# mkkellogg/GaussianSplats3D

Hardware: NVIDIA H100
Metric: frames_per_sec (higher is better)
Workload: dtype int32 sort keys / f32 raster

## Files before the change

### gaussiansplats3d_b200/csrc/engine.cu

```cuda
#include "../../include/gsplat_b200.h"
#include "common.cuh"
#include "sort_kernels.cuh"
#include "raster_kernels.cuh"
#include "shard_kernels.cuh"
#include "ksplat_transform.h"
#include "ksplat_kernels.cuh"
#include "file_kernels.cuh"
#include "cull_kernels.cuh"
#include "ray_kernels.cuh"
#include "generate_kernels.cuh"

#include <algorithm>
#include <cmath>
#include <cstdarg>
#include <cstdlib>
#include <cstring>
#include <memory>
#include <new>
#include <vector>

using namespace gs;

thread_local char g_gs_err[512] = "";
#define g_err g_gs_err
// ... 208 lines not shown
    CUE(cudaStreamCreateWithFlags(&e->stream, cudaStreamNonBlocking));
    CUE(cudaStreamCreateWithFlags(&e->stream2, cudaStreamNonBlocking));
    CUE(cudaEventCreateWithFlags(&e->ev_fork, cudaEventDisableTiming));
    CUE(cudaEventCreateWithFlags(&e->ev_join, cudaEventDisableTiming));
    for (int i = 0; i < EV_COUNT; ++i) CUE(cudaEventCreate(&e->ev[i]));
    int kb = 0;
    while ((1u << kb) < c.distance_map_range) ++kb;
    e->key_bits = kb;
    int rc = GS_OK;
    const size_t n = std::max<uint32_t>(c.max_splat_count, 1);
    if ((rc = e->centers.ensure(n)) || (rc = e->indexes.ensure(n)) || (rc = e->dist.ensure(n)) || (rc = e->sorted.ensure(n)) ||
        (rc = e->vals[0].ensure(n)) || (rc = e->vals[1].ensure(n)) || (rc = e->keys[0].ensure(n)) || (rc = e->keys[1].ensure(n)) ||
        (rc = e->ctl.ensure(1)) || (rc = e->depthp.ensure(2)) || (rc = e->transforms.ensure(16 * GS_MAX_SCENES)) || (rc = e->h_ctl.ensure(sizeof(SortControl) / 4 + 64 + sizeof(RasterControl) / 4 + sizeof(ShardHeader) / 4))) {
        gs_destroy(e);
        return rc;
    }
    if (c.dynamic_mode && (rc = e->scene_idx.ensure(n))) { gs_destroy(e); return rc; }
    if (c.ray_records && (rc = e->ray.rec.ensure(n))) { gs_destroy(e); return rc; }
    if (e->scene_idx.p) CUE(cudaMemsetAsync(e->scene_idx.p, 0, e->scene_idx.n * 4, e->stream));
    {
        std::vector<float> id(16 * GS_MAX_SCENES, 0.f);
        for (int s = 0; s < GS_MAX_SCENES; ++s) id[16 * s] = id[16 * s + 5] = id[16 * s + 10] = id[16 * s + 15] = 1.f;
        CUE(cudaMemcpy(e->transforms.p, id.data(), id.size() * 4, cudaMemcpyHostToDevice));
    }
    CUE(cudaMemset(e->ctl.p, 0, sizeof(SortControl)));
    rc = raster_init(e->rs, c, e->sm_count);
    if (rc) { gs_destroy(e); return fail(rc, "raster_init failed: %s", g_err); }
    if ((rc = e->status_dev.ensure(2 * kPipeSlotWords))) { gs_destroy(e); return rc; }
    CUE(cudaMemset(e->status_dev.p, 0, 2 * kPipeSlotWords * 4));
    e->rs.snap_base = e->status_dev.p;
    e->rs.snap_stride = (uint32_t)kPipeSlotWords;
    e->rs.snap_sort_ctl = reinterpret_cast<const uint32_t *>(e->ctl.p);
    CUE(cudaStreamSynchronize(e->stream));
    *out = e;
    return GS_OK;
}

#undef CUE

extern "C" void gs_destroy(gs_engine *e) {
    if (!e) return;
    cudaSetDevice(e->cfg.device);
    if (e->stream) cudaStreamSynchronize(e->stream);
    e->centers.release(); e->scene_idx.release(); e->indexes.release(); e->precomputed.release(); e->dist.release();
    e->keys[0].release(); e->keys[1].release(); e->vals[0].release(); e->vals[1].release(); e->sorted.release();
    e->transforms.release(); e->ctl.release(); e->depthp.release(); e->tile_hist.release(); e->freq.release(); e->dist_rows_i.release(); e->dist_rows_f.release(); e->sub_idx.release(); e->sub_dist.release();
    e->h_indexes.release(); e->h_sorted.release(); e->h_ctl.release(); e->h_frame.release(); e->h_pipe.release();
    e->tree.center.release(); e->tree.nmin.release(); e->tree.nmax.release(); e->tree.offsets.release(); e->tree.indexes.release(); e->tree.start.release(); e->tree.key.release(); e->tree.total.release(); e->tree.all_min.release(); e->tree.all_max.release(); e->tree.parent.release(); e->tree.leaf_node.release(); e->ray.release(); e->flush.release(); e->prof.release();
    e->shard.block.release(); e->shard.total.release(); e->shard.ahead.release(); e->shard.block_total.release(); e->shard.delta.release(); e->shard.local_sorted.release();
    for (void *m : e->shard.opened) if (m) cudaIpcCloseMemHandle(m);
    if (e->rs.peer_attached) { if (e->rs.peer_frame) cudaIpcCloseMemHandle(e->rs.peer_frame); if (e->rs.peer_sync) cudaIpcCloseMemHandle(e->rs.peer_sync); }
    raster_release(e->rs);
    for (int i = 0; i < EV_COUNT; ++i) if (e->ev[i]) cudaEventDestroy(e->ev[i]);
    if (e->stream) cudaStreamDestroy(e->stream);
    if (e->stream2) cudaStreamDestroy(e->stream2);
    if (e->copy_stream) cudaStreamDestroy(e->copy_stream);
    for (int i = 0; i < gs_engine::kPipeRing; ++i) { if (e->ev_frame_done[i]) cudaEventDestroy(e->ev_frame_done[i]); if (e->ev_copy_done[i]) cudaEventDestroy(e->ev_copy_done[i]); }
    for (int i = 0; i < 2; ++i) if (e->ev_params[i]) cudaEventDestroy(e->ev_params[i]);
    if (e->param_stream) cudaStreamDestroy(e->param_stream);
    e->status_dev.release();
    if (e->graph_exec) cudaGraphExecDestroy(e->graph_exec);
    if (e->graph_exec_alt) cudaGraphExecDestroy(e->graph_exec_alt);
    if (e->ev_fork) cudaEventDestroy(e->ev_fork);
    if (e->ev_join) cudaEventDestroy(e->ev_join);
    delete e;
}

extern "C" int gs_upload_centers(gs_engine *e, const void *centers, const uint32_t *sceneIndexes, uint32_t from, uint32_t count) {
    int rc = check_engine(e);
    if (rc) return rc;
    if (!centers && count) return fail(GS_ERR_BAD_ARG, "gs_upload_centers: null centers");
    if ((uint64_t)from + count > e->cfg.max_splat_count) return fail(GS_ERR_CAPACITY, "centres [%u,%u) exceed max_splat_count %u", from, from + count, e->cfg.max_splat_count);
    e->ray.valid = false;
    if (count) CU(cudaMemcpyAsync(e->centers.p + from, centers, (size_t)count * 16, cudaMemcpyHostToDevice, e->stream));
    if (e->cfg.dynamic_mode && sceneIndexes && count)
        CU(cudaMemcpyAsync(e->scene_idx.p + from, sceneIndexes, (size_t)count * 4, cudaMemcpyHostToDevice, e->stream));
    CU(cudaStreamSynchronize(e->stream));
    e->uploaded_splats = from + count;
    return GS_OK;
}

template <int MODE>
static void launch_depth(bool identity, int blocks, cudaStream_t st, const uint32_t *idx, const void *centers, const void *pre,
                         const uint32_t *scene, const float *tr, const DepthParams *P, uint32_t s0, uint32_t rc, int32_t *dist, SortControl *ctl) {
    if (identity) gs_launch(k_depth<MODE, true>, blocks, kDepthThreads, 0, st, idx, centers, pre, scene, tr, P, s0, rc, dist, ctl);
    else gs_launch(k_depth<MODE, false>, blocks, kDepthThreads, 0, st, idx, centers, pre, scene, tr, P, s0, rc, dist, ctl);
}

static int enqueue_depth(gs_engine *e, const uint32_t *d_indexes, const float *mvp, bool use_pre, uint32_t lo, uint32_t hi, bool capturing) {
    cudaStream_t st = e->stream;
    const uint32_t n = hi - lo;
    DepthParams P{};
    memcpy(P.mvp, mvp, 64);
    P.irow[0] = (int32_t)((double)mvp[2] * 1000.0);
    P.irow[1] = (int32_t)((double)mvp[6] * 1000.0);
    P.irow[2] = (int32_t)((double)mvp[10] * 1000.0);
    P.irow[3] = 1;
    P.frow[0] = mvp[2]; P.frow[1] = mvp[6]; P.frow[2] = mvp[10]; P.frow[3] = 0.f;
    if (!capturing) CU(cudaMemcpyAsync(e->depthp.p + e->rs.frame_parity, &P, sizeof(P), cudaMemcpyHostToDevice, st));
    const bool integer = e->cfg.integer_based_sort, dyn = e->cfg.dynamic_mode;
    const int mode = use_pre ? (integer ? kIntPrecomputed : kFloatPrecomputed)
                             : (integer ? (dyn ? kIntDynamic : kIntStatic) : (dyn ? kFloatDynamic : kFloatStatic));
    const int dblocks = (int)std::max<uint64_t>(1, std::min<uint64_t>(((uint64_t)n + kDepthThreads * kDepthItems - 1) / (kDepthThreads * kDepthItems), (uint64_t)e->sm_count * 8));
    const bool identity = (d_indexes == nullptr);
    const void *pre = e->precomputed.p;
    switch (mode) {
        case kIntStatic: launch_depth<kIntStatic>(identity, dblocks, st, d_indexes, e->centers.p, pre, e->scene_idx.p, e->transforms.p, e->depthp.p + e->rs.frame_parity, lo, hi, e->dist.p, e->ctl.p); break;
        case kIntDynamic: launch_depth<kIntDynamic>(identity, dblocks, st, d_indexes, e->centers.p, pre, e->scene_idx.p, e->transforms.p, e->depthp.p + e->rs.frame_parity, lo, hi, e->dist.p, e->ctl.p); break;
        case kIntPrecomputed: launch_depth<kIntPrecomputed>(identity, dblocks, st, d_indexes, e->centers.p, pre, e->scene_idx.p, e->transforms.p, e->depthp.p + e->rs.frame_parity, lo, hi, e->dist.p, e->ctl.p); break;
        case kFloatStatic: launch_depth<kFloatStatic>(identity, dblocks, st, d_indexes, e->centers.p, pre, e->scene_idx.p, e->transforms.p, e->depthp.p + e->rs.frame_parity, lo, hi, e->dist.p, e->ctl.p); break;
        case kFloatDynamic: launch_depth<kFloatDynamic>(identity, dblocks, st, d_indexes, e->centers.p, pre, e->scene_idx.p, e->transforms.p, e->depthp.p + e->rs.frame_parity, lo, hi, e->dist.p, e->ctl.p); break;
        default: launch_depth<kFloatPrecomputed>(identity, dblocks, st, d_indexes, e->centers.p, pre, e->scene_idx.p, e->transforms.p, e->depthp.p + e->rs.frame_parity, lo, hi, e->dist.p, e->ctl.p); break;
    }
    return GS_OK;
}

static int sort_on_device(gs_engine *e, const uint32_t *d_indexes, const float *mvp, uint32_t sort_count, uint32_t render_count,
                          bool use_pre, bool write_buckets, bool capturing = false, bool subset = false, cudaEvent_t wait_for_rects = nullptr) {
    if (sort_count > render_count) return fail(GS_ERR_BAD_ARG, "sortCount %u > renderCount %u", sort_count, render_count);
    if (render_count > e->cfg.max_splat_count) return fail(GS_ERR_CAPACITY, "renderCount %u > max_splat_count %u", render_count, e->cfg.max_splat_count);
    cudaStream_t st = e->stream;
    const uint32_t s0 = render_count - sort_count, n = sort_count;
    const PassPlan pl = make_plan_bits(e->key_bits);
    uint32_t launches = 0;
    uint32_t stride = 0;
    int rc = e->tile_hist.ensure(radix_tile_hist_words(std::max(n, 1u), pl.npasses, &stride));
    if (rc) return rc;
    if (!capturing) CU(cudaEventRecord(e->ev[EV_SORT0], st));
    if (!e->have_prof_begin) e->prof.begin(st);
    if (e->ctl_dirty && !capturing) {
        gs_launch(k_sort_init, 1, 256, 0, st, e->ctl.p);
        ++launches;
    }
    if (!capturing) e->ctl_dirty = true;
    if (s0 > 0) { gs_launch(k_copy_head, std::min<uint32_t>((s0 + 255) / 256, e->sm_count * 8), 256, 0, st, d_indexes, e->sorted.p, s0); ++launches; e->prof.mark("k_copy_head", st); }
    if (n > 0) {
        if ((rc = enqueue_depth(e, d_indexes, mvp, use_pre, s0, render_count, capturing))) return rc;
        const bool identity = (d_indexes == nullptr);
        ++launches;
        e->prof.mark("k_depth", st);
        if (!capturing) CU(cudaEventRecord(e->ev[EV_DEPTH], st));
        const uint32_t tiles = (n + kRadixTile - 1) / kRadixTile;
        const uint32_t R = e->cfg.distance_map_range;
        const uint32_t *vsrc = identity ? nullptr : d_indexes + s0;
        int vmode = identity ? kValIotaReversed : kValArrayReversed;
        int32_t *dist_sorted = e->dist.p + s0;
        const unsigned long long *n_dev = nullptr;
        if (subset) {
            if (wait_for_rects) CU(cudaStreamWaitEvent(st, wait_for_rects, 0));
            int rcs = raster_subset(e->rs, e->cfg, d_indexes, render_count, e->dist.p, e->sub_idx.p, e->sub_dist.p, st, e->prof, launches);
            if (rcs) return rcs;
            vsrc = e->sub_idx.p; vmode = kValArrayReversed;
            dist_sorted = e->sub_dist.p;
            n_dev = &e->rs.rctl.p->subset_count;
        }
        static const RadixNames names = {{"k_radix_hist[depth,0]", "k_radix_hist[depth,1]", "k_radix_hist[depth,2]", "k_radix_hist[depth,3]"},
                                         {"k_radix_scan[depth,0]", "k_radix_scan[depth,1]", "k_radix_scan[depth,2]", "k_radix_scan[depth,3]"},
                                         {"k_radix_scatter[depth,0]", "k_radix_scatter[depth,1]", "k_radix_scatter[depth,2]", "k_radix_scatter[depth,3]"}};
        if (e->key_bits <= 16) {
            gs_launch(k_bucket<uint16_t>, tiles, kRadixThreads, 0, st, dist_sorted, (uint16_t *)e->keys[0].p, n, n_dev, R, pl, write_buckets ? 1 : 0, e->ctl.p, e->tile_hist.p, stride);
            ++launches;
            e->prof.mark("k_bucket", st);
            if (!capturing) CU(cudaEventRecord(e->ev[EV_BUCKET], st));
            radix_sort_pairs<uint16_t, uint32_t>((uint16_t *)e->keys[0].p, (uint16_t *)e->keys[1].p, vsrc, render_count - 1u, vmode, e->vals[0].p, e->vals[1].p,
                                       e->sorted.p + s0, n, n_dev, (unsigned long long)n, pl, e->ctl.p, e->tile_hist.p, stride, true, nullptr, st, launches, &e->prof, names, true);
        } else {
            gs_launch(k_bucket<uint32_t>, tiles, kRadixThreads, 0, st, dist_sorted, e->keys[0].p, n, n_dev, R, pl, write_buckets ? 1 : 0, e->ctl.p, e->tile_hist.p, stride);
            ++launches;
            e->prof.mark("k_bucket", st);
            if (!capturing) CU(cudaEventRecord(e->ev[EV_BUCKET], st));
            radix_sort_pairs<uint32_t, uint32_t>(e->keys[0].p, e->keys[1].p, vsrc, render_count - 1u, vmode, e->vals[0].p, e->vals[1].p, e->sorted.p + s0, n,
                                       n_dev, (unsigned long long)n, pl, e->ctl.p, e->tile_hist.p, stride, true, nullptr, st, launches, &e->prof, names, true);
        }
    } else if (!capturing) {
        CU(cudaEventRecord(e->ev[EV_DEPTH], st));
        CU(cudaEventRecord(e->ev[EV_BUCKET], st));
    }
    if (!capturing) CU(cudaEventRecord(e->ev[EV_SORT1], st));
    CU(cudaGetLastError());
    e->tm.kernel_launches = launches;
    e->last_render_count = render_count;
    e->have_sorted = true;
    if (!capturing) e->ctl_dirty = false;
    return GS_OK;
}

static int finish_sort(gs_engine *e, float *sort_time_ms) {
    CU(cudaMemcpyAsync(e->h_ctl.p, e->ctl.p, 12, cudaMemcpyDeviceToHost, e->stream));
    CU(cudaStreamSynchronize(e->stream));
    float ms = 0.f;
    if (e->last_frame_was_graph) {
        e->tm.depth_ms = e->tm.bucket_ms = e->tm.scatter_ms = 0.f;
        cudaEventElapsedTime(&ms, e->ev[EV_SORT0], e->ev[EV_R1]);
    } else {
        cudaEventElapsedTime(&e->tm.depth_ms, e->ev[EV_SORT0], e->ev[EV_DEPTH]);
        cudaEventElapsedTime(&e->tm.bucket_ms, e->ev[EV_DEPTH], e->ev[EV_BUCKET]);
        cudaEventElapsedTime(&e->tm.scatter_ms, e->ev[EV_BUCKET], e->ev[EV_SORT1]);
        cudaEventElapsedTime(&ms, e->ev[EV_SORT0], e->ev[EV_SORT1]);
    }
    e->tm.sort_total_ms = ms;
    if (sort_time_ms) *sort_time_ms = ms;
    const uint32_t err = e->h_ctl.p[2];
    if (err & kErrBucketRange) return fail(GS_ERR_BUCKET_RANGE, "a bucket index fell outside [0,%u): distances overflow the int32/f32 range map", e->cfg.distance_map_range);
    return GS_OK;
}

static int stage_sort_inputs(gs_engine *e, const gs_sort_params *p, const uint32_t **d_indexes) {
    cudaStream_t st = e->stream;
    *d_indexes = nullptr;
    CU(cudaEventRecord(e->ev[EV_H2D0], st));
    if (p->indexes_to_sort_dev) *d_indexes = p->indexes_to_sort_dev;
    else if (p->indexes_to_sort) {
        CU(cudaMemcpyAsync(e->indexes.p, p->indexes_to_sort, (size_t)p->render_count * 4, cudaMemcpyHostToDevice, st));
        *d_indexes = e->indexes.p;
    }
    if (e->cfg.dynamic_mode && p->transforms) CU(cudaMemcpyAsync(e->transforms.p, p->transforms, 16 * GS_MAX_SCENES * 4, cudaMemcpyHostToDevice, st));
    if (p->use_precomputed_distances) {
        if (!p->precomputed_distances) return fail(GS_ERR_BAD_ARG, "use_precomputed_distances without precomputed_distances");
        int rc = e->precomputed.ensure(e->cfg.max_splat_count);
        if (rc) return rc;
        CU(cudaMemcpyAsync(e->precomputed.p, p->precomputed_distances, (size_t)e->uploaded_splats * 4, cudaMemcpyHostToDevice, st));
    }
    CU(cudaEventRecord(e->ev[EV_H2D1], st));
    return GS_OK;
}

extern "C" int gs_sort(gs_engine *e, const gs_sort_params *p, uint32_t *sorted_out, float *sort_time_ms) {
    int rc = check_engine(e);
    if (rc) return rc;
    if (!p) return fail(GS_ERR_BAD_ARG, "gs_sort: null params");
    gs_sort_params q = *p;
    q.render_count = std::min(q.render_count, e->uploaded_splats);
    q.sort_count = std::min(q.sort_count, e->uploaded_splats);
    if (q.sort_count > q.render_count) return fail(GS_ERR_BAD_ARG, "sortCount %u > renderCount %u", q.sort_count, q.render_count);
    const uint32_t *d_idx = nullptr;
    e->last_frame_was_graph = false;
    if ((rc = stage_sort_inputs(e, &q, &d_idx))) return rc;
    if ((rc = sort_on_device(e, d_idx, q.model_view_proj, q.sort_count, q.render_count, q.use_precomputed_distances != 0, false))) return rc;
    CU(cudaEventRecord(e->ev[EV_D2H0], e->stream));
    if (sorted_out && q.render_count) CU(cudaMemcpyAsync(sorted_out, e->sorted.p, (size_t)q.render_count * 4, cudaMemcpyDeviceToHost, e->stream));
    CU(cudaEventRecord(e->ev[EV_D2H1], e->stream));
    rc = finish_sort(e, sort_time_ms);
    cudaEventElapsedTime(&e->tm.h2d_ms, e->ev[EV_H2D0], e->ev[EV_H2D1]);
    cudaEventElapsedTime(&e->tm.d2h_ms, e->ev[EV_D2H0], e->ev[EV_D2H1]);
    return rc;
}


static int shard_prepare(gs_engine *e) {
    const uint32_t R = e->cfg.distance_map_range;
    int rc;
    const size_t bytes = sizeof(ShardHeader) + (size_t)R * sizeof(uint2);
    if (e->shard.block.n < bytes) {
        if ((rc = e->shard.block.ensure(bytes))) return rc;
        CU(cudaMemset(e->shard.block.p, 0, bytes));
    }
    const size_t blocks = ((size_t)R + kShardScanThreads - 1) / kShardScanThreads;
    if ((rc = e->shard.total.ensure(R)) || (rc = e->shard.ahead.ensure(R)) || (rc = e->shard.delta.ensure(R)) || (rc = e->shard.block_total.ensure(blocks)) ||
        (rc = e->shard.local_sorted.ensure(e->cfg.max_splat_count)))
        return rc;
    const PassPlan pl = make_plan_bits(e->key_bits);
    if ((rc = e->tile_hist.ensure(radix_tile_hist_words(std::max(e->cfg.max_splat_count, 1u), pl.npasses, nullptr))) || (rc = e->precomputed.ensure(e->cfg.max_splat_count))) return rc;
    return GS_OK;
}
template <typename F> static inline void preload_kernel(F f) { cudaFuncAttributes a; (void)cudaFuncGetAttributes(&a, f); }
template <typename KeyT> static void shard_preload_keyed() {
    preload_kernel(k_bucket<KeyT>);
    preload_kernel(k_radix_hist<KeyT>);
    preload_kernel(k_shard_place<KeyT>);
    preload_kernel(k_radix_scatter<KeyT, uint32_t, kValArray, true, false>);
    preload_kernel(k_radix_scatter<KeyT, uint32_t, kValArrayReversed, true, false>);
    preload_kernel(k_radix_scatter<KeyT, uint32_t, kValIotaReversed, true, false>);
    preload_kernel(k_radix_scatter<KeyT, uint32_t, kValArray, true, true>);
    preload_kernel(k_radix_scatter<KeyT, uint32_t, kValArrayReversed, true, true>);
    preload_kernel(k_radix_scatter<KeyT, uint32_t, kValIotaReversed, true, true>);
}
template <int MODE> static void shard_preload_depth() { preload_kernel(k_depth<MODE, true>); preload_kernel(k_depth<MODE, false>); }
static void shard_preload(gs_engine *e) {
    preload_kernel(k_sort_init); preload_kernel(k_copy_head); preload_kernel(k_radix_scan);
    preload_kernel(k_shard_exchange_minmax); preload_kernel(k_shard_exchange_runs); preload_kernel(k_shard_totals); preload_kernel(k_shard_delta); preload_kernel(k_shard_done);
    shard_preload_depth<kIntStatic>(); shard_preload_depth<kIntDynamic>(); shard_preload_depth<kIntPrecomputed>();
    shard_preload_depth<kFloatStatic>(); shard_preload_depth<kFloatDynamic>(); shard_preload_depth<kFloatPrecomputed>();
    if (e->key_bits <= 16) shard_preload_keyed<uint16_t>(); else shard_preload_keyed<uint32_t>();
    (void)cudaGetLastError();
}
static inline ShardHeader *shard_hdr(void *block) { return (ShardHeader *)block; }
static inline const uint2 *shard_runs(void *block) { return (const uint2 *)((unsigned char *)block + sizeof(ShardHeader)); }

extern "C" int gs_shard_export(gs_engine *e, void *block_handle, void *sorted_handle) {
    int rc = check_engine(e);
    if (rc) return rc;
    if (!block_handle || !sorted_handle) return fail(GS_ERR_BAD_ARG, "gs_shard_export: null");
    if ((rc = shard_prepare(e))) return rc;
    cudaIpcMemHandle_t h;
    CU(cudaIpcGetMemHandle(&h, e->shard.block.p));
    memcpy(block_handle, &h, sizeof(h));
    CU(cudaIpcGetMemHandle(&h, e->sorted.p));
    memcpy(sorted_handle, &h, sizeof(h));
    return GS_OK;
}
static int shard_bind(gs_engine *e, uint32_t world, void *const *blocks, uint32_t *root_out) {
    for (uint32_t g = 0; g < world; ++g) {
        e->shard.peers.hdr[g] = shard_hdr(blocks[g]);
        e->shard.peers.runs[g] = shard_runs(blocks[g]);
    }
    shard_preload(e);
    e->shard.root_out = root_out;
    e->shard.world = world;
    e->shard.seq = 0;
    e->shard.attached = true;
    return GS_OK;
}
static int shard_check_group(gs_engine *e, uint32_t world, const char *who) {
    if (world < 1 || world > (uint32_t)kMaxShardRanks) return fail(GS_ERR_BAD_ARG, "%s: world %u outside [1, %d]", who, world, kMaxShardRanks);
    if (e->cfg.world_size != world || e->cfg.rank >= world) return fail(GS_ERR_BAD_ARG, "%s: engine was created as rank %u of %u, not of %u", who, e->cfg.rank, e->cfg.world_size, world);
    return GS_OK;
}
extern "C" int gs_shard_attach(gs_engine *e, uint32_t world, const void *block_handles, const void *root_sorted_handle) {
    int rc = check_engine(e);
    if (rc) return rc;
    if (!block_handles || !root_sorted_handle) return fail(GS_ERR_BAD_ARG, "gs_shard_attach: null");
    if ((rc = shard_check_group(e, world, "gs_shard_attach")) || (rc = shard_prepare(e))) return rc;
    void *blocks[kMaxShardRanks] = {nullptr};
    for (uint32_t g = 0; g < world; ++g) {
        if (g == e->cfg.rank) { blocks[g] = e->shard.block.p; continue; }
        cudaIpcMemHandle_t h;
        memcpy(&h, (const unsigned char *)block_handles + (size_t)g * GS_IPC_HANDLE_BYTES, sizeof(h));
        CU(cudaIpcOpenMemHandle(&blocks[g], h, cudaIpcMemLazyEnablePeerAccess));
        e->shard.opened[g] = blocks[g];
    }
    uint32_t *root_out = e->sorted.p;
    if (e->cfg.rank != 0) {
        cudaIpcMemHandle_t h;
        void *m = nullptr;
        memcpy(&h, root_sorted_handle, sizeof(h));
        CU(cudaIpcOpenMemHandle(&m, h, cudaIpcMemLazyEnablePeerAccess));
        e->shard.opened[kMaxShardRanks] = m;
        root_out = (uint32_t *)m;
    }
    return shard_bind(e, world, blocks, root_out);
}
extern "C" int gs_shard_attach_local(gs_engine *e, uint32_t world, gs_engine *const *engines) {
    int rc = check_engine(e);
    if (rc) return rc;
    if (!engines) return fail(GS_ERR_BAD_ARG, "gs_shard_attach_local: null");
    if ((rc = shard_check_group(e, world, "gs_shard_attach_local"))) return rc;
    void *blocks[kMaxShardRanks] = {nullptr};
    for (uint32_t g = 0; g < world; ++g) {
        gs_engine *pe = engines[g];
        if (!pe || pe->cfg.device != e->cfg.device || pe->cfg.rank != g || pe->cfg.world_size != world ||
            pe->cfg.distance_map_range != e->cfg.distance_map_range)
            return fail(GS_ERR_BAD_ARG, "gs_shard_attach_local: engines[%u] must be rank %u of %u on device %d with the same distance_map_range", g, g, world, e->cfg.device);
        if ((rc = shard_prepare(pe))) return rc;
        blocks[g] = pe->shard.block.p;
    }
    return shard_bind(e, world, blocks, engines[0]->sorted.p);
}

template <typename KeyT>
static int shard_local_sort(gs_engine *e, const uint32_t *d_indexes, uint32_t s0, uint32_t lo, uint32_t hi, uint32_t &launches) {
    cudaStream_t st = e->stream;
    const uint32_t n = hi - lo, R = e->cfg.distance_map_range;
    const PassPlan pl = make_plan_bits(e->key_bits);
    uint32_t stride = 0;
    int rc = e->tile_hist.ensure(radix_tile_hist_words(std::max(n, 1u), pl.npasses, &stride));
    if (rc) return rc;
    const bool identity = (d_indexes == nullptr);
    static const RadixNames names = {{"k_radix_hist[shard,0]", "k_radix_hist[shard,1]", "k_radix_hist[shard,2]", "k_radix_hist[shard,3]"},
                                     {"k_radix_scan[shard,0]", "k_radix_scan[shard,1]", "k_radix_scan[shard,2]", "k_radix_scan[shard,3]"},
                                     {"k_radix_scatter[shard,0]", "k_radix_scatter[shard,1]", "k_radix_scatter[shard,2]", "k_radix_scatter[shard,3]"}};
    const uint32_t me = e->cfg.rank, world = e->shard.world, seq = e->shard.seq;
    uint2 *runs = (uint2 *)shard_runs(e->shard.block.p);
    KeyT *final_keys = nullptr;
    if (n) {
        const uint32_t tiles = (n + kRadixTile - 1) / kRadixTile;
        gs_launch(k_bucket<KeyT>, tiles, kRadixThreads, 0, st, e->dist.p + lo, (KeyT *)e->keys[0].p, n, nullptr, R, pl, 0, e->ctl.p, e->tile_hist.p, stride);
        ++launches;
        e->prof.mark("k_bucket", st);
        radix_sort_pairs<KeyT, uint32_t>((KeyT *)e->keys[0].p, (KeyT *)e->keys[1].p, identity ? nullptr : d_indexes + lo, hi - 1u,
                                         identity ? kValIotaReversed : kValArrayReversed, e->vals[0].p, e->vals[1].p, e->shard.local_sorted.p, n, nullptr,
                                         (unsigned long long)n, pl, e->ctl.p, e->tile_hist.p, stride, true, runs, st, launches, &e->prof, names, true, true, &final_keys);
    }
    k_shard_exchange_runs<<<1, 32, 0, st>>>(e->shard.peers, me, world, seq);
    ++launches;
    e->prof.mark("k_shard_exchange_runs", st);
    if (n) {
        const uint32_t sblocks = (R + kShardScanThreads - 1) / kShardScanThreads;
        k_shard_totals<<<sblocks, kShardScanThreads, 0, st>>>(e->shard.peers, me, world, R, e->shard.total.p, e->shard.ahead.p, e->shard.block_total.p);
        k_shard_delta<<<sblocks, kShardScanThreads, 0, st>>>(runs, R, e->shard.total.p, e->shard.ahead.p, e->shard.block_total.p, e->shard.delta.p);
        e->prof.mark("k_shard_offsets", st);
        k_shard_place<KeyT><<<std::min<uint32_t>((n + 255) / 256, e->sm_count * 16), 256, 0, st>>>(final_keys, e->shard.local_sorted.p, n, e->shard.delta.p, e->shard.root_out + s0);
        e->prof.mark("k_shard_place", st);
        launches += 3;
    }
    return GS_OK;
}

static inline uint32_t shard_bound(uint32_t s0, uint32_t n, uint32_t g, uint32_t world) { return s0 + (uint32_t)(((uint64_t)n * g) / world); }

extern "C" int gs_sort_sharded_async(gs_engine *e, const gs_sort_params *p) {
    int rc = check_engine(e);
    if (rc) return rc;
    if (!p) return fail(GS_ERR_BAD_ARG, "gs_sort_sharded: null params");
    if (!e->shard.attached) return fail(GS_ERR_NOT_READY, "gs_sort_sharded: call gs_shard_attach (or gs_shard_attach_local) first");
    if (e->shard.pending) return fail(GS_ERR_NOT_READY, "gs_sort_sharded_async: the previous sharded sort has not been finished");
    gs_sort_params q = *p;
    q.render_count = std::min(q.render_count, e->uploaded_splats);
    q.sort_count = std::min(q.sort_count, e->uploaded_splats);
    if (q.sort_count > q.render_count) return fail(GS_ERR_BAD_ARG, "sortCount %u > renderCount %u", q.sort_count, q.render_count);
    const uint32_t *d_idx = nullptr;
    e->last_frame_was_graph = false;
    const uint32_t me = e->cfg.rank, world = e->shard.world;
    uint32_t split_min = 8000000u;
    if (const char *sv = getenv("GS_SHARD_MIN")) split_min = (uint32_t)strtoul(sv, nullptr, 10);
    if (world == 1 || q.sort_count < split_min) {
        e->shard.pending = true;
        e->shard.pending_unsplit = true;
        e->shard.pending_render_count = q.render_count;
        if (me != 0) return GS_OK;
        if ((rc = stage_sort_inputs(e, &q, &d_idx)) ||
            (rc = sort_on_device(e, d_idx, q.model_view_proj, q.sort_count, q.render_count, q.use_precomputed_distances != 0, false))) {
            e->shard.pending = false;
            return rc;
        }
        return GS_OK;
    }
    e->shard.pending_unsplit = false;
    if ((rc = stage_sort_inputs(e, &q, &d_idx))) return rc;
    cudaStream_t st = e->stream;
    const uint32_t s0 = q.render_count - q.sort_count;
    const uint32_t lo = shard_bound(s0, q.sort_count, me, world), hi = shard_bound(s0, q.sort_count, me + 1, world);
    const uint32_t seq = ++e->shard.seq;
    uint32_t launches = 0;
    CU(cudaEventRecord(e->ev[EV_SORT0], st));
    e->prof.begin(st);
    if (e->ctl_dirty) { gs_launch(k_sort_init, 1, 256, 0, st, e->ctl.p); ++launches; }
    e->ctl_dirty = true;
    if (me == 0 && s0 > 0) { gs_launch(k_copy_head, std::min<uint32_t>((s0 + 255) / 256, e->sm_count * 8), 256, 0, st, d_idx, e->sorted.p, s0); ++launches; e->prof.mark("k_copy_head", st); }
    if (hi > lo) {
        if ((rc = enqueue_depth(e, d_idx, q.model_view_proj, q.use_precomputed_distances != 0, lo, hi, false))) return rc;
        ++launches;
        e->prof.mark("k_depth", st);
    }
    k_shard_exchange_minmax<<<1, kShardSyncThreads, 0, st>>>(e->shard.peers, e->ctl.p, me, world, seq, hi > lo ? 0 : 1, (uint2 *)shard_runs(e->shard.block.p),
                                                             e->cfg.distance_map_range);
    ++launches;
    e->prof.mark("k_shard_exchange_minmax", st);
    CU(cudaEventRecord(e->ev[EV_DEPTH], st));
    CU(cudaEventRecord(e->ev[EV_BUCKET], st));
    rc = (e->key_bits <= 16) ? shard_local_sort<uint16_t>(e, d_idx, s0, lo, hi, launches) : shard_local_sort<uint32_t>(e, d_idx, s0, lo, hi, launches);
    if (rc) return rc;
    k_shard_done<<<1, 32, 0, st>>>(e->shard.peers, me, world, seq);
    ++launches;
    e->prof.mark("k_shard_done", st);
    CU(cudaEventRecord(e->ev[EV_SORT1], st));
    CU(cudaGetLastError());
    e->tm.kernel_launches = launches;
    e->last_render_count = q.render_count;
    e->have_sorted = (me == 0);
    e->ctl_dirty = !(hi > lo);
    e->shard.pending = true;
    e->shard.pending_render_count = q.render_count;
    return GS_OK;
}
// ... 204 lines not shown
    e->tm.visible_splats = vis;
    if (rc.peer_timeout) return fail(GS_ERR_CUDA, "multi-GPU tile gather: a peer did not arrive within the time limit (ranks must render the same frames)");
    if (rc.overflow) return fail(GS_ERR_CAPACITY, "tile-instance buffer overflow: %llu instances needed, capacity %llu (raise GS_INSTANCE_FACTOR)",
                                 (unsigned long long)rc.total_instances, (unsigned long long)e->rs.instance_capacity);
    return GS_OK;
}

static int stage_order(gs_engine *e, const gs_render_params *p, const uint32_t **d_order) {
    *d_order = nullptr;
    if (p->render_count > e->cfg.max_splat_count) return fail(GS_ERR_CAPACITY, "render_count %u > max_splat_count %u", p->render_count, e->cfg.max_splat_count);
    if (p->sorted_indexes_dev) *d_order = p->sorted_indexes_dev;
    else if (p->sorted_indexes) {
        CU(cudaMemcpyAsync(e->sorted.p, p->sorted_indexes, (size_t)p->render_count * 4, cudaMemcpyHostToDevice, e->stream));
        *d_order = e->sorted.p;
        e->have_sorted = true;
        e->last_render_count = p->render_count;
    } else {
        if (!e->have_sorted || e->last_render_count < p->render_count) return fail(GS_ERR_NOT_READY, "gs_render without sorted indexes: call gs_sort first or pass sorted_indexes");
        *d_order = e->sorted.p;
    }
    return GS_OK;
}

extern "C" int gs_render(gs_engine *e, const gs_uniforms *u, const gs_render_params *p, void *frame_out) {
    int rc = check_engine(e);
    if (rc) return rc;
    if (!u || !p) return fail(GS_ERR_BAD_ARG, "gs_render: null argument");
    if (e->pipe_inflight()) return fail(GS_ERR_NOT_READY, "gs_render: pipelined frames are in flight (gs_frame_end first)");
    const uint32_t *d_order = nullptr;
    e->last_frame_was_graph = false;
    if ((rc = stage_order(e, p, &d_order))) return rc;
    if ((rc = render_on_device(e, u, p, d_order))) return rc;
    return finish_render(e, p, frame_out);
}

static int upload_frame_params(gs_engine *e, const float *mvp, const gs_uniforms &u, const gs_render_params &p) {
    DepthParams P{};
    memcpy(P.mvp, mvp, 64);
    P.irow[0] = (int32_t)((double)mvp[2] * 1000.0);
    P.irow[1] = (int32_t)((double)mvp[6] * 1000.0);
    P.irow[2] = (int32_t)((double)mvp[10] * 1000.0);
    P.irow[3] = 1;
    P.frow[0] = mvp[2]; P.frow[1] = mvp[6]; P.frow[2] = mvp[10]; P.frow[3] = 0.f;
    cudaStream_t st = e->param_side ? e->param_stream : e->stream;
    CU(cudaMemcpyAsync(e->depthp.p + e->rs.frame_parity, &P, sizeof(P), cudaMemcpyHostToDevice, st));
    int rc = raster_upload_params(e->rs, e->cfg, u, p, st);
    if (rc) return rc;
    if (e->param_side) {
        CU(cudaEventRecord(e->ev_params[e->rs.frame_parity], st));
        CU(cudaStreamWaitEvent(e->stream, e->ev_params[e->rs.frame_parity], 0));
    }
    return GS_OK;
}

static int enqueue_frame(gs_engine *e, const gs_sort_params *s, const gs_uniforms *u, const gs_render_params *p, gs_sort_params &q, gs_render_params &rp) {
    q = *s;
    q.render_count = std::min(q.render_count, e->uploaded_splats);
    q.sort_count = std::min(q.sort_count, e->uploaded_splats);
    const uint32_t *d_idx = nullptr;
    int rc;
    if ((rc = stage_sort_inputs(e, &q, &d_idx))) return rc;
    rp = *p;
    rp.sorted_indexes = nullptr; rp.sorted_indexes_dev = nullptr;
    rp.render_count = std::min(rp.render_count, q.render_count);
    cudaStream_t st = e->stream;
    e->last_frame_was_graph = false;
    const uint32_t subset_min = getenv("GS_SUBSET_MIN") ? (uint32_t)atoll(getenv("GS_SUBSET_MIN")) : 3000000u;
    const bool subset = e->cfg.world_size > 1 && q.sort_count == q.render_count && q.render_count >= subset_min && q.render_count > 0 && !e->no_subset;
    if (subset) {
        if ((rc = e->sub_idx.ensure(e->cfg.max_splat_count)) || (rc = e->sub_dist.ensure(e->cfg.max_splat_count))) return rc;
    }
    const unsigned long long *order_count = subset ? &e->rs.rctl.p->subset_count : nullptr;
    const bool use_graph = e->graph_enabled && !e->prof.on && q.sort_count <= q.render_count && q.render_count <= e->cfg.max_splat_count && e->rs.uploaded;
    if (use_graph) {
        const unsigned long long key[8] = {q.render_count, q.sort_count, ((unsigned long long)rp.width << 32) | rp.height,
                                           ((unsigned long long)rp.frame_format << 8) | (unsigned long long)(rp.flip_y ? 1 : 0) | ((unsigned long long)q.use_precomputed_distances << 4),
                                           (unsigned long long)(uintptr_t)d_idx, ((unsigned long long)e->rs.cov_format << 16) | ((unsigned long long)e->rs.sh_format << 8) | e->rs.sh_degree,
                                           e->rs.uploaded, ((unsigned long long)rp.render_count << 1) | (subset ? 1ull : 0ull)};
        if ((rc = upload_frame_params(e, q.model_view_proj, *u, rp))) return rc;
        cudaGraphExec_t &gexec = e->rs.frame_parity ? e->graph_exec_alt : e->graph_exec;
        unsigned long long *gkey = e->rs.frame_parity ? e->graph_key_alt : e->graph_key;
        if (!gexec || memcmp(key, gkey, sizeof(key)) != 0) {
            if (gexec) { cudaGraphExecDestroy(gexec); gexec = nullptr; }
            uint32_t stride = 0;
            const PassPlan pl = make_plan_bits(e->key_bits);
            if ((rc = e->tile_hist.ensure(radix_tile_hist_words(std::max(q.sort_count, 1u), pl.npasses, &stride)))) return rc;
            CU(cudaStreamBeginCapture(st, cudaStreamCaptureModeThreadLocal));
            struct CaptureGuard {
                cudaStream_t st; bool armed;
                ~CaptureGuard() { if (armed) { cudaGraph_t g = nullptr; cudaStreamEndCapture(st, &g); if (g) cudaGraphDestroy(g); (void)cudaGetLastError(); } }
            } guard{st, true};
            CU(cudaEventRecord(e->ev_fork, st));
            CU(cudaStreamWaitEvent(e->stream2, e->ev_fork, 0));
            int rc2 = GS_OK;
            uint32_t proj_launches = 0;
            {
                cudaStream_t keep = e->stream;
                e->stream = e->stream2;
                rc2 = render_on_device(e, u, &rp, e->sorted.p, true, 1);
                proj_launches = e->tm.kernel_launches;
                e->stream = keep;
            }
            CU(cudaEventRecord(e->ev_join, e->stream2));
            rc = sort_on_device(e, d_idx, q.model_view_proj, q.sort_count, q.render_count, q.use_precomputed_distances != 0, false, true, subset, e->ev_join);
            const uint32_t sort_launches = e->tm.kernel_launches;
            CU(cudaStreamWaitEvent(st, e->ev_join, 0));
            if (!rc2) rc2 = rc ? rc : render_on_device(e, u, &rp, e->sorted.p, true, 2, order_count);
            e->graph_launches = e->tm.kernel_launches + sort_launches + proj_launches;
            cudaGraph_t g = nullptr;
            guard.armed = false;
            cudaError_t ce = cudaStreamEndCapture(st, &g);
            if (rc2) { if (g) cudaGraphDestroy(g); return rc2; }
            if (ce != cudaSuccess) return fail(GS_ERR_CUDA, "cudaStreamEndCapture -> %s", cudaGetErrorString(ce));
            ce = cudaGraphInstantiate(&gexec, g, 0);
            cudaGraphDestroy(g);
            if (ce != cudaSuccess) { gexec = nullptr; return fail(GS_ERR_CUDA, "cudaGraphInstantiate -> %s", cudaGetErrorString(ce)); }
            memcpy(gkey, key, sizeof(key));
            e->graph_snapshot[e->rs.frame_parity ? 1 : 0] = e->rs.snapshot_taken;
        }
        if (e->ctl_dirty) gs_launch(k_sort_init, 1, 256, 0, st, e->ctl.p);
        e->ctl_dirty = true;
        CU(cudaEventRecord(e->ev[EV_SORT0], st));
        CU(cudaGraphLaunch(gexec, st));
        e->ctl_dirty = false;
        CU(cudaEventRecord(e->ev[EV_R1], st));
        e->tm.kernel_launches = e->graph_launches;
        e->last_render_count = q.render_count;
        e->have_sorted = !subset;
        e->last_frame_was_graph = true;
        return GS_OK;
    }
    if (subset) {
        e->prof.begin(st);
        e->have_prof_begin = true;
        if ((rc = render_on_device(e, u, &rp, e->sorted.p, false, 1))) { e->have_prof_begin = false; return rc; }
        const uint32_t proj_launches = e->tm.kernel_launches;
        if ((rc = sort_on_device(e, d_idx, q.model_view_proj, q.sort_count, q.render_count, q.use_precomputed_distances != 0, false, false, true, nullptr))) { e->have_prof_begin = false; return rc; }
        const uint32_t sort_launches = e->tm.kernel_launches;
        rc = render_on_device(e, u, &rp, e->sorted.p, false, 2, order_count);
        e->have_prof_begin = false;
        if (rc) return rc;
        e->tm.kernel_launches += sort_launches + proj_launches;
        e->have_sorted = false;
        return GS_OK;
    }
    if ((rc = sort_on_device(e, d_idx, q.model_view_proj, q.sort_count, q.render_count, q.use_precomputed_distances != 0, false))) return rc;
    const uint32_t sort_launches = e->tm.kernel_launches;
    e->have_prof_begin = true;
    rc = render_on_device(e, u, &rp, e->sorted.p);
    e->have_prof_begin = false;
    if (rc) return rc;
    e->tm.kernel_launches += sort_launches;
    return GS_OK;
}

extern "C" int gs_frame(gs_engine *e, const gs_sort_params *s, const gs_uniforms *u, const gs_render_params *p, uint32_t *sorted_out, void *frame_out) {
    int rc = check_engine(e);
    if (rc) return rc;
    if (!s || !u || !p) return fail(GS_ERR_BAD_ARG, "gs_frame: null argument");
    if (e->pipe_inflight()) return fail(GS_ERR_NOT_READY, "gs_frame: pipelined frames are in flight (gs_frame_end first)");
    e->rs.frame_parity = 0;
    gs_sort_params q; gs_render_params rp;
    e->no_subset = (sorted_out != nullptr);
    rc = enqueue_frame(e, s, u, p, q, rp);
    e->no_subset = false;
    if (rc) return rc;
    if (sorted_out && q.render_count) CU(cudaMemcpyAsync(sorted_out, e->sorted.p, (size_t)q.render_count * 4, cudaMemcpyDeviceToHost, e->stream));
    int rc2 = finish_render(e, &rp, frame_out);
    rc = finish_sort(e, nullptr);
// ... 142 lines not shown
    return GS_OK;
}

extern "C" int gs_upload_ray_records(gs_engine *e, const gs_ray_record *records, uint32_t from, uint32_t count, const double *scene_transform) {
    int rc = check_engine(e);
    if (rc) return rc;
    if (!e->ray.rec.p) return fail(GS_ERR_NOT_READY, "gs_upload_ray_records: engine created without ray_records");
    if (!records && count) return fail(GS_ERR_BAD_ARG, "gs_upload_ray_records: null records");
    if ((uint64_t)from + count > e->cfg.max_splat_count) return fail(GS_ERR_CAPACITY, "ray records [%u,%u) exceed max_splat_count %u", from, from + count, e->cfg.max_splat_count);
    if (count) CU(cudaMemcpyAsync(e->ray.rec.p + from, records, (size_t)count * sizeof(gs_ray_record), cudaMemcpyHostToDevice, e->stream));
    CU(cudaStreamSynchronize(e->stream));
    static const double kIdentity[16] = {1, 0, 0, 0, 0, 1, 0, 0, 0, 0, 1, 0, 0, 0, 0, 1};
    memcpy(e->ray.xf, scene_transform ? scene_transform : kIdentity, sizeof(e->ray.xf));
    e->ray.valid = true;
    return GS_OK;
}

extern "C" int gs_upload_splat_tree_nodes(gs_engine *e, const double *node_min, const double *node_max, const int32_t *node_parent, uint32_t node_count,
                                          const uint32_t *leaf_node, uint32_t leaf_count) {
    int rc = check_engine(e);
    if (rc) return rc;
    auto &t = e->tree;
    if (leaf_count != t.count) return fail(GS_ERR_BAD_ARG, "gs_upload_splat_tree_nodes: %u leaves, the uploaded tree has %u", leaf_count, t.count);
    if ((node_count && (!node_min || !node_max || !node_parent)) || (leaf_count && !leaf_node)) return fail(GS_ERR_BAD_ARG, "gs_upload_splat_tree_nodes: null argument");
    for (uint32_t i = 0; i < node_count; ++i)
        if (node_parent[i] >= (int32_t)i || (i == 0) != (node_parent[i] < 0)) return fail(GS_ERR_BAD_ARG, "gs_upload_splat_tree_nodes: node %u has parent %d", i, node_parent[i]);
    for (uint32_t i = 0; i < leaf_count; ++i)
        if (leaf_node[i] >= node_count) return fail(GS_ERR_BAD_ARG, "gs_upload_splat_tree_nodes: leaf %u -> node %u of %u", i, leaf_node[i], node_count);
    const size_t m = std::max<uint32_t>(node_count, 1);
    if ((rc = t.all_min.ensure(3 * m)) || (rc = t.all_max.ensure(3 * m)) || (rc = t.parent.ensure(m)) || (rc = t.leaf_node.ensure(std::max<uint32_t>(leaf_count, 1))))
        return rc;
    cudaStream_t st = e->stream;
    if (node_count) {
        CU(cudaMemcpyAsync(t.all_min.p, node_min, 24 * (size_t)node_count, cudaMemcpyHostToDevice, st));
        CU(cudaMemcpyAsync(t.all_max.p, node_max, 24 * (size_t)node_count, cudaMemcpyHostToDevice, st));
        CU(cudaMemcpyAsync(t.parent.p, node_parent, 4 * (size_t)node_count, cudaMemcpyHostToDevice, st));
    }
    if (leaf_count) CU(cudaMemcpyAsync(t.leaf_node.p, leaf_node, 4 * (size_t)leaf_count, cudaMemcpyHostToDevice, st));
    CU(cudaStreamSynchronize(st));
    t.node_count = node_count;
    t.have_nodes = true;
    return GS_OK;
}

extern "C" int gs_raycast(gs_engine *e, const gs_raycast_params *p, gs_ray_hit *hits, uint32_t capacity, uint32_t *hit_count) {
    int rc = check_engine(e);
    if (rc) return rc;
    if (!p || !hit_count || (capacity && !hits)) return fail(GS_ERR_BAD_ARG, "gs_raycast: null argument");
    gs_raycast_params q{};
    memcpy(&q, p, std::min<size_t>(p->struct_size ? p->struct_size : sizeof(q), sizeof(q)));
    auto &t = e->tree;
    auto &R = e->ray;
    if (!R.rec.p) return fail(GS_ERR_NOT_READY, "gs_raycast: engine created without ray_records");
    if (!R.valid) return fail(GS_ERR_NOT_READY, "gs_raycast: the ray records are stale (upload the scene or gs_upload_ray_records)");
    if (!t.have_nodes) return fail(GS_ERR_NOT_READY, "gs_raycast: no SplatTree (gs_upload_splat_tree + gs_upload_splat_tree_nodes)");
    *hit_count = 0;
    if (!t.count || !t.node_count || !q.scene_visible) return GS_OK;
    RayParams P{};
    memcpy(P.origin, q.origin, sizeof(P.origin)); memcpy(P.dir, q.direction, sizeof(P.dir));
    memcpy(P.from_local, q.from_local, sizeof(P.from_local)); memcpy(P.xf, R.xf, sizeof(P.xf));
    P.ellipsoid = q.mode == GS_RAYCAST_ELLIPSOID; P.dynamic = e->cfg.dynamic_mode;
    const uint32_t m = t.count, nn = t.node_count, n = std::max<uint32_t>(t.splats, 1);
    if ((rc = R.setup.ensure(1)) || (rc = R.pass.ensure(nn)) || (rc = R.reached.ensure(m)) || (rc = R.list.ensure(m)) || (rc = R.counts.ensure(4)) ||
        (rc = R.hits.ensure(n)))
        return rc;
    cudaStream_t st = e->stream;
    uint32_t launches = 0;
    k_ray_setup<<<1, 1, 0, st>>>(P, R.setup.p);
    k_ray_nodes<<<(nn + 127) / 128, 128, 0, st>>>(t.all_min.p, t.all_max.p, nn, R.setup.p, R.pass.p);
    k_ray_leaves<<<(m + 127) / 128, 128, 0, st>>>(t.leaf_node.p, t.parent.p, R.pass.p, m, R.reached.p);
    k_ray_compact<<<1, kRayCompactThreads, 0, st>>>(R.reached.p, m, R.list.p, R.counts.p);
    const uint32_t grid = std::min<uint32_t>((m + kRaySplatThreads / 32 - 1) / (kRaySplatThreads / 32), (uint32_t)e->sm_count * 16);
    k_ray_splats<<<grid, kRaySplatThreads, 0, st>>>(R.list.p, R.counts.p, t.offsets.p, t.indexes.p, R.rec.p, P, R.setup.p, R.hits.p, R.counts.p + 1);
    launches += 5;
    CU(cudaGetLastError());
    CU(cudaMemcpyAsync(e->h_ctl.p + 8, R.counts.p, 8, cudaMemcpyDeviceToHost, st));
    CU(cudaStreamSynchronize(st));
    const uint32_t total = e->h_ctl.p[9];
    *hit_count = total;
    const uint32_t k = std::min(capacity, total);
    if (!k) { e->tm.kernel_launches = launches; return GS_OK; }
    const uint32_t *perm = nullptr;
    if (total > 1) {
        uint32_t stride = 0;
        int pos_bits = 1;
        while (pos_bits < 32 && (1ull << pos_bits) < (unsigned long long)t.splats) ++pos_bits;
        if ((rc = R.keys[0].ensure(n)) || (rc = R.keys[1].ensure(n)) || (rc = R.vals[0].ensure(n)) || (rc = R.vals[1].ensure(n)) || (rc = R.vals[2].ensure(n)) ||
            (rc = R.vals[3].ensure(n)) || (rc = R.tile_hist.ensure(radix_tile_hist_words(total, 4, &stride))))
            return rc;
        if (!R.ctl.p) {
            if ((rc = R.ctl.ensure(1))) return rc;
            CU(cudaMemsetAsync(R.ctl.p, 0, sizeof(SortControl), st));
        }
        static const RadixNames names{{"ray_hist0", "ray_hist1", "ray_hist2", "ray_hist3"}, {"ray_scan0", "ray_scan1", "ray_scan2", "ray_scan3"},
                                      {"ray_scatter0", "ray_scatter1", "ray_scatter2", "ray_scatter3"}};
        uint32_t *order = nullptr;
        for (int which = 0; which < 4; ++which) {
            const PassPlan pl = make_plan_bits(which == 0 ? pos_bits : kRayKeyBits[which]);
            uint32_t *dst = R.vals[2 + (which & 1)].p;
            k_ray_keys<<<(total + 255) / 256, 256, 0, st>>>(R.hits.p, order, total, which, R.keys[0].p, R.vals[0].p);
            ++launches;
            radix_sort_pairs<uint32_t, uint32_t>(R.keys[0].p, R.keys[1].p, R.vals[0].p, 0, kValArray, R.vals[1].p, R.vals[0].p, dst, total, nullptr, 0, pl,
                                                 R.ctl.p, R.tile_hist.p, stride, false, nullptr, st, launches, nullptr, names, true);
            order = dst;
        }
        perm = order;
    }
    if ((rc = R.out.ensure(k))) return rc;
    k_ray_out<<<(k + 127) / 128, 128, 0, st>>>(R.hits.p, perm, k, R.out.p);
    ++launches;
    CU(cudaMemcpyAsync(hits, R.out.p, (size_t)k * sizeof(gs_ray_hit), cudaMemcpyDeviceToHost, st));
    CU(cudaStreamSynchronize(st));
    CU(cudaGetLastError());
    e->tm.kernel_launches = launches;
    return GS_OK;
}

static void set_ray_scene(gs_engine *e, const gs_ksplat_options &o) {
    if (!e->ray.rec.p) return;
    static const double kIdentity[16] = {1, 0, 0, 0, 0, 1, 0, 0, 0, 0, 1, 0, 0, 0, 0, 1};
    memcpy(e->ray.xf, o.has_transform ? o.transform : kIdentity, sizeof(e->ray.xf));
    e->ray.valid = true;
}

static uint32_t rd32(const unsigned char *p) { uint32_t v; memcpy(&v, p, 4); return v; }
static uint16_t rd16(const unsigned char *p) { uint16_t v; memcpy(&v, p, 2); return v; }
static float rdf(const unsigned char *p) { float v; memcpy(&v, p, 4); return v; }

static int upload_ksplat_image(gs_engine *e, const void *data, size_t bytes, const gs_ksplat_options *opt, gs_ksplat_info *info, const unsigned char *d_image) {
    int rc = check_engine(e);
    if (rc) return rc;
    if (!data || bytes < 4096) return fail(GS_ERR_BAD_ARG, "gs_upload_ksplat: buffer shorter than the 4096-byte header");
    if (!e->cfg.max_width || !e->cfg.max_height) return fail(GS_ERR_NOT_READY, "engine created without a framebuffer (max_width/max_height = 0)");
    gs_ksplat_options o{};
    o.minimum_alpha = 1; o.upload_sort_centers = 1;
    if (opt) memcpy(&o, opt, std::min<size_t>(opt->struct_size ? opt->struct_size : sizeof(o), sizeof(o)));
    const unsigned char *f = (const unsigned char *)data;
    const uint32_t max_sections = rd32(f + 4), max_splats = rd32(f + 12), level = rd16(f + 20);
    if (f[0] == 0 && f[1] < 1) return fail(GS_ERR_BAD_ARG, "unsupported .ksplat version %u.%u", f[0], f[1]);
    if (level > 2) return fail(GS_ERR_BAD_ARG, ".ksplat compression level %u unknown", level);
    if (max_splats > e->cfg.max_splat_count) return fail(GS_ERR_CAPACITY, ".ksplat holds %u splats, engine capacity %u", max_splats, e->cfg.max_splat_count);
    if (4096ull + 1024ull * max_sections > bytes) return fail(GS_ERR_BAD_ARG, ".ksplat truncated (section headers)");
    static const uint32_t kC[3] = {12, 6, 6}, kS[3] = {12, 6, 6}, kR[3] = {16, 8, 8}, kSH[3] = {4, 2, 1}, kRange[3] = {1, 32767, 32767};
    std::vector<KSectionParams> secs;
    std::vector<std::vector<uint32_t>> prefixes;
    unsigned long long base = 4096ull + 1024ull * max_sections;
    uint32_t offset = 0, min_degree = 2;
    for (uint32_t i = 0; i < max_sections; ++i) {
        const unsigned char *h = f + 4096 + 1024ull * i;
        KSectionParams P{};
        P.count = rd32(h + 4);
        P.bucket_size = rd32(h + 8);
        const uint32_t bucket_count = rd32(h + 12);
        const float block = rdf(h + 16);
        const uint32_t storage = rd16(h + 20);
        P.scale_range = rd32(h + 24) ? rd32(h + 24) : kRange[level];
        P.full_bucket_count = rd32(h + 32);
        P.partial_count = rd32(h + 36);
        P.sh_degree_file = rd16(h + 40);
        if (P.sh_degree_file > 2) return fail(GS_ERR_BAD_ARG, ".ksplat section %u: SH degree %d", i, P.sh_degree_file);
        const uint32_t ncomp = P.sh_degree_file == 2 ? 24 : (P.sh_degree_file == 1 ? 9 : 0);
        P.bytes_per_splat = kC[level] + kS[level] + kR[level] + 4 + kSH[level] * ncomp;
        const unsigned long long meta = 4ull * P.partial_count, buckets_bytes = (unsigned long long)storage * bucket_count + meta;
        P.base = base; P.buckets_base = base + meta; P.data_base = base + buckets_bytes;
        P.splat_offset = offset; P.level = (int)level;
        P.scale_factor = ((double)block / 2.0) / (double)P.scale_range;
        if (P.data_base + (unsigned long long)P.bytes_per_splat * P.count > bytes) return fail(GS_ERR_BAD_ARG, ".ksplat truncated (section %u data)", i);
        if (level >= 1 && P.count) {
            if (P.bucket_size == 0 || storage != 12) return fail(GS_ERR_BAD_ARG, ".ksplat section %u: bucket size %u / bucket storage %u bytes (expected > 0 / 12)", i, P.bucket_size, storage);
            if ((unsigned long long)P.full_bucket_count + P.partial_count > bucket_count) return fail(GS_ERR_BAD_ARG, ".ksplat section %u: %u full + %u partial buckets exceed its %u bucket centres", i, P.full_bucket_count, P.partial_count, bucket_count);
        }
        if (P.data_base > bytes || P.buckets_base > P.data_base) return fail(GS_ERR_BAD_ARG, ".ksplat truncated (section %u buckets)", i);
        std::vector<uint32_t> pre(P.partial_count + 1, 0);
        for (uint32_t k = 0; k < P.partial_count; ++k) {
            const unsigned long long len = rd32(f + P.base + 4ull * k);
            if (len > P.count) return fail(GS_ERR_BAD_ARG, ".ksplat section %u: partial bucket %u claims %llu splats", i, k, len);
            pre[k + 1] = pre[k] + (uint32_t)len;
        }
        if (level >= 1 && (unsigned long long)P.full_bucket_count * P.bucket_size + pre[P.partial_count] < P.count) return fail(GS_ERR_BAD_ARG, ".ksplat section %u: buckets do not cover its splats", i);
        if ((unsigned long long)offset + P.count > max_splats || (unsigned long long)offset + P.count > e->cfg.max_splat_count)
            return fail(GS_ERR_CAPACITY, ".ksplat sections hold more than the %u splats its header declares (engine capacity %u)", max_splats, e->cfg.max_splat_count);
        prefixes.push_back(pre);
        min_degree = std::min<uint32_t>(min_degree, (uint32_t)P.sh_degree_file);
        base += (unsigned long long)P.bytes_per_splat * P.count + buckets_bytes;
        offset += P.count;
        secs.push_back(P);
// ... 186 lines not shown

extern "C" int gs_upload_file(gs_engine *e, int format, const void *data, size_t bytes, uint32_t sh_degree, const gs_ksplat_options *opt,
                              gs_ksplat_info *info) {
    int rc = check_engine(e);
    if (rc) return rc;
    if (!e->cfg.max_width || !e->cfg.max_height) return fail(GS_ERR_NOT_READY, "engine created without a framebuffer (max_width/max_height = 0)");
    if (sh_degree > 2) return fail(GS_ERR_BAD_ARG, "gs_upload_file: sphericalHarmonicsDegree %u (0..2)", sh_degree);
    FileLayout L;
    if (parse_file(format, data, bytes, L, g_err, sizeof(g_err))) return GS_ERR_BAD_ARG;
    if (L.count > e->cfg.max_splat_count) return fail(GS_ERR_CAPACITY, "the file holds %u splats, engine capacity %u", L.count, e->cfg.max_splat_count);
    gs_ksplat_options o{};
    o.minimum_alpha = 1; o.upload_sort_centers = 1;
    if (opt) memcpy(&o, opt, std::min<size_t>(opt->struct_size ? opt->struct_size : sizeof(o), sizeof(o)));
    const uint32_t degree = std::min<uint32_t>(sh_degree, (uint32_t)L.sh_degree);
    const uint32_t ncomp = degree == 2 ? 24 : (degree == 1 ? 9 : 0), out_bytes = 44 + 4 * ncomp;

    DevBuf<KTransform> d_xf;
    struct Scratch {
        DevBuf<KTransform> &c;
        ~Scratch() { c.release(); }
    } scratch{d_xf};
    cudaStream_t st = e->stream;
    RasterState &rs = e->rs;
    KSectionParams KP{};
    KP.level = 0; KP.bytes_per_splat = out_bytes; KP.sh_degree_file = (int)degree; KP.sh_degree_out = (int)degree;
    KP.scale_range = 1; KP.minimum_alpha = o.minimum_alpha; KP.half_cov = o.half_covariances; KP.integer_centers = e->cfg.integer_based_sort;
    KP.write_sort_centers = o.upload_sort_centers;
    auto prepare = [&]() -> int {
        if (o.has_transform) {
            KTransform K;
            ksplat_transform_params(o.transform, -1.5, 1.5, K);
            int r;
            if ((r = d_xf.ensure(1))) return r;
            CU(cudaMemcpyAsync(d_xf.p, &K, sizeof(K), cudaMemcpyHostToDevice, st));
            CU(cudaStreamSynchronize(st));
        }
        cudaError_t ce;
        if ((ce = rs.cov.ensure((size_t)e->cfg.max_splat_count * (o.half_covariances ? 12 : 24) + 16)) != cudaSuccess) return fail(GS_ERR_CUDA, "cudaMalloc -> %s", cudaGetErrorString(ce));
        if (ncomp && (ce = rs.sh.ensure((size_t)e->cfg.max_splat_count * ncomp * 2 + 16)) != cudaSuccess) return fail(GS_ERR_CUDA, "cudaMalloc -> %s", cudaGetErrorString(ce));
        rs.uploaded = 0;
        e->ray.valid = false;
        rs.cov_format = o.half_covariances ? GS_COV_F16 : GS_COV_F32;
        rs.sh_degree = degree;
        rs.sh_format = degree ? GS_SH_F16 : GS_SH_NONE;
        e->prof.begin(st);
        return GS_OK;
    };
    rc = parse_file_chunks(L, data, degree, st, e->prof, nullptr, GenOut{}, prepare, [&](uint32_t first, uint32_t n, const unsigned char *d_l0) -> int {
        KP.count = n; KP.splat_offset = first;
        if (o.has_transform) k_ksplat_decode<true><<<(n + 127) / 128, 128, 0, st>>>(d_l0, KP, nullptr, rs.cc.p, rs.cov.p, rs.sh.p, e->centers.p, d_xf.p, e->ray.rec.p);
        else k_ksplat_decode<false><<<(n + 127) / 128, 128, 0, st>>>(d_l0, KP, nullptr, rs.cc.p, rs.cov.p, rs.sh.p, e->centers.p, nullptr, e->ray.rec.p);
        e->prof.mark("k_ksplat_decode", st);
        CU(cudaGetLastError());
        return GS_OK;
    });
    if (rc) return rc;
    rs.uploaded = L.count;
    rs.have_scene_idx = false;
    if (o.upload_sort_centers) e->uploaded_splats = L.count;
    set_ray_scene(e, o);
    if (info) fill_file_info(info, L.count, degree);
    return GS_OK;
}

template <typename T> struct ScopedBuf : DevBuf<T> {
    ScopedBuf() = default;
    ScopedBuf(const ScopedBuf &) = delete;
    ScopedBuf &operator=(const ScopedBuf &) = delete;
    ~ScopedBuf() { this->release(); }
};
struct GenImage {
    ScopedBuf<unsigned char> image;
    size_t bytes = 0;
    uint32_t splats = 0, sections = 0, level = 0;
    std::vector<unsigned char> head;
    std::vector<std::pair<unsigned long long, uint32_t>> lens;
};

struct GenSort {
    ScopedBuf<uint32_t> keys[2], vals[3], tile_hist;
    ScopedBuf<SortControl> ctl;
    int run(const unsigned long long *key, const uint32_t *order, uint32_t n, int bits, uint32_t *out, cudaStream_t st, uint32_t &launches) {
        int rc;
        uint32_t stride = 0;
        if ((rc = keys[0].ensure(n)) || (rc = keys[1].ensure(n)) || (rc = vals[0].ensure(n)) || (rc = vals[1].ensure(n)) || (rc = vals[2].ensure(n)) ||
            (rc = tile_hist.ensure(radix_tile_hist_words(std::max(n, 1u), 3, &stride))))
            return rc;
        if (!ctl.p) {
            if ((rc = ctl.ensure(1))) return rc;
            CU(cudaMemsetAsync(ctl.p, 0, sizeof(SortControl), st));
        }
        static const RadixNames names{{"gen_hist0", "gen_hist1", "gen_hist2", "gen_hist3"}, {"gen_scan0", "gen_scan1", "gen_scan2", "gen_scan3"},
                                      {"gen_scatter0", "gen_scatter1", "gen_scatter2", "gen_scatter3"}};
        if (n == 0) return GS_OK;
        const int rounds = std::max(1, (bits + 23) / 24);
        for (int r = 0; r < rounds; ++r) {
            const PassPlan pl = make_plan_bits(std::min(24, bits - 24 * r));
            uint32_t *dst = (r == rounds - 1) ? out : vals[2].p;
            k_gen_sort_piece<<<(n + 255) / 256, 256, 0, st>>>(key, order, n, 24 * r, keys[0].p, vals[0].p);
            ++launches;
            radix_sort_pairs<uint32_t, uint32_t>(keys[0].p, keys[1].p, vals[0].p, 0, kValArray, vals[1].p, vals[0].p, dst, n, nullptr, 0, pl,
                                                 ctl.p, tile_hist.p, stride, false, nullptr, st, launches, nullptr, names, true);
            order = dst;
        }
        return GS_OK;
    }
};

static int gen_scan(const uint32_t *in, uint32_t n, uint32_t *out, ScopedBuf<uint32_t> &sums, cudaStream_t st, uint32_t &launches) {
    int rc;
    const uint32_t tiles = (uint32_t)(((uint64_t)n + kScanTile - 1) / kScanTile);
    if ((rc = sums.ensure(tiles + 1))) return rc;
    CU(cudaMemsetAsync(sums.p + tiles, 0, 4, st));
    if (tiles) k_gen_scan_reduce<<<tiles, kScanThreads, 0, st>>>(in, n, sums.p);
    k_exclusive_scan_single_block<<<1, 1024, 0, st>>>(sums.p, tiles + 1);
    if (tiles) k_gen_scan_apply<<<tiles, kScanThreads, 0, st>>>(in, n, sums.p, tiles, out);
    else CU(cudaMemsetAsync(out, 0, 4, st));
    launches += tiles ? 3 : 1;
    return GS_OK;
}

static int check_generate_options(const gs_generate_options *gen, gs_generate_options &g) {
    memset(&g, 0, sizeof(g));
    g.compression_level = 1; g.minimum_alpha = 1;
    if (gen) memcpy(&g, gen, std::min<size_t>(gen->struct_size ? gen->struct_size : sizeof(g), sizeof(g)));
    if (g.bucket_size == 0) g.bucket_size = 256;
    if (g.block_size == 0.0) g.block_size = 5.0;
    if (g.compression_level > 2) return fail(GS_ERR_BAD_ARG, "generate: compression level %u (0..2)", g.compression_level);
    if (!(g.block_size > 0.0) || !std::isfinite(g.block_size)) return fail(GS_ERR_BAD_ARG, "generate: block size %g (finite, > 0)", g.block_size);
    if (g.bucket_size > 0x80000000u) return fail(GS_ERR_BAD_ARG, "generate: bucket size %u (<= 2^31)", g.bucket_size);
    return GS_OK;
}

static void put32(unsigned char *p, uint32_t v) { memcpy(p, &v, 4); }
static void put16(unsigned char *p, uint16_t v) { memcpy(p, &v, 2); }
static void putf(unsigned char *p, float v) { memcpy(p, &v, 4); }

static int generate_image(const FileLayout &L, const void *data, uint32_t sh_degree, const gs_generate_options &g, cudaStream_t st, Profiler &prof,
                          GenImage &out, uint32_t &launches) {
    int rc;
    const uint32_t degree = std::min<uint32_t>(sh_degree, (uint32_t)L.sh_degree);
    const uint32_t ncomp = degree == 2 ? 24 : (degree == 1 ? 9 : 0), rec_bytes = 44 + 4 * ncomp, n = L.count;
    const uint32_t level = g.compression_level, B = g.bucket_size;
    static const uint32_t kBytes[3] = {44, 24, 24}, kSH[3] = {4, 2, 1};
    const uint32_t bps = kBytes[level] + kSH[level] * ncomp;
    const uint32_t S = (g.section_size == 0 || g.section_size > n) ? n : g.section_size;
    const uint32_t nsec = n ? (uint32_t)(((uint64_t)n + S - 1) / S) : 0;

    ScopedBuf<unsigned char> rec0; ScopedBuf<double> c64, sh64, bcenter, bucket_center, range;
    ScopedBuf<unsigned long long> key, lo, hi, bmin, bmax, pkey_lo, pkey_hi, offs;
    ScopedBuf<uint32_t> perm, keep, kscan, src, sec, sec_base, nanf, order, head, gscan, gstart, complete, fscan, fbase, pflag, pscan, plist, porder, pinv,
        plen, pcount, pbase, pprefix, bbase, out_src, out_bucket, sums;
    ScopedBuf<GenGeom> geom; ScopedBuf<ShRun> runs;
    GenSort sorter;
    if ((rc = rec0.ensure((size_t)n * rec_bytes)) || (rc = c64.ensure((size_t)n * 3)) || (ncomp && (rc = sh64.ensure((size_t)n * ncomp)))) return rc;
    rc = parse_file_chunks(L, data, degree, st, prof, rec0.p, GenOut{c64.p, ncomp ? sh64.p : nullptr}, [] { return GS_OK; },
                           [](uint32_t, uint32_t, const unsigned char *) { return GS_OK; });
    if (rc) return rc;
    const uint32_t grid_n = (n + kGenThreads - 1) / kGenThreads;
    if ((rc = key.ensure(n)) || (rc = perm.ensure(n))) return rc;
    if (n) k_gen_partition_key<<<grid_n, kGenThreads, 0, st>>>(c64.p, n, g.scene_center[0], g.scene_center[1], g.scene_center[2], key.p);
    if ((rc = sorter.run(key.p, nullptr, n, 64, perm.p, st, launches))) return rc;
    prof.mark("gen_partition", st);
    const uint32_t sh_blocks = (uint32_t)(((uint64_t)n + kGenThreads * kGenShItems - 1) / (kGenThreads * kGenShItems));
    if ((rc = range.ensure(2)) || (rc = runs.ensure(2 * (size_t)std::max(sh_blocks, 1u)))) return rc;
    if (ncomp && sh_blocks) k_gen_sh_scan<<<sh_blocks, kGenThreads, 0, st>>>(sh64.p, (int)ncomp, (int)std::min(ncomp, 23u), perm.p, n, runs.p);
    k_gen_sh_final<<<1, 1, 0, st>>>(runs.p, ncomp ? sh_blocks : 0, range.p);
    prof.mark("gen_sh_range", st);
    if ((rc = keep.ensure(n)) || (rc = kscan.ensure((size_t)n + 1)) || (rc = src.ensure(n)) || (rc = sec.ensure(n)) || (rc = sec_base.ensure((size_t)nsec + 1)))
        return rc;
    if (n) k_gen_keep<<<grid_n, kGenThreads, 0, st>>>(rec0.p, rec_bytes, perm.p, n, g.minimum_alpha, keep.p);
    if ((rc = gen_scan(keep.p, n, kscan.p, sums, st, launches))) return rc;
    if (n) k_gen_compact<<<grid_n, kGenThreads, 0, st>>>(perm.p, keep.p, kscan.p, n, std::max(S, 1u), src.p, sec.p);
    k_gen_section_base<<<nsec / 256 + 1, 256, 0, st>>>(kscan.p, n, std::max(S, 1u), nsec, sec_base.p);
    uint32_t m = 0;
    CU(cudaMemcpyAsync(&m, kscan.p + n, 4, cudaMemcpyDeviceToHost, st));
    CU(cudaStreamSynchronize(st));
    prof.mark("gen_alpha", st);
    const uint32_t grid_m = (m + kGenThreads - 1) / kGenThreads, grid_s = nsec / 256 + 1;
    if ((rc = bmin.ensure((size_t)nsec * 3 + 1)) || (rc = bmax.ensure((size_t)nsec * 3 + 1)) || (rc = nanf.ensure((size_t)nsec * 3 + 1)) ||
        (rc = geom.ensure((size_t)nsec + 1)) || (rc = lo.ensure(m)) || (rc = hi.ensure(m)) || (rc = bcenter.ensure((size_t)m * 3)) || (rc = order.ensure(m)))
        return rc;
    CU(cudaMemsetAsync(bmin.p, 0xff, ((size_t)nsec * 3 + 1) * 8, st));
    CU(cudaMemsetAsync(bmax.p, 0, ((size_t)nsec * 3 + 1) * 8, st));
    CU(cudaMemsetAsync(nanf.p, 0, ((size_t)nsec * 3 + 1) * 4, st));
// ... 353 lines not shown
```

### gaussiansplats3d_b200/csrc/raster_kernels.cuh

```cuda
#pragma once
#include "common.cuh"
#include "sort_kernels.cuh"
#include "../../include/gsplat_b200.h"
#include <cuda_fp16.h>
#include "ellipse_mask.h"

namespace gs {

constexpr int kTile = 16;
constexpr int kTileShift = 4;
constexpr float kTransmittanceCutoff = 1.0f / 512.0f;

struct __align__(16) SplatRecord {
    float cx, cy;
    float g1x, g1y;
    float g2x, g2y;
    uint32_t hxhy;
    float a;
    float r, g, b;
    float ndc_z;
};

constexpr int kVisibleSlots = 64;
struct RasterControl {
// ... 494 lines not shown
            const int src = __ffs(multi) - 1;
            multi &= multi - 1;
            const uint32_t bsid = __shfl_sync(0xffffffffu, sid, src);
            unsigned long long bw = __shfl_sync(0xffffffffu, w, src);
            const int bx0 = __shfl_sync(0xffffffffu, (int)r.x, src), by0 = __shfl_sync(0xffffffffu, (int)r.y, src);
            const int bx1 = __shfl_sync(0xffffffffu, (int)r.z, src), by1 = __shfl_sync(0xffffffffu, (int)r.w, src);
            const int ccx0 = bx0 >> kCoarseShiftX, ccy0 = by0 >> kCoarseShiftY;
            const int cw = (bx1 >> kCoarseShiftX) - ccx0 + 1, chh = (by1 >> kCoarseShiftY) - ccy0 + 1;
            const int ntile = cw * chh;
            for (int i0 = 0; i0 < ntile; i0 += 32) {
                const int i = i0 + lane;
                bool mineq = false;
                int cx = 0, cy = 0;
                if (i < ntile) {
                    cy = ccy0 + i / cw; cx = ccx0 + i % cw;
                    mineq = !sharded || own_diag(own, cx + cy);
                }
                const uint32_t bal = __ballot_sync(0xffffffffu, mineq);
                if (mineq) {
                    const unsigned long long at = bw + __popc(bal & lanemask_lt());
                    const int fx0 = max(bx0, cx * kCoarseW) - cx * kCoarseW, fx1 = min(bx1, cx * kCoarseW + kCoarseW - 1) - cx * kCoarseW;
                    const int fy0 = max(by0, cy * kCoarseH) - cy * kCoarseH, fy1 = min(by1, cy * kCoarseH + kCoarseH - 1) - cy * kCoarseH;
                    const uint32_t rowsel = (0x01010101u >> (8 * (kCoarseH - 1 - (fy1 - fy0)))) << (8 * fy0);
                    const uint32_t mask = (((1u << (fx1 - fx0 + 1)) - 1u) << fx0) * rowsel;
                    if (at < capacity) {
                        keys[at] = (uint16_t)(cy * coarse_x + cx);
                        vals[at] = ((unsigned long long)mask << 32) | bsid;
                    } else overflow = true;
                }
                bw += __popc(bal);
            }
        }
    }
    if (overflow) rctl->overflow = 1;
}


constexpr int kBinTiles = 256;
constexpr int kBinWarps = 16;
constexpr int kBinRankItems = 4;
constexpr int kBinRanks = kBinWarps * 32 * kBinRankItems;

__device__ __forceinline__ uint32_t fine_mask_in_coarse(int rx0, int ry0, int rx1, int ry1, int cx, int cy) {
    const int fx0 = max(rx0, cx * kCoarseW) - cx * kCoarseW, fx1 = min(rx1, cx * kCoarseW + kCoarseW - 1) - cx * kCoarseW;
    const int fy0 = max(ry0, cy * kCoarseH) - cy * kCoarseH, fy1 = min(ry1, cy * kCoarseH + kCoarseH - 1) - cy * kCoarseH;
    const uint32_t rowsel = (0x01010101u >> (8 * (kCoarseH - 1 - (fy1 - fy0)))) << (8 * fy0);
    return (((1u << (fx1 - fx0 + 1)) - 1u) << fx0) * rowsel;
}

template <typename F>
__device__ __forceinline__ void round_instances(bool valid, uint32_t sid, ushort4 r, int coarse_x, const OwnMask &own, bool sharded, F f) {
    const int lane = threadIdx.x & 31;
    const bool nonempty = valid && r.z >= r.x && r.w >= r.y;
    const int cx0 = r.x >> kCoarseShiftX, cx1 = r.z >> kCoarseShiftX, cy0 = r.y >> kCoarseShiftY, cy1 = r.w >> kCoarseShiftY;
    const bool big = nonempty && (uint32_t)(cx1 - cx0 + 1) * (uint32_t)(cy1 - cy0 + 1) > 32u;
    if (nonempty && !big) {
#pragma unroll 1
        for (int cy = cy0; cy <= cy1; ++cy)
#pragma unroll 1
            for (int cx = cx0; cx <= cx1; ++cx) {
                if (sharded && !own_diag(own, cx + cy)) continue;
                f(lane, sid, cy * coarse_x + cx, fine_mask_in_coarse((int)r.x, (int)r.y, (int)r.z, (int)r.w, cx, cy));
            }
    }
    uint32_t multi = __ballot_sync(0xffffffffu, big);
    while (multi) {
        const int src = __ffs(multi) - 1;
        multi &= multi - 1;
        const uint32_t bsid = __shfl_sync(0xffffffffu, sid, src);
        const int bx0 = __shfl_sync(0xffffffffu, (int)r.x, src), by0 = __shfl_sync(0xffffffffu, (int)r.y, src);
        const int bx1 = __shfl_sync(0xffffffffu, (int)r.z, src), by1 = __shfl_sync(0xffffffffu, (int)r.w, src);
        const int ccx0 = bx0 >> kCoarseShiftX, ccy0 = by0 >> kCoarseShiftY;
        const int cw = (bx1 >> kCoarseShiftX) - ccx0 + 1, ntile = cw * ((by1 >> kCoarseShiftY) - ccy0 + 1);
        for (int i = lane; i < ntile; i += 32) {
            const int cy = ccy0 + i / cw, cx = ccx0 + i % cw;
            if (sharded && !own_diag(own, cx + cy)) continue;
            f(src, bsid, cy * coarse_x + cx, fine_mask_in_coarse(bx0, by0, bx1, by1, cx, cy));
        }
    }
}

__global__ void __launch_bounds__(kBinWarps * 32)
k_bin_count(const uint32_t *__restrict__ order, uint32_t render_count_host, const unsigned long long *__restrict__ n_dev, const ushort4 *__restrict__ rects,
            int coarse_x, uint32_t nt, uint32_t *__restrict__ hist, uint32_t stride, uint32_t *__restrict__ totals, ushort4 *__restrict__ rect_by_rank,
            OwnMask own, int sharded) {
    pdl_enter();
    constexpr int W = kBinWarps, ITEMS = kBinRankItems, NT = kBinTiles;
    const uint32_t n = n_dev ? (uint32_t)*n_dev : render_count_host;
    const uint32_t base = blockIdx.x * (uint32_t)(W * 32 * ITEMS);
    if (base >= n) return;
    __shared__ uint32_t s_hist[NT];
    for (uint32_t t = threadIdx.x; t < nt; t += W * 32) s_hist[t] = 0;
    __syncthreads();
    const int lane = threadIdx.x & 31, warp = threadIdx.x >> 5;
    const uint32_t run = base + (uint32_t)warp * (32 * ITEMS) + lane;
    uint32_t sid[ITEMS];
    ushort4 rc[ITEMS];
#pragma unroll
    for (int k = 0; k < ITEMS; ++k) {
        const uint32_t p = run + (uint32_t)k * 32;
        sid[k] = p < n ? ld_nc_u32(order + (n - 1u - p)) : 0xffffffffu;
    }
#pragma unroll
    for (int k = 0; k < ITEMS; ++k) rc[k] = sid[k] != 0xffffffffu ? rects[sid[k]] : make_ushort4(1, 1, 0, 0);
#pragma unroll
    for (int k = 0; k < ITEMS; ++k) {
        const uint32_t p = run + (uint32_t)k * 32;
        if (p < n) rect_by_rank[p] = rc[k];
    }
#pragma unroll 1
    for (int k = 0; k < ITEMS; ++k) {
        uint32_t id = 0; ushort4 r = make_ushort4(1, 1, 0, 0);
#pragma unroll
        for (int j = 0; j < ITEMS; ++j) if (j == k) { id = sid[j]; r = rc[j]; }
        round_instances(id != 0xffffffffu, id, r, coarse_x, own, sharded != 0, [&](int, uint32_t, int t, uint32_t) { atomicAdd(&s_hist[t], 1u); });
    }
    __syncthreads();
    for (uint32_t t = threadIdx.x; t < nt; t += W * 32) {
        const uint32_t v = s_hist[t];
        hist[(size_t)t * stride + blockIdx.x] = v;
        if (v) atomicAdd(&totals[t], v);
    }
}

__global__ void __launch_bounds__(1024)
k_bin_scan(uint32_t *__restrict__ hist, uint32_t stride, uint32_t ranks_per_chunk, uint32_t render_count_host, const unsigned long long *__restrict__ n_dev,
           const uint32_t *__restrict__ totals, uint32_t nt, uint2 *__restrict__ ranges, RasterControl *rctl, uint32_t *__restrict__ tile_order,
           unsigned long long capacity) {
    pdl_enter();
    __shared__ uint32_t s_scan[40];
    __shared__ uint32_t s_carry;
    {
        const uint32_t mine = totals[blockIdx.x];
        bool ahead = false;
        if (threadIdx.x < nt) { const uint32_t o = totals[threadIdx.x]; ahead = o > mine || (o == mine && threadIdx.x < blockIdx.x); }
        const int rank = __syncthreads_count(ahead);
        if (threadIdx.x == 0) tile_order[rank] = blockIdx.x;
    }
    const uint32_t n = n_dev ? (uint32_t)*n_dev : render_count_host;
    const uint32_t nchunks = (uint32_t)(((uint64_t)n + ranks_per_chunk - 1) / ranks_per_chunk);
    const uint32_t d = blockIdx.x;
    {
        uint32_t total;
        const uint32_t c = threadIdx.x < d ? totals[threadIdx.x] : 0u;
        (void)block_exclusive_scan<1024>(c, s_scan, total);
        if (threadIdx.x == 0) {
            s_carry = total;
            const uint32_t mine = totals[d];
            const unsigned long long lo = total, hi = lo + mine;
            ranges[d] = make_uint2((uint32_t)min(lo, capacity), (uint32_t)min(hi, capacity));
            if (d == nt - 1) rctl->total_instances = hi;
        }
    }
    __syncthreads();
    uint32_t *col = hist + (size_t)d * stride;
    for (uint32_t b = 0; b < nchunks; b += 1024) {
        const uint32_t t = b + threadIdx.x;
        const uint32_t v = t < nchunks ? col[t] : 0u;
        uint32_t total;
        const uint32_t ex = block_exclusive_scan<1024>(v, s_scan, total);
        const uint32_t carry = s_carry;
        if (t < nchunks) col[t] = ex + carry;
        __syncthreads();
        if (threadIdx.x == 0) s_carry = carry + total;
        __syncthreads();
    }
}

__global__ void __launch_bounds__(kBinWarps * 32)
k_bin_place(const uint32_t *__restrict__ order, uint32_t render_count_host, const unsigned long long *__restrict__ n_dev, const ushort4 *__restrict__ rect_by_rank,
            int coarse_x, uint32_t nt, const uint32_t *__restrict__ offsets, uint32_t stride, unsigned long long *__restrict__ list, unsigned long long capacity,
            RasterControl *rctl, OwnMask own, int sharded, int pack_ok) {
    pdl_enter();
    constexpr int W = kBinWarps, ITEMS = kBinRankItems, NT = kBinTiles;
    const uint32_t n = n_dev ? (uint32_t)*n_dev : render_count_host;
    const uint32_t base = blockIdx.x * (uint32_t)(W * 32 * ITEMS);
    if (base >= n) return;
    __shared__ uint32_t s_pre[W][NT];
    __shared__ __align__(8) uint32_t s_mask[W][NT];
    static_assert(NT * 4 >= 32 * ITEMS * 8, "the mask row of a warp doubles as the staging buffer of its compacted items");
    for (uint32_t i = threadIdx.x; i < (uint32_t)(W * NT); i += W * 32) (&s_pre[0][0])[i] = 0;
    __syncthreads();
    const int lane = threadIdx.x & 31, warp = threadIdx.x >> 5;
    const uint32_t run = base + (uint32_t)warp * (32 * ITEMS) + lane;
    uint32_t sid[ITEMS];
    ushort4 rc[ITEMS];
#pragma unroll
    for (int k = 0; k < ITEMS; ++k) {
        const uint32_t p = run + (uint32_t)k * 32;
        sid[k] = p < n ? ld_nc_u32(order + (n - 1u - p)) : 0xffffffffu;
        rc[k] = p < n ? rect_by_rank[p] : make_ushort4(1, 1, 0, 0);
    }
    uint32_t *my_pre = s_pre[warp], *my_mask = s_mask[warp];
    uint32_t nvalid = 32u * ITEMS;
    if (pack_ok) {
        const uint32_t lt = lanemask_lt();
        unsigned long long *stage = reinterpret_cast<unsigned long long *>(my_mask);
        uint32_t before = 0;
#pragma unroll
        for (int k = 0; k < ITEMS; ++k) {
            const bool keep = sid[k] != 0xffffffffu && (sharded ? rect_touches_owned(rc[k], own) : (rc[k].z >= rc[k].x && rc[k].w >= rc[k].y));
            const uint32_t bal = __ballot_sync(0xffffffffu, keep);
            if (keep) stage[before + __popc(bal & lt)] = ((unsigned long long)((uint32_t)rc[k].x | ((uint32_t)rc[k].y << 8) | ((uint32_t)rc[k].z << 16) | ((uint32_t)rc[k].w << 24)) << 32) | sid[k];
            before += __popc(bal);
        }
        nvalid = before;
        __syncwarp();
#pragma unroll
        for (int k = 0; k < ITEMS; ++k) {
            const uint32_t j = (uint32_t)k * 32u + (uint32_t)lane;
            sid[k] = 0xffffffffu;
            rc[k] = make_ushort4(1, 1, 0, 0);
            if (j < nvalid) {
                const unsigned long long v = stage[j];
                const uint32_t pr = (uint32_t)(v >> 32);
                sid[k] = (uint32_t)v;
                rc[k] = make_ushort4((unsigned short)(pr & 255u), (unsigned short)((pr >> 8) & 255u), (unsigned short)((pr >> 16) & 255u), (unsigned short)(pr >> 24));
            }
        }
        __syncwarp();
#pragma unroll
        for (int i = 0; i < NT / 32; ++i) my_mask[i * 32 + lane] = 0u;
        __syncwarp();
    }
#pragma unroll
    for (int k = 0; k < ITEMS; ++k)
        if ((uint32_t)k * 32u < nvalid)
            round_instances(sid[k] != 0xffffffffu, sid[k], rc[k], coarse_x, own, sharded != 0, [&](int, uint32_t, int t, uint32_t) { atomicAdd(&my_pre[t], 1u); });
    __syncthreads();
    for (uint32_t t = threadIdx.x; t < nt; t += W * 32) {
        uint32_t at = offsets[(size_t)t * stride + blockIdx.x];
#pragma unroll
        for (int w = 0; w < W; ++w) {
            const uint32_t c = s_pre[w][t];
            s_pre[w][t] = at;
            at += c;
        }
    }
    __syncthreads();
    bool overflow = false;
#pragma unroll
    for (int k = 0; k < ITEMS; ++k) {
        if ((uint32_t)k * 32u >= nvalid) break;
        const bool valid = sid[k] != 0xffffffffu;
#pragma unroll
        for (int i = 0; i < NT / 32; ++i) my_mask[i * 32 + lane] = 0u;
        __syncwarp();
        round_instances(valid, sid[k], rc[k], coarse_x, own, sharded != 0, [&](int owner, uint32_t, int t, uint32_t) {
            atomicOr(&my_mask[t], 1u << owner);
            atomicAdd(&my_pre[t], 1u);
        });
        __syncwarp();
        round_instances(valid, sid[k], rc[k], coarse_x, own, sharded != 0, [&](int owner, uint32_t sid_o, int t, uint32_t fmask) {
            const uint32_t m = my_mask[t];
            const unsigned long long at = (unsigned long long)(my_pre[t] - (uint32_t)__popc(m)) + __popc(m & ((1u << owner) - 1u));
            if (at < capacity) list[at] = ((unsigned long long)fmask << 32) | sid_o;
            else overflow = true;
        });
        __syncwarp();
    }
    if (overflow) rctl->overflow = 1;
}

__global__ void __launch_bounds__(kBinThreads)
k_subset_count(const uint32_t *__restrict__ indexes, uint32_t count, const ushort4 *__restrict__ rects, OwnMask own,
               uint32_t *__restrict__ block_sums, uint32_t *__restrict__ warp_sums, uint32_t *__restrict__ super_sums) {
    pdl_enter();
    __shared__ uint32_t s_w[kBinThreads / 32];
    const int lane = threadIdx.x & 31, warp = threadIdx.x >> 5;
    const uint32_t run = blockIdx.x * kBinTile + (uint32_t)warp * (32 * kBinItems) + lane;
    uint32_t mine = 0;
#pragma unroll
    for (int k = 0; k < kBinItems; ++k) {
        const uint32_t i = run + (uint32_t)k * 32;
        if (i < count) mine += rect_touches_owned(rects[indexes ? ld_nc_u32(indexes + i) : i], own) ? 1u : 0u;
    }
#pragma unroll
    for (int o = 16; o > 0; o >>= 1) mine += __shfl_xor_sync(0xffffffffu, mine, o);
    if (lane == 0) { s_w[warp] = mine; warp_sums[blockIdx.x * (kBinThreads / 32) + warp] = mine; }
    __syncthreads();
    if (threadIdx.x == 0) {
        uint32_t total = 0;
#pragma unroll
        for (int w = 0; w < kBinThreads / 32; ++w) total += s_w[w];
        block_sums[blockIdx.x] = total;
        if (total) atomicAdd(&super_sums[blockIdx.x / kBinThreads], total);
    }
}
__global__ void __launch_bounds__(kBinThreads)
k_subset_emit(const uint32_t *__restrict__ indexes, uint32_t count, const ushort4 *__restrict__ rects, OwnMask own,
              const uint32_t *__restrict__ block_sums, const uint32_t *__restrict__ warp_sums, const uint32_t *__restrict__ super_sums,
              const int32_t *__restrict__ dist, uint32_t *__restrict__ sub_idx, int32_t *__restrict__ sub_dist, RasterControl *rctl) {
    pdl_enter();
    __shared__ uint32_t s_prefix;
    const int lane = threadIdx.x & 31, warp = threadIdx.x >> 5;
    uint32_t before = (uint32_t)chunk_prefix(block_sums, super_sums);
#pragma unroll
    for (int o = 16; o > 0; o >>= 1) before += __shfl_xor_sync(0xffffffffu, before, o);
    if (threadIdx.x == 0) s_prefix = 0;
    __syncthreads();
    if (lane == 0 && before) atomicAdd(&s_prefix, before);
    __syncthreads();
    if (blockIdx.x == gridDim.x - 1 && threadIdx.x == 0) rctl->subset_count = (unsigned long long)s_prefix + block_sums[blockIdx.x];
    uint32_t w0 = s_prefix;
    for (int w = 0; w < warp; ++w) w0 += warp_sums[blockIdx.x * (kBinThreads / 32) + w];
    const uint32_t run = blockIdx.x * kBinTile + (uint32_t)warp * (32 * kBinItems) + lane;
#pragma unroll 2
    for (int k = 0; k < kBinItems; ++k) {
        const uint32_t i = run + (uint32_t)k * 32;
        uint32_t g = 0;
        bool keep = false;
        if (i < count) {
            g = indexes ? ld_nc_u32(indexes + i) : i;
            keep = rect_touches_owned(rects[g], own);
        }
        const uint32_t bal = __ballot_sync(0xffffffffu, keep);
        if (keep) {
            const uint32_t at = w0 + __popc(bal & lanemask_lt());
            sub_idx[at] = g;
            sub_dist[at] = dist[i];
        }
        w0 += __popc(bal);
    }
}

__global__ void k_raster_init(RasterControl *rctl, SortControl *ctl, uint2 *ranges, uint32_t ntiles, uint32_t *super_sums, uint32_t nsuper, uint32_t *bin_totals, uint32_t *tile_order) {
    pdl_enter();
    const size_t tid = (size_t)blockIdx.x * blockDim.x + threadIdx.x;
    const size_t stride = (size_t)gridDim.x * blockDim.x;
    if (tid == 0) {
        rctl->total_instances = 0; rctl->overflow = 0; rctl->visible = 0; rctl->subset_count = 0;
        rctl->frame_seq += 1;
        ctl->error = 0;
    }
    uint32_t *h = &ctl->hist[0][0];
    for (size_t i = tid; i < 4 * kRadix; i += stride) h[i] = 0;
    for (size_t i = tid; i < ntiles; i += stride) ranges[i] = make_uint2(0xffffffffu, 0u);
    for (size_t i = tid; i < (size_t)kVisibleSlots * 8; i += stride) rctl->visible_slots[i] = 0;
    for (size_t i = tid; i < nsuper; i += stride) super_sums[i] = 0;
    if (bin_totals) for (size_t i = tid; i < kBinTiles; i += stride) bin_totals[i] = 0;
    for (size_t i = tid; i < ntiles; i += stride) tile_order[i] = (uint32_t)i;
}

__device__ __forceinline__ float ex2_approx(float x) {
    float y;
    asm("ex2.approx.ftz.f32 %0, %1;" : "=f"(y) : "f"(x));
    return y;
}

struct f32x2 { float lo, hi; };
__device__ __forceinline__ f32x2 pack2(float lo, float hi) { return f32x2{lo, hi}; }
__device__ __forceinline__ f32x2 bcast2(float v) { return pack2(v, v); }
__device__ __forceinline__ float lo2(f32x2 v) { return v.lo; }
__device__ __forceinline__ float hi2(f32x2 v) { return v.hi; }
__device__ __forceinline__ f32x2 fma2(f32x2 a, f32x2 b, f32x2 c) { return f32x2{__fmaf_rn(a.lo, b.lo, c.lo), __fmaf_rn(a.hi, b.hi, c.hi)}; }
__device__ __forceinline__ f32x2 mul2(f32x2 a, f32x2 b) { return f32x2{__fmul_rn(a.lo, b.lo), __fmul_rn(a.hi, b.hi)}; }

template <int NBX, int NBY>
__device__ __noinline__ uint32_t block_touch_mask(float4 a0, float4 a1, float tile_x0, float tile_y0) {
    if (!(a1.w > 0.0f)) return 0u;
    const uint32_t hb = __float_as_uint(a1.z);
    const __half2 hh = *reinterpret_cast<const __half2 *>(&hb);
    const float hx = __low2float(hh), hy = __high2float(hh);
    const float qxx = a0.z * a0.z + a1.x * a1.x, qxy = a0.z * a0.w + a1.x * a1.y, qyy = a0.w * a0.w + a1.y * a1.y;
    const float X0 = tile_x0 - a0.x, Y0 = tile_y0 - a0.y;
    const int ix0 = max(0, (int)ceilf((-hx - X0 - 7.0f) * 0.125f)), ix1 = min(NBX - 1, (int)floorf((hx - X0) * 0.125f));
    const int iy0 = max(0, (int)ceilf((-hy - Y0 - 7.0f) * 0.125f)), iy1 = min(NBY - 1, (int)floorf((hy - Y0) * 0.125f));
    if (ix0 == ix1 && iy0 == iy1) return 1u << (iy0 * NBX + ix0);
    uint32_t bm = 0;
#pragma unroll 1
    for (int iy = iy0; iy <= iy1; ++iy) {
        const float by0 = Y0 + (float)(8 * iy), by1 = by0 + 7.0f;
#pragma unroll 1
        for (int ix = ix0; ix <= ix1; ++ix) {
            const float bx0 = X0 + (float)(8 * ix), bx1 = bx0 + 7.0f;
            if (ellipse_min_q(bx0, bx1, by0, by1, qxx, qxy, qyy) <= 1.0f + kEllipseSlack) bm |= 1u << (iy * NBX + ix);
        }
    }
    return bm;
}

struct StatusSnapshot {
    const uint32_t *sort_ctl;
    const uint32_t *raster_ctl;
    uint32_t *dst;
    const uint32_t *half_src;
    unsigned long long half_bytes;
};

template <int FORMAT, int S>
__global__ void __launch_bounds__(128 * S * S, S == 1 ? 8 : 2)
k_blend(const uint2 *__restrict__ ranges, const unsigned long long *__restrict__ list, const SplatRecord *__restrict__ rec, int tiles_x,
        int tiles_y, int coarse_x, uint32_t rank, uint32_t world, int width, int height, int flip_y, void *__restrict__ frame_base, const uint32_t *__restrict__ tile_order,
        StatusSnapshot snap) {
    pdl_enter();
    void *__restrict__ frame = snap.half_src ? (void *)((unsigned char *)frame_base + (size_t)(*snap.half_src & 1u) * snap.half_bytes) : frame_base;
    if (snap.dst && blockIdx.x == 0) {
        if (threadIdx.x < 3) snap.dst[threadIdx.x] = snap.sort_ctl[threadIdx.x];
        for (uint32_t i = threadIdx.x; i < (uint32_t)(sizeof(RasterControl) / 4); i += blockDim.x) snap.dst[4 + i] = snap.raster_ctl[i];
    }
    constexpr int THREADS = 128 * S * S, WARPS = THREADS / 32, NBX = 2 * S, NBY = 2 * S, TILE = 16 * S;
    constexpr int ROUNDS = S == 1 ? 4 : 1;
    constexpr int BATCH = ROUNDS * THREADS;
    __shared__ float4 s_rec[THREADS + 1][3];
    __shared__ uint32_t s_ids[BATCH];
    __shared__ uint32_t s_cnt[ROUNDS * WARPS + 1];
    __shared__ uint8_t s_list[WARPS][THREADS];
    __shared__ uint8_t s_nlist[WARPS][WARPS];
    static_assert(THREADS <= 256 || sizeof(uint8_t) == 1, "");
    const uint32_t coarse = tile_order[blockIdx.x / kFinePerCoarse], sub = blockIdx.x % kFinePerCoarse;
    const int ccx = (int)(coarse % (uint32_t)coarse_x), ccy = (int)(coarse / (uint32_t)coarse_x);
    const int tx = ccx * kCoarseW + (int)(sub & (kCoarseW - 1)), ty = ccy * kCoarseH + (int)(sub >> kCoarseShiftX);
    if (tx >= tiles_x || ty >= tiles_y) return;
    if (!owns_coarse(ccx, ccy, rank, world)) return;
    const int lane = threadIdx.x & 31, warp = threadIdx.x >> 5;
    const int x = tx * TILE + (warp % NBX) * 8 + (lane & 7), y0 = ty * TILE + (warp / NBX) * 8 + (lane >> 3) * 2;
    const float pxc = (float)x + 0.5f, pyc = (float)y0 + 0.5f;
    const float tile_x0 = (float)(tx * TILE) + 0.5f, tile_y0 = (float)(ty * TILE) + 0.5f;
    f32x2 T = pack2((x < width && y0 < height) ? 1.0f : 0.0f, (x < width && y0 + 1 < height) ? 1.0f : 0.0f);
// ... 94 lines not shown
                    }
                }
            }
            if (__syncthreads_and(wdone)) break;
        }
    }
    const float T0 = lo2(T), T1 = hi2(T), r0 = lo2(Rr), r1 = hi2(Rr), g0 = lo2(Gg), g1 = hi2(Gg), b0 = lo2(Bb), b1 = hi2(Bb);
    if (x < width) {
#pragma unroll
        for (int k = 0; k < 2; ++k) {
            const int y = y0 + k;
            if (y < height) {
                const float Tk = k ? T1 : T0, Rk = k ? r1 : r0, Gk = k ? g1 : g0, Bk = k ? b1 : b0;
                const float A = 1.0f - Tk;
                const int out_row = flip_y ? (height - 1 - y) : y;
                const size_t at = (size_t)out_row * width + x;
                if (FORMAT == GS_FRAME_RGBA32F) {
                    reinterpret_cast<float4 *>(frame)[at] = make_float4(Rk, Gk, Bk, A);
                } else {
                    const uint32_t r8 = (uint32_t)(__saturatef(Rk) * 255.0f + 0.5f), g8 = (uint32_t)(__saturatef(Gk) * 255.0f + 0.5f);
                    const uint32_t b8 = (uint32_t)(__saturatef(Bk) * 255.0f + 0.5f), a8 = (uint32_t)(__saturatef(A) * 255.0f + 0.5f);
                    reinterpret_cast<uint32_t *>(frame)[at] = r8 | (g8 << 8) | (b8 << 16) | (a8 << 24);
                }
            }
        }
    }
    if (world > 1) __threadfence_system();
}

__global__ void k_export_projected(const SplatRecord *__restrict__ rec, const ushort4 *__restrict__ rects, uint32_t count, gs_projected_splat *out) {
    const uint32_t s = blockIdx.x * blockDim.x + threadIdx.x;
    if (s >= count) return;
    const SplatRecord r = rec[s];
    gs_projected_splat o;
    o.cx = r.cx; o.cy = r.cy;
    const float n1 = r.g1x * r.g1x + r.g1y * r.g1y, n2 = r.g2x * r.g2x + r.g2y * r.g2y;
    o.b1x = n1 > 0.f ? r.g1x / n1 : 0.f; o.b1y = n1 > 0.f ? r.g1y / n1 : 0.f;
    o.b2x = n2 > 0.f ? r.g2x / n2 : 0.f; o.b2y = n2 > 0.f ? r.g2y / n2 : 0.f;
    o.r = r.r; o.g = r.g; o.b = r.b; o.a = r.a;
    o.ndc_z = r.ndc_z;
    o.valid = (r.ndc_z >= -1.0f && r.ndc_z <= 1.0f) ? 1u : 0u;
    if (!o.valid) o.ndc_z = 0.f;
    out[s] = o;
}

template <typename T> struct RBuf {
    T *p = nullptr;
    size_t n = 0;
    cudaError_t ensure(size_t count) {
        if (count <= n) return cudaSuccess;
        if (p) cudaFree(p);
        p = nullptr; n = 0;
        cudaError_t e = cudaMalloc((void **)&p, (count ? count : 1) * sizeof(T));
        if (e == cudaSuccess) n = count;
        return e;
    }
    void release() { if (p) cudaFree(p); p = nullptr; n = 0; }
};

struct RasterState {
    RBuf<uint4> cc;
    RBuf<unsigned char> cov, sh;
    RBuf<uint32_t> scene_idx;
    int cov_format = GS_COV_F32, sh_format = GS_SH_NONE;
    uint32_t sh_degree = 0, uploaded = 0;
    bool have_scene_idx = false;
    RBuf<SplatRecord> records;
    RBuf<ushort4> rects;
    RBuf<uint32_t> block_sums;
    RBuf<uint32_t> warp_sums;
    RBuf<uint32_t> super_sums;
    uint32_t super_stride = 0;
    RBuf<uint16_t> ikeys[2];
    RBuf<unsigned long long> ivals[2];
    RBuf<unsigned long long> list;
    RBuf<uint2> ranges;
    RBuf<RasterControl> rctl;
    RBuf<SortControl> sctl;
    RBuf<uint32_t> tile_hist;
    RBuf<uint32_t> bin_hist;
    RBuf<ushort4> rect_by_rank;
    RBuf<uint32_t> tile_order;
    RBuf<uint32_t> bin_totals;
    uint32_t bin_stride = 0;
    RBuf<DynamicUniforms> dyn;
    RBuf<ProjParams> projp;
    RBuf<unsigned char> frame;
    RBuf<unsigned char> frame_alt;
    unsigned char *frame_half2 = nullptr;
    size_t frame_half_bytes = 0;
    int frame_parity = 0;
    uint32_t *snap_base = nullptr;
    uint32_t snap_stride = 0;
    const uint32_t *snap_sort_ctl = nullptr;
    bool snapshot_taken = false;
    RBuf<gs_projected_splat> exported;
    RBuf<PeerSync> peer_sync_local;
    PeerSync *peer_sync = nullptr;
    void *peer_frame = nullptr;
    bool peer_root = false, peer_attached = false;
    unsigned long long instance_capacity = 0;
    uint32_t hist_stride = 0;
    int sm_count = 132;
    int last_format = GS_FRAME_RGBA32F;
    size_t last_frame_bytes = 0;
};

#define RCU(call)                                                                                                 \
    do {                                                                                                          \
        cudaError_t _e = (call);                                                                                  \
        if (_e != cudaSuccess) { snprintf(raster_err(), 512, "%s -> %s (%s:%d)", #call, cudaGetErrorString(_e), __FILE__, __LINE__); return GS_ERR_CUDA; } \
    } while (0)

static inline char *raster_err() { return g_gs_err; }

static inline int frame_tile_shift(uint32_t width, uint32_t height) {
    const uint32_t cx = (width + kTile * kCoarseW - 1) / (kTile * kCoarseW), cy = (height + kTile * kCoarseH - 1) / (kTile * kCoarseH);
    return (cx * cy <= (uint32_t)kBinTiles) ? kTileShift : kTileShift + 1;
}

static inline uint32_t frame_coarse_tiles(uint32_t width, uint32_t height) {
    const uint32_t tpx = 1u << frame_tile_shift(width, height);
    const uint32_t tiles_x = (width + tpx - 1) / tpx, tiles_y = (height + tpx - 1) / tpx;
    return ((tiles_x + kCoarseW - 1) / kCoarseW) * ((tiles_y + kCoarseH - 1) / kCoarseH);
}

static int raster_init(RasterState &rs, const gs_config &c, int sm_count) {
    rs.sm_count = sm_count;
    const size_t n = c.max_splat_count ? c.max_splat_count : 1;
    RCU(rs.rctl.ensure(1));
    RCU(cudaMemset(rs.rctl.p, 0, sizeof(RasterControl)));
    RCU(rs.sctl.ensure(1));
    RCU(rs.dyn.ensure(2));
    RCU(rs.projp.ensure(2));
    RCU(cudaMemset(rs.dyn.p, 0, 2 * sizeof(DynamicUniforms)));
    if (c.max_width && c.max_height) {
        RCU(rs.cc.ensure(n));
        RCU(rs.records.ensure(n));
        RCU(rs.rects.ensure(n));
        RCU(rs.block_sums.ensure((n + kBinTile - 1) / kBinTile + 1));
        RCU(rs.warp_sums.ensure(((n + kBinTile - 1) / kBinTile + 1) * (kBinThreads / 32)));
        rs.super_stride = (uint32_t)(((n + kBinTile - 1) / kBinTile) / kBinThreads + 2);
        RCU(rs.super_sums.ensure(2 * (size_t)rs.super_stride));
        const char *f = getenv("GS_INSTANCE_FACTOR");
        const double factor = f ? atof(f) : 4.0;
        const size_t tiles = (size_t)((c.max_width + kTile - 1) / kTile) * ((c.max_height + kTile - 1) / kTile);
        rs.instance_capacity = (unsigned long long)(factor * (double)n) + 4ull * tiles + 65536ull;
        if (rs.instance_capacity > 0xfffffff0ull) rs.instance_capacity = 0xfffffff0ull;
        RCU(rs.list.ensure(rs.instance_capacity));
        RCU(rs.ranges.ensure(65536));
        RCU(rs.tile_order.ensure(65536));
        RCU(rs.frame.ensure((size_t)c.max_width * (c.max_height + kTile) * 16));
        if (frame_coarse_tiles(c.max_width, c.max_height) > (uint32_t)kBinTiles) {
            for (int i = 0; i < 2; ++i) { RCU(rs.ikeys[i].ensure(rs.instance_capacity)); RCU(rs.ivals[i].ensure(rs.instance_capacity)); }
            RCU(rs.tile_hist.ensure(radix_tile_hist_words(rs.instance_capacity, 2, &rs.hist_stride)));
        }
        {
            const size_t coarse = (size_t)((c.max_width + kTile * kCoarseW - 1) / (kTile * kCoarseW)) * ((c.max_height + kTile * kCoarseH - 1) / (kTile * kCoarseH));
            const size_t chunks = (n + kBinRanks - 1) / kBinRanks + 1;
            rs.bin_stride = (uint32_t)((chunks + 31) & ~(size_t)31);
            RCU(rs.bin_hist.ensure(std::max<size_t>(coarse, 1) * rs.bin_stride));
            RCU(rs.rect_by_rank.ensure(n));
            RCU(rs.bin_totals.ensure(kBinTiles));
            RCU(cudaMemset(rs.bin_totals.p, 0, kBinTiles * 4));
        }
    }
    return GS_OK;
}

static void raster_release(RasterState &rs) {
    rs.cc.release(); rs.cov.release(); rs.sh.release(); rs.scene_idx.release(); rs.records.release(); rs.rects.release();
    rs.block_sums.release(); rs.warp_sums.release(); rs.super_sums.release(); rs.ikeys[0].release(); rs.ikeys[1].release(); rs.ivals[0].release(); rs.ivals[1].release();
    rs.list.release(); rs.ranges.release(); rs.rctl.release(); rs.sctl.release(); rs.tile_hist.release(); rs.bin_hist.release(); rs.bin_totals.release(); rs.rect_by_rank.release(); rs.tile_order.release();
    rs.dyn.release(); rs.projp.release(); rs.frame.release(); rs.frame_alt.release(); rs.peer_sync_local.release(); rs.exported.release();
}

static int raster_upload(RasterState &rs, const gs_config &c, const gs_splat_data &d, cudaStream_t st) {
    if (!c.max_width || !c.max_height) { snprintf(raster_err(), 512, "engine created without a framebuffer (max_width/max_height = 0)"); return GS_ERR_NOT_READY; }
    if ((uint64_t)d.from + d.count > c.max_splat_count) { snprintf(raster_err(), 512, "splat data [%u,%u) exceeds max_splat_count %u", d.from, d.from + d.count, c.max_splat_count); return GS_ERR_CAPACITY; }
    if (!d.centers_colors || !d.covariances) { snprintf(raster_err(), 512, "gs_upload_splat_data: null centers_colors/covariances"); return GS_ERR_BAD_ARG; }
    if (d.sh_degree > 2) { snprintf(raster_err(), 512, "sh_degree %u > 2", d.sh_degree); return GS_ERR_BAD_ARG; }
    const size_t n = c.max_splat_count;
    const size_t cov_elt = d.cov_format == GS_COV_F16 ? 12 : 24;
    const size_t ncomp = d.sh_degree == 2 ? 24 : (d.sh_degree == 1 ? 9 : 0);
    const size_t sh_elt = ncomp * (d.sh_format == GS_SH_F16 ? 2 : (d.sh_format == GS_SH_U8 ? 1 : 4));
    if (d.from == 0) rs.uploaded = 0;
    if (rs.uploaded && (rs.cov_format != d.cov_format || (rs.sh_degree != d.sh_degree) || (ncomp && rs.sh_format != d.sh_format))) {
        snprintf(raster_err(), 512, "splat data format changed between partial uploads"); return GS_ERR_BAD_ARG;
    }
    rs.cov_format = d.cov_format;
    rs.sh_degree = d.sh_degree;
    rs.sh_format = ncomp ? d.sh_format : GS_SH_NONE;
    RCU(rs.cov.ensure(n * cov_elt + 16));
    if (ncomp) {
        if (!d.spherical_harmonics) { snprintf(raster_err(), 512, "sh_degree %u without spherical_harmonics", d.sh_degree); return GS_ERR_BAD_ARG; }
        RCU(rs.sh.ensure(n * sh_elt + 16));
    }
    RCU(cudaMemcpyAsync(rs.cc.p + d.from, d.centers_colors, (size_t)d.count * 16, cudaMemcpyHostToDevice, st));
    RCU(cudaMemcpyAsync(rs.cov.p + (size_t)d.from * cov_elt, d.covariances, (size_t)d.count * cov_elt, cudaMemcpyHostToDevice, st));
    if (ncomp) RCU(cudaMemcpyAsync(rs.sh.p + (size_t)d.from * sh_elt, d.spherical_harmonics, (size_t)d.count * sh_elt, cudaMemcpyHostToDevice, st));
    if (d.scene_indexes) {
        RCU(rs.scene_idx.ensure(n));
        RCU(cudaMemcpyAsync(rs.scene_idx.p + d.from, d.scene_indexes, (size_t)d.count * 4, cudaMemcpyHostToDevice, st));
        rs.have_scene_idx = true;
    }
    rs.uploaded = std::max<uint32_t>(rs.uploaded, d.from + d.count);
    return GS_OK;
}

static unsigned char *raster_second_frame(RasterState &rs) { return rs.frame_alt.p ? rs.frame_alt.p : rs.frame_half2; }
static void *raster_frame_ptr(RasterState &rs, int) { return (rs.frame_parity && raster_second_frame(rs)) ? raster_second_frame(rs) : rs.frame.p; }

template <bool COVF16>
static void launch_project(RasterState &rs, uint32_t count, cudaStream_t st) {
    const int blocks = (int)((count + kProjThreads - 1) / kProjThreads);
    const uint32_t *sc = rs.have_scene_idx ? rs.scene_idx.p : nullptr;
#define GS_PROJ(FMT) gs_launch(k_project<COVF16, FMT>, blocks, kProjThreads, 0, st, rs.cc.p, rs.cov.p, rs.sh.p, (int)rs.sh_degree, sc, rs.dyn.p + rs.frame_parity, rs.projp.p + rs.frame_parity, count, rs.records.p, rs.rects.p, rs.rctl.p)
    switch (rs.sh_format) {
        case GS_SH_F16: GS_PROJ(GS_SH_F16); break;
        case GS_SH_U8: GS_PROJ(GS_SH_U8); break;
        case GS_SH_F32: GS_PROJ(GS_SH_F32); break;
        default: GS_PROJ(GS_SH_NONE); break;
    }
#undef GS_PROJ
}

static int raster_upload_params(RasterState &rs, const gs_config &c, const gs_uniforms &u, const gs_render_params &p, cudaStream_t st) {
    const int tshift = frame_tile_shift(p.width, p.height), tpx = 1 << tshift;
    const int tiles_x = (p.width + tpx - 1) / tpx, tiles_y = (p.height + tpx - 1) / tpx;
    const uint32_t world = c.world_size, rank = c.rank;
    ProjParams P{};
    memcpy(P.mv, u.model_view, 64); memcpy(P.proj, u.projection, 64);
    memcpy(P.cam, u.camera_position, 12);
    P.focal[0] = u.focal[0]; P.focal[1] = u.focal[1]; P.viewport[0] = u.viewport[0]; P.viewport[1] = u.viewport[1];
    P.inv_focal_adj = u.inverse_focal_adjustment; P.ortho_zoom = u.ortho_zoom; P.orthographic = u.orthographic_mode;
    P.splat_scale = u.splat_scale; P.point_cloud = u.point_cloud_mode; P.sh_degree = u.sh_degree; P.antialiased = u.antialiased;
    P.kernel2d = u.kernel_2d_size; P.max_size = u.max_screen_space_splat_size; P.fade_in_complete = u.fade_in_complete;
    memcpy(P.scene_center, u.scene_center, 12); P.fade_start = u.visible_region_fade_start_radius;
    P.dynamic = u.dynamic_mode; P.optional_effects = u.enable_optional_effects; P.scene_count = (int)u.scene_count;
    P.tiles_x = tiles_x; P.tiles_y = tiles_y; P.rank = rank; P.world = world; P.width = (int)p.width; P.height = (int)p.height;
    P.tile_shift = tshift;
    RCU(cudaMemcpyAsync(rs.projp.p + rs.frame_parity, &P, sizeof(P), cudaMemcpyHostToDevice, st));
    if (u.dynamic_mode || u.enable_optional_effects || rs.sh_format == GS_SH_U8) {
        DynamicUniforms du;
        memcpy(du.view, u.view_matrix, 64);
        memcpy(du.transforms, u.scene_transforms, sizeof(du.transforms));
        memcpy(du.sh8_min, u.sh8_min, sizeof(du.sh8_min)); memcpy(du.sh8_max, u.sh8_max, sizeof(du.sh8_max));
        memcpy(du.opacity, u.scene_opacity, sizeof(du.opacity)); memcpy(du.visibility, u.scene_visibility, sizeof(du.visibility));
        RCU(cudaMemcpyAsync(rs.dyn.p + rs.frame_parity, &du, sizeof(du), cudaMemcpyHostToDevice, st));
    }

    return GS_OK;
}

static int raster_render(RasterState &rs, const gs_config &c, const gs_uniforms &u, const gs_render_params &p, const uint32_t *d_order,
                         cudaStream_t st, cudaEvent_t ev_project, cudaEvent_t ev_bin, gs_timings &tm, Profiler &prof, bool upload_params, bool record_events,
                         int phases = 3, const unsigned long long *order_count_dev = nullptr) {
    if (!rs.uploaded) { snprintf(raster_err(), 512, "gs_render before gs_upload_splat_data"); return GS_ERR_NOT_READY; }
    if (p.width == 0 || p.height == 0 || p.width > c.max_width || p.height > c.max_height) {
        snprintf(raster_err(), 512, "frame %ux%u outside the engine's %ux%u", p.width, p.height, c.max_width, c.max_height); return GS_ERR_BAD_ARG;
    }
    if (p.render_count > rs.uploaded) { snprintf(raster_err(), 512, "render_count %u > uploaded splats %u", p.render_count, rs.uploaded); return GS_ERR_CAPACITY; }
    const int tshift = frame_tile_shift(p.width, p.height), tpx = 1 << tshift;
    const int tiles_x = (p.width + tpx - 1) / tpx, tiles_y = (p.height + tpx - 1) / tpx;
    const uint32_t world = c.world_size, rank = c.rank;
    const uint32_t local_tiles = (uint32_t)tiles_x * (uint32_t)tiles_y;
    uint32_t launches = 0;

    if (upload_params) { int prc = raster_upload_params(rs, c, u, p, st); if (prc) return prc; }
    const int coarse_x = (tiles_x + kCoarseW - 1) / kCoarseW, coarse_y = (tiles_y + kCoarseH - 1) / kCoarseH;
    const uint32_t ncoarse = (uint32_t)coarse_x * (uint32_t)coarse_y;
    if (ncoarse > 65536u) { snprintf(raster_err(), 512, "frame %ux%u needs %u coarse tiles (> 65536)", p.width, p.height, ncoarse); return GS_ERR_BAD_ARG; }
    int tile_bits = 1;
    while ((1u << tile_bits) < std::max(ncoarse, 2u)) ++tile_bits;
    const PassPlan pl = make_plan_bits(tile_bits);
    if (phases & 1) {
        gs_launch(k_raster_init, 8, 256, 0, st, rs.rctl.p, rs.sctl.p, rs.ranges.p, ncoarse, rs.super_sums.p, 2 * rs.super_stride, rs.bin_totals.p, rs.tile_order.p);
        ++launches;
        prof.mark("k_raster_init", st);
        if (world > 1 && rs.peer_root) { k_peer_release<<<1, 1, 0, st>>>(rs.peer_sync, rs.rctl.p, (uint32_t)(rs.frame_parity && rs.frame_half2)); ++launches; }
        const uint32_t count = rs.uploaded;
        if (rs.cov_format == GS_COV_F16) launch_project<true>(rs, count, st); else launch_project<false>(rs, count, st);
        ++launches;
        prof.mark("k_project", st);
        if (record_events) RCU(cudaEventRecord(ev_project, st));
    }
    if (!(phases & 2)) { tm.kernel_launches = launches; return GS_OK; }
    rs.snapshot_taken = false;
    const bool counting_sort = ncoarse <= (uint32_t)kBinTiles;
    if (p.render_count && local_tiles && counting_sort) {
        const OwnMask own = make_own_mask(rank, world);
        const int sharded = world > 1 ? 1 : 0;
        const uint32_t chunks = (p.render_count + kBinRanks - 1u) / kBinRanks;
        gs_launch(k_bin_count, chunks, kBinWarps * 32, 0, st, d_order, p.render_count, order_count_dev, rs.rects.p, coarse_x, ncoarse, rs.bin_hist.p, rs.bin_stride,
                  rs.bin_totals.p, rs.rect_by_rank.p, own, sharded);
        ++launches;
        prof.mark("k_bin_count", st);
        gs_launch(k_bin_scan, ncoarse, 1024, 0, st, rs.bin_hist.p, rs.bin_stride, (uint32_t)kBinRanks, p.render_count, order_count_dev, rs.bin_totals.p, ncoarse, rs.ranges.p, rs.rctl.p, rs.tile_order.p, rs.instance_capacity);
        ++launches;
        prof.mark("k_bin_scan", st);
        gs_launch(k_bin_place, chunks, kBinWarps * 32, 0, st, d_order, p.render_count, order_count_dev, rs.rect_by_rank.p, coarse_x, ncoarse, rs.bin_hist.p, rs.bin_stride,
                  rs.list.p, rs.instance_capacity, rs.rctl.p, own, sharded, (tiles_x <= 256 && tiles_y <= 256) ? 1 : 0);
        ++launches;
        prof.mark("k_bin_place", st);
    }
    if (p.render_count && local_tiles && !counting_sort) {
        const uint32_t chunks = (p.render_count + kBinTile - 1) / kBinTile;
        gs_launch(k_tile_count, chunks, kBinThreads, 0, st, d_order, p.render_count, order_count_dev, rs.rects.p, rs.block_sums.p, rs.warp_sums.p, rs.super_sums.p, make_own_mask(rank, world), world > 1 ? 1 : 0);
        ++launches;
        prof.mark("k_tile_count", st);
        gs_launch(k_tile_emit, chunks, kBinThreads, 0, st, d_order, p.render_count, order_count_dev, rs.rects.p, rs.block_sums.p, rs.warp_sums.p, rs.super_sums.p, coarse_x, rs.ikeys[0].p,
                                                    rs.ivals[0].p, rs.instance_capacity, rs.rctl.p, make_own_mask(rank, world), world > 1 ? 1 : 0);
        ++launches;
        prof.mark("k_tile_emit", st);
        static const RadixNames names = {{"k_radix_hist[tile,0]", "k_radix_hist[tile,1]", "k_radix_hist[tile,2]", "k_radix_hist[tile,3]"},
                                         {"k_radix_scan[tile,0]", "k_radix_scan[tile,1]", "k_radix_scan[tile,2]", "k_radix_scan[tile,3]"},
                                         {"k_radix_scatter[tile,0]", "k_radix_scatter[tile,1]", "k_radix_scatter[tile,2]", "k_radix_scatter[tile,3]"}};
        const unsigned long long *n_dev = &rs.rctl.p->total_instances;
        radix_sort_pairs<uint16_t, unsigned long long>(rs.ikeys[0].p, rs.ikeys[1].p, rs.ivals[0].p, 0u, kValArray, rs.ivals[1].p, rs.ivals[0].p, rs.list.p, 0u,
                                                       n_dev, rs.instance_capacity, pl, rs.sctl.p, rs.tile_hist.p, rs.hist_stride, false, rs.ranges.p, st, launches,
                                                       &prof, names);
    }
    if (record_events) RCU(cudaEventRecord(ev_bin, st));
    if (local_tiles) {
        const bool peer_mode = world > 1 && (rs.peer_root || rs.peer_attached);
        void *target = raster_frame_ptr(rs, p.frame_format);
        if (world > 1 && !peer_mode) RCU(cudaMemsetAsync(target, 0, (size_t)p.width * p.height * (p.frame_format == GS_FRAME_RGBA8 ? 4 : 16), st));
        if (peer_mode && rs.peer_attached) {
            k_peer_wait_release<<<1, 1, 0, st>>>(rs.peer_sync, rs.rctl.p);
            ++launches;
            target = rs.peer_frame;
        }
        const uint32_t grid = ncoarse * kFinePerCoarse;
        const bool to_peer = peer_mode && rs.peer_attached;
        const StatusSnapshot snap{rs.snap_sort_ctl, reinterpret_cast<const uint32_t *>(rs.rctl.p),
                                  (rs.snap_base && rs.snap_sort_ctl) ? rs.snap_base + (size_t)rs.frame_parity * rs.snap_stride : nullptr,
                                  to_peer ? &rs.rctl.p->peer_parity : nullptr, to_peer ? (unsigned long long)rs.frame.n : 0ull};
        rs.snapshot_taken = snap.dst != nullptr;
        const bool rgba8 = p.frame_format == GS_FRAME_RGBA8, tile16 = tshift == kTileShift;
        const auto blend = tile16 ? (rgba8 ? k_blend<GS_FRAME_RGBA8, 1> : k_blend<GS_FRAME_RGBA32F, 1>)
                                  : (rgba8 ? k_blend<GS_FRAME_RGBA8, 2> : k_blend<GS_FRAME_RGBA32F, 2>);
        gs_launch(blend, grid, tile16 ? 128 : 512, 0, st, rs.ranges.p, rs.list.p, rs.records.p, tiles_x, tiles_y, coarse_x, rank, world, (int)p.width, (int)p.height,
                  p.flip_y, target, rs.tile_order.p, snap);
        ++launches;
        prof.mark("k_blend", st);
        if (peer_mode && rs.peer_attached) { k_peer_signal<<<1, 1, 0, st>>>(rs.peer_sync); ++launches; }
        if (peer_mode && rs.peer_root) { k_peer_wait_arrived<<<1, 1, 0, st>>>(rs.peer_sync, rs.rctl.p, world - 1); ++launches; prof.mark("k_peer_wait_arrived", st); }
    }
    rs.last_format = p.frame_format;
    const size_t rows = p.height;
    rs.last_frame_bytes = rows * p.width * (p.frame_format == GS_FRAME_RGBA8 ? 4 : 16);
    tm.kernel_launches = launches;
    return GS_OK;
}

static int raster_subset(RasterState &rs, const gs_config &c, const uint32_t *d_indexes, uint32_t count, const int32_t *dist, uint32_t *sub_idx,
                         int32_t *sub_dist, cudaStream_t st, Profiler &prof, uint32_t &launches) {
    const uint32_t chunks = (count + kBinTile - 1) / kBinTile;
    const OwnMask own = make_own_mask(c.rank, c.world_size);
    gs_launch(k_subset_count, chunks, kBinThreads, 0, st, d_indexes, count, rs.rects.p, own, rs.block_sums.p, rs.warp_sums.p, rs.super_sums.p + rs.super_stride);
    ++launches;
    prof.mark("k_subset_count", st);
    gs_launch(k_subset_emit, chunks, kBinThreads, 0, st, d_indexes, count, rs.rects.p, own, rs.block_sums.p, rs.warp_sums.p, rs.super_sums.p + rs.super_stride, dist, sub_idx, sub_dist, rs.rctl.p);
    ++launches;
    prof.mark("k_subset_emit", st);
    return GS_OK;
}

static int raster_read_projected(RasterState &rs, gs_projected_splat *out, uint32_t count, cudaStream_t st) {
    if (count > rs.uploaded) { snprintf(raster_err(), 512, "count %u > uploaded %u", count, rs.uploaded); return GS_ERR_CAPACITY; }
    RCU(rs.exported.ensure(count));
    if (count) k_export_projected<<<(count + 255) / 256, 256, 0, st>>>(rs.records.p, rs.rects.p, count, rs.exported.p);
    RCU(cudaMemcpyAsync(out, rs.exported.p, (size_t)count * sizeof(gs_projected_splat), cudaMemcpyDeviceToHost, st));
    return GS_OK;
}

}
```

### gaussiansplats3d_b200/csrc/sort_kernels.cuh

```cuda
#pragma once
#include "common.cuh"

namespace gs {

enum DepthMode : int {
    kIntStatic = 0, kIntDynamic = 1, kIntPrecomputed = 2, kFloatStatic = 3, kFloatDynamic = 4, kFloatPrecomputed = 5
};

struct DepthParams {
    int32_t irow[4];
    float frow[4];
    float mvp[16];
};

__global__ void k_sort_init(SortControl *ctl) {
    pdl_enter();
    const uint32_t tid = threadIdx.x;
    if (tid == 0) {
        ctl->dmin = 2147483640;
        ctl->dmax = -2147483640;
        ctl->error = 0;
    }
    uint32_t *h = &ctl->hist[0][0];
    for (uint32_t i = tid; i < 4 * kRadix; i += blockDim.x) h[i] = 0;
}

__device__ __forceinline__ void scene_row(const float *mvp, const float *t, float out[4]) {
#pragma unroll
    for (int c = 0; c < 4; ++c) {
        float acc = __fmul_rn(mvp[2], t[4 * c + 0]);
        acc = __fadd_rn(acc, __fmul_rn(mvp[6], t[4 * c + 1]));
        acc = __fadd_rn(acc, __fmul_rn(mvp[10], t[4 * c + 2]));
        acc = __fadd_rn(acc, __fmul_rn(mvp[14], t[4 * c + 3]));
        out[c] = acc;
    }
}
__device__ __forceinline__ int32_t trunc_scaled(float f, double scale) { return __double2int_rz((double)f * scale); }

template <int MODE>
__device__ __forceinline__ int32_t splat_distance(uint32_t g, const void *__restrict__ centers, const void *__restrict__ pre,
                                                  const uint32_t *__restrict__ scene_idx, const DepthParams &P,
                                                  const int32_t (*s_irow)[4], const float (*s_frow)[4]) {
    if (MODE == kIntPrecomputed) return (int32_t)ld_nc_u32((const uint32_t *)pre + g);
    if (MODE == kFloatPrecomputed) return trunc_scaled(__uint_as_float(ld_nc_u32((const uint32_t *)pre + g)), 4096.0);
    const int4 c = ld_nc_v4((const int4 *)centers + g);
    if (MODE == kIntStatic) {
        return (int32_t)((uint32_t)P.irow[0] * (uint32_t)c.x + (uint32_t)P.irow[1] * (uint32_t)c.y + (uint32_t)P.irow[2] * (uint32_t)c.z);
    } else if (MODE == kIntDynamic) {
        const int32_t *r = s_irow[ld_nc_u32(scene_idx + g) & (GS_MAX_SCENES_DEV - 1)];
        return (int32_t)((uint32_t)r[0] * (uint32_t)c.x + (uint32_t)r[1] * (uint32_t)c.y + (uint32_t)r[2] * (uint32_t)c.z +
                         (uint32_t)r[3] * (uint32_t)c.w);
    } else if (MODE == kFloatStatic) {
        float acc = __fmul_rn(P.frow[0], __int_as_float(c.x));
        acc = __fadd_rn(acc, __fmul_rn(P.frow[1], __int_as_float(c.y)));
        acc = __fadd_rn(acc, __fmul_rn(P.frow[2], __int_as_float(c.z)));
        return trunc_scaled(acc, 4096.0);
    } else {
        const float *r = s_frow[ld_nc_u32(scene_idx + g) & (GS_MAX_SCENES_DEV - 1)];
        float acc = __fmul_rn(r[0], __int_as_float(c.x));
        acc = __fadd_rn(acc, __fmul_rn(r[1], __int_as_float(c.y)));
        acc = __fadd_rn(acc, __fmul_rn(r[2], __int_as_float(c.z)));
        acc = __fadd_rn(acc, __fmul_rn(r[3], __int_as_float(c.w)));
        return trunc_scaled(acc, 4096.0);
    }
}

constexpr int kDepthThreads = 256;
constexpr int kDepthItems = 4;

template <int MODE, bool IDENTITY>
__global__ void __launch_bounds__(kDepthThreads)
k_depth(const uint32_t *__restrict__ indexes, const void *__restrict__ centers, const void *__restrict__ pre,
        const uint32_t *__restrict__ scene_idx, const float *__restrict__ transforms, const DepthParams *__restrict__ Pp, uint32_t s0,
        uint32_t rc, int32_t *__restrict__ dist, SortControl *ctl) {
    pdl_enter();
    DepthParams P;
#pragma unroll
    for (int i = 0; i < 4; ++i) { P.irow[i] = __ldg(&Pp->irow[i]); P.frow[i] = __ldg(&Pp->frow[i]); }
    if (MODE == kIntDynamic || MODE == kFloatDynamic) {
#pragma unroll
        for (int i = 0; i < 16; ++i) P.mvp[i] = __ldg(&Pp->mvp[i]);
    }
    __shared__ int32_t s_irow[GS_MAX_SCENES_DEV][4];
    __shared__ float s_frow[GS_MAX_SCENES_DEV][4];
    __shared__ int s_min[kDepthThreads / 32], s_max[kDepthThreads / 32];
    if (MODE == kIntDynamic || MODE == kFloatDynamic) {
        if (threadIdx.x < GS_MAX_SCENES_DEV) {
            float row[4];
            scene_row(P.mvp, transforms + 16 * threadIdx.x, row);
#pragma unroll
            for (int k = 0; k < 4; ++k) {
                s_frow[threadIdx.x][k] = row[k];
                s_irow[threadIdx.x][k] = trunc_scaled(row[k], 1000.0);
            }
        }
        __syncthreads();
    }
    if (blockIdx.x == 0 && threadIdx.x == 0) ctl->error = 0;
    int32_t lmin = 2147483640, lmax = -2147483640;
    const uint32_t tile = kDepthThreads * kDepthItems;
    for (uint64_t base = (uint64_t)s0 + (uint64_t)blockIdx.x * tile; base < rc; base += (uint64_t)gridDim.x * tile) {
        uint32_t g[kDepthItems];
#pragma unroll
        for (int k = 0; k < kDepthItems; ++k) {
            const uint64_t i = base + (uint64_t)k * kDepthThreads + threadIdx.x;
            g[k] = (i < rc) ? (IDENTITY ? (uint32_t)i : ld_nc_u32(indexes + i)) : 0xffffffffu;
        }
        int32_t d[kDepthItems];
#pragma unroll
        for (int k = 0; k < kDepthItems; ++k)
            if (g[k] != 0xffffffffu) d[k] = splat_distance<MODE>(g[k], centers, pre, scene_idx, P, s_irow, s_frow);
#pragma unroll
        for (int k = 0; k < kDepthItems; ++k) {
            const uint64_t i = base + (uint64_t)k * kDepthThreads + threadIdx.x;
            if (i < rc) {
                dist[i] = d[k];
                lmin = min(lmin, d[k]);
                lmax = max(lmax, d[k]);
            }
        }
    }
    lmin = warp_min(lmin);
    lmax = warp_max(lmax);
    if ((threadIdx.x & 31) == 0) { s_min[threadIdx.x >> 5] = lmin; s_max[threadIdx.x >> 5] = lmax; }
    __syncthreads();
    if (threadIdx.x < 32) {
        lmin = threadIdx.x < kDepthThreads / 32 ? s_min[threadIdx.x] : 2147483640;
        lmax = threadIdx.x < kDepthThreads / 32 ? s_max[threadIdx.x] : -2147483640;
        lmin = warp_min(lmin);
        lmax = warp_max(lmax);
        if (threadIdx.x == 0) {
            atomicMin(&ctl->dmin, lmin);
            atomicMax(&ctl->dmax, lmax);
        }
    }
}

struct PassPlan {
    int npasses;
    int shift[4];
    int bits[4];
};

constexpr int kRadixThreads = 512;
constexpr int kRadixItems = 8;
constexpr int kRadixTile = kRadixThreads * kRadixItems;
constexpr int kRadixWarps = kRadixThreads / 32;

enum ValMode : int { kValArray = 0, kValArrayReversed = 1, kValIotaReversed = 2 };

template <int NB>
__device__ __forceinline__ uint32_t warp_peers(uint32_t d) {
    uint32_t peers = 0xffffffffu;
#pragma unroll
    for (int b = 0; b < NB; ++b) {
        const bool bit = (d >> b) & 1u;
        const uint32_t vote = __ballot_sync(0xffffffffu, bit);
        peers &= bit ? vote : ~vote;
    }
    return peers;
}

template <typename KeyT>
__global__ void __launch_bounds__(kRadixThreads)
k_bucket(int32_t *__restrict__ dist , KeyT *__restrict__ keys, uint32_t n_host,
         const unsigned long long *__restrict__ n_dev, uint32_t R, PassPlan plan, int write_buckets, SortControl *ctl,
         uint32_t *__restrict__ tile_hist, uint32_t stride) {
    pdl_enter();
    __shared__ uint32_t s_hist[kRadix];
    if (threadIdx.x < kRadix) s_hist[threadIdx.x] = 0;
    __syncthreads();
    const int32_t dmin = ctl->dmin, dmax = ctl->dmax;
    const float span = __fsub_rn(__int2float_rn(dmax), __int2float_rn(dmin));
    const float range_map = __fdiv_rn(__uint2float_rn(R - 1u), span);
    const bool degenerate = (dmax == dmin);
    uint32_t err = 0;
    const uint32_t n = n_dev ? (uint32_t)*n_dev : n_host;
    const uint64_t jbase = (uint64_t)blockIdx.x * kRadixTile;
    int32_t d[kRadixItems];
#pragma unroll
    for (int k = 0; k < kRadixItems; ++k) {
        const uint64_t j = jbase + (uint64_t)k * kRadixThreads + threadIdx.x;
        d[k] = (j < n) ? dist[(uint64_t)n - 1u - j] : 0;
    }
#pragma unroll
    for (int k = 0; k < kRadixItems; ++k) {
        const uint64_t j = jbase + (uint64_t)k * kRadixThreads + threadIdx.x;
        if (j < n) {
            const int32_t rel = (int32_t)((uint32_t)d[k] - (uint32_t)dmin);
            int32_t b = __float2int_rz(__fmul_rn(__int2float_rn(rel), range_map));
            if (degenerate) b = 0;
            if (rel < 0 || b < 0) { err |= kErrBucketRange; b = 0; }
            else if ((uint32_t)b >= R) b = (int32_t)(R - 1u);
            if (write_buckets) dist[(uint64_t)n - 1u - j] = b;
            const uint32_t key = (R - 1u) - (uint32_t)b;
            keys[j] = (KeyT)key;
            atomicAdd(&s_hist[(key >> plan.shift[0]) & ((1u << plan.bits[0]) - 1u)], 1u);
        }
    }
    __syncthreads();
    if (threadIdx.x < kRadix) {
        const uint32_t v = s_hist[threadIdx.x];
        tile_hist[(size_t)threadIdx.x * stride + blockIdx.x] = v;
        if (v) atomicAdd(&ctl->hist[0][threadIdx.x], v);
    }
    if (err) atomicOr(&ctl->error, err);
    if (degenerate && blockIdx.x == 0 && threadIdx.x == 0) atomicOr(&ctl->error, kErrDegenerate);
}

template <typename KeyT>
__global__ void __launch_bounds__(kRadixThreads)
k_radix_hist(const KeyT *__restrict__ keys, uint32_t n_host, const unsigned long long *__restrict__ n_dev, unsigned long long n_cap,
             int shift, int bits, uint32_t *__restrict__ tile_hist, uint32_t stride, uint32_t *global_hist, int add_global) {
    pdl_enter();
    const uint32_t n = n_dev ? (uint32_t)min(*n_dev, n_cap) : n_host;
    const uint64_t base = (uint64_t)blockIdx.x * kRadixTile;
    if (base >= n) return;
    __shared__ uint32_t s_hist[kRadix];
    if (threadIdx.x < kRadix) s_hist[threadIdx.x] = 0;
    __syncthreads();
    const uint32_t dmask = (1u << bits) - 1u;
    uint32_t kk[kRadixItems];
#pragma unroll
    for (int k = 0; k < kRadixItems; ++k) {
        const uint64_t e = base + (uint64_t)k * kRadixThreads + threadIdx.x;
        kk[k] = (e < n) ? (((uint32_t)keys[e] >> shift) & dmask) : 0xffffffffu;
    }
#pragma unroll
    for (int k = 0; k < kRadixItems; ++k)
        if (kk[k] != 0xffffffffu) atomicAdd(&s_hist[kk[k]], 1u);
    __syncthreads();
    if (threadIdx.x < kRadix) {
        const uint32_t v = s_hist[threadIdx.x];
        tile_hist[(size_t)threadIdx.x * stride + blockIdx.x] = v;
        if (add_global && v) atomicAdd(global_hist + threadIdx.x, v);
    }
}

constexpr int kScanColThreads = 1024;
__global__ void __launch_bounds__(kScanColThreads)
k_radix_scan(uint32_t *__restrict__ tile_hist, uint32_t stride, uint32_t n_host, const unsigned long long *__restrict__ n_dev,
             unsigned long long n_cap, const uint32_t *__restrict__ global_hist) {
    pdl_enter();
    __shared__ uint32_t s_scan[40];
    __shared__ uint32_t s_carry;
    const uint32_t n = n_dev ? (uint32_t)min(*n_dev, n_cap) : n_host;
    const uint32_t ntiles = (uint32_t)(((uint64_t)n + kRadixTile - 1) / kRadixTile);
    const uint32_t d = blockIdx.x;
    {
        uint32_t total;
        const uint32_t c = (threadIdx.x < kRadix && threadIdx.x < d) ? global_hist[threadIdx.x] : 0u;
        (void)block_exclusive_scan<kScanColThreads>(c, s_scan, total);
        if (threadIdx.x == 0) s_carry = total;
    }
    __syncthreads();
    uint32_t *col = tile_hist + (size_t)d * stride;
    for (uint32_t base = 0; base < ntiles; base += kScanColThreads) {
        const uint32_t t = base + threadIdx.x;
        const uint32_t v = t < ntiles ? col[t] : 0u;
        uint32_t total;
        const uint32_t ex = block_exclusive_scan<kScanColThreads>(v, s_scan, total);
        const uint32_t carry = s_carry;
        if (t < ntiles) col[t] = ex + carry;
        __syncthreads();
        if (threadIdx.x == 0) s_carry = carry + total;
        __syncthreads();
    }
}

template <typename KeyT, typename ValT, int VALMODE, bool WRITE_KEYS, bool RANGES, bool FULL>
__device__ __forceinline__ void radix_scatter_tile(const KeyT *__restrict__ keys_in, const ValT *__restrict__ vals_in, uint32_t iota_top,
                                                   KeyT *__restrict__ keys_out, ValT *__restrict__ vals_out, uint32_t n, uint32_t tile,
                                                   int shift, uint32_t dmask, const uint32_t *__restrict__ tile_offsets, uint32_t stride,
                                                   uint2 *ranges, unsigned char *s_raw, uint32_t *s_tile_count, uint32_t *s_tile_start,
                                                   uint32_t *s_gbase, uint32_t *s_scan) {
    uint32_t(*s_whist)[kRadix + 1] = reinterpret_cast<uint32_t(*)[kRadix + 1]>(s_raw);
    ValT *s_vals = reinterpret_cast<ValT *>(s_raw);
    KeyT *s_keys = reinterpret_cast<KeyT *>(s_raw + (size_t)kRadixTile * sizeof(ValT));
    const int tid = threadIdx.x, lane = tid & 31, warp = tid >> 5;
    const uint32_t tile_base = tile * (uint32_t)kRadixTile;
    const uint32_t run_base = tile_base + (uint32_t)warp * (32 * kRadixItems) + lane;
    for (int i = tid; i < kRadixWarps * (kRadix + 1); i += kRadixThreads) (&s_whist[0][0])[i] = 0;

    uint32_t key[kRadixItems];
#pragma unroll
    for (int k = 0; k < kRadixItems; ++k) {
        const uint32_t e = run_base + (uint32_t)k * 32;
        key[k] = (FULL || e < n) ? (uint32_t)keys_in[e] : 0xffffffffu;
    }
    const uint32_t my_offset = tid < kRadix ? tile_offsets[(size_t)tid * stride + tile] : 0u;
    uint32_t peers[kRadixItems];
#pragma unroll
    for (int k = 0; k < kRadixItems; ++k) {
        const uint32_t d = (FULL || key[k] != 0xffffffffu) ? ((key[k] >> shift) & dmask) : (uint32_t)kRadix;
        peers[k] = warp_peers<FULL ? 8 : 9>(d);
    }
    __syncthreads();
    uint32_t rank[kRadixItems];
    const uint32_t lt = lanemask_lt();
#pragma unroll
    for (int k = 0; k < kRadixItems; ++k) {
        const uint32_t d = (FULL || key[k] != 0xffffffffu) ? ((key[k] >> shift) & dmask) : (uint32_t)kRadix;
        const uint32_t before = s_whist[warp][d];
        rank[k] = before + __popc(peers[k] & lt);
        __syncwarp();
        if ((peers[k] & lt) == 0) s_whist[warp][d] = before + __popc(peers[k]);
        __syncwarp();
    }
    __syncthreads();
    if (tid < kRadix) {
        uint32_t run = 0;
#pragma unroll
        for (int w = 0; w < kRadixWarps; ++w) {
            const uint32_t c = s_whist[w][tid];
            s_whist[w][tid] = run;
            run += c;
        }
        s_tile_count[tid] = run;
    }
    __syncthreads();
    {
        uint32_t total;
        const uint32_t c = tid < kRadix ? s_tile_count[tid] : 0u;
        const uint32_t ex = block_exclusive_scan<kRadixThreads>(c, s_scan, total);
        if (tid < kRadix) { s_tile_start[tid] = ex; s_gbase[tid] = my_offset - ex; }
    }
    __syncthreads();
#pragma unroll
    for (int k = 0; k < kRadixItems; ++k) {
        const uint32_t d = (key[k] >> shift) & dmask;
        rank[k] = (FULL || key[k] != 0xffffffffu) ? (s_tile_start[d] + s_whist[warp][d] + rank[k]) : 0xffffffffu;
    }
    __syncthreads();
#pragma unroll
    for (int k = 0; k < kRadixItems; ++k) {
        const uint32_t e = run_base + (uint32_t)k * 32;
        if (FULL || rank[k] != 0xffffffffu) {
            ValT v;
            if (VALMODE == kValArray) v = __ldg(vals_in + e);
            else if (VALMODE == kValArrayReversed) v = __ldg(vals_in + (n - 1u - e));
            else v = (ValT)(iota_top - e);
            s_vals[rank[k]] = v;
            s_keys[rank[k]] = (KeyT)key[k];
        }
    }
    __syncthreads();
    const uint32_t valid = FULL ? (uint32_t)kRadixTile : (n - tile_base);
#pragma unroll
    for (int k = 0; k < kRadixItems; ++k) {
        const uint32_t q = (uint32_t)k * kRadixThreads + tid;
        if (FULL || q < valid) {
            const KeyT kk = s_keys[q];
            const uint32_t d = ((uint32_t)kk >> shift) & dmask;
            const uint32_t dst = s_gbase[d] + q;
            vals_out[dst] = s_vals[q];
            if (WRITE_KEYS) keys_out[dst] = kk;
            if (RANGES) {
                if (q == 0 || s_keys[q - 1] != kk) atomicMin(&ranges[(uint32_t)kk].x, dst);
                if (q + 1 == valid || s_keys[q + 1] != kk) atomicMax(&ranges[(uint32_t)kk].y, dst + 1u);
            }
        }
    }
}

template <typename KeyT, typename ValT, int VALMODE, bool WRITE_KEYS, bool RANGES>
__global__ void __launch_bounds__(kRadixThreads, 2)
k_radix_scatter(const KeyT *__restrict__ keys_in, const ValT *__restrict__ vals_in, uint32_t iota_top,
                KeyT *__restrict__ keys_out, ValT *__restrict__ vals_out, uint32_t n_host,
                const unsigned long long *__restrict__ n_dev, unsigned long long n_cap, int shift, int bits,
                const uint32_t *__restrict__ tile_offsets, uint32_t stride, uint2 *ranges, uint32_t *clear_hist, SortControl *reset_ctl) {
    pdl_enter();
    const uint32_t n = n_dev ? (uint32_t)min(*n_dev, n_cap) : n_host;
    const uint32_t tile = blockIdx.x;
    if (tile == 0) {
        if (clear_hist && threadIdx.x < kRadix) clear_hist[threadIdx.x] = 0;
        if (reset_ctl && threadIdx.x == 0) { reset_ctl->dmin = 2147483640; reset_ctl->dmax = -2147483640; }
    }
    const uint64_t tile_base = (uint64_t)tile * kRadixTile;
    if (tile_base >= n) return;
    __shared__ __align__(16) unsigned char s_raw[kRadixTile * (sizeof(KeyT) + sizeof(ValT)) > kRadixWarps * (kRadix + 1) * 4
                                                     ? kRadixTile * (sizeof(KeyT) + sizeof(ValT))
                                                     : kRadixWarps * (kRadix + 1) * 4];
    __shared__ uint32_t s_tile_count[kRadix];
    __shared__ uint32_t s_tile_start[kRadix];
    __shared__ uint32_t s_gbase[kRadix];
    __shared__ uint32_t s_scan[40];
    const uint32_t dmask = (1u << bits) - 1u;
    if (tile_base + kRadixTile <= n)
        radix_scatter_tile<KeyT, ValT, VALMODE, WRITE_KEYS, RANGES, true>(keys_in, vals_in, iota_top, keys_out, vals_out, n, tile, shift, dmask, tile_offsets, stride,
                                                                          ranges, s_raw, s_tile_count, s_tile_start, s_gbase, s_scan);
    else
        radix_scatter_tile<KeyT, ValT, VALMODE, WRITE_KEYS, RANGES, false>(keys_in, vals_in, iota_top, keys_out, vals_out, n, tile, shift, dmask, tile_offsets, stride,
                                                                           ranges, s_raw, s_tile_count, s_tile_start, s_gbase, s_scan);
}

__global__ void k_copy_head(const uint32_t *__restrict__ indexes, uint32_t *__restrict__ out, uint32_t s0) {
    pdl_enter();
    for (uint64_t i = (uint64_t)blockIdx.x * blockDim.x + threadIdx.x; i < s0; i += (uint64_t)gridDim.x * blockDim.x)
        out[i] = indexes ? indexes[i] : (uint32_t)i;
}

__global__ void k_bucket_counts(const int32_t *__restrict__ buckets, uint32_t s0, uint32_t rc, uint32_t *counts) {
    for (uint64_t i = (uint64_t)s0 + (uint64_t)blockIdx.x * blockDim.x + threadIdx.x; i < rc; i += (uint64_t)gridDim.x * blockDim.x)
        atomicAdd(&counts[buckets[i]], 1u);
}
__global__ void __launch_bounds__(1024) k_exclusive_scan_single_block(uint32_t *data, uint32_t n) {
    __shared__ uint32_t s_scan[40];
    __shared__ uint32_t s_carry;
    if (threadIdx.x == 0) s_carry = 0;
    __syncthreads();
    for (uint32_t base = 0; base < n; base += 1024) {
        const uint32_t i = base + threadIdx.x;
        const uint32_t v = i < n ? data[i] : 0u;
        uint32_t total;
        const uint32_t ex = block_exclusive_scan<1024>(v, s_scan, total);
        const uint32_t carry = s_carry;
        if (i < n) data[i] = ex + carry;
        __syncthreads();
        if (threadIdx.x == 0) s_carry = carry + total;
        __syncthreads();
    }
}

template <bool INTEGER, bool DYNAMIC>
__global__ void k_distances_splat_order(const void *__restrict__ centers, const uint32_t *__restrict__ scene_idx,
                                        const int32_t *__restrict__ irows , const float *__restrict__ frows,
                                        uint32_t count, void *__restrict__ out) {
    for (uint64_t i = (uint64_t)blockIdx.x * blockDim.x + threadIdx.x; i < count; i += (uint64_t)gridDim.x * blockDim.x) {
        const int4 c = ld_nc_v4((const int4 *)centers + i);
        const uint32_t sc = DYNAMIC ? (scene_idx[i] & (GS_MAX_SCENES_DEV - 1)) : 0u;
        if (INTEGER) {
            const int32_t *r = irows + 4 * sc;
            uint32_t d = (uint32_t)c.x * (uint32_t)r[0] + (uint32_t)c.y * (uint32_t)r[1] + (uint32_t)c.z * (uint32_t)r[2];
            if (DYNAMIC) d += (uint32_t)r[3] * (uint32_t)c.w;
            ((int32_t *)out)[i] = (int32_t)d;
        } else {
            const float *r = frows + 4 * sc;
            float acc = __fmul_rn(__int_as_float(c.x), r[0]);
            acc = __fadd_rn(acc, __fmul_rn(__int_as_float(c.y), r[1]));
            acc = __fadd_rn(acc, __fmul_rn(__int_as_float(c.z), r[2]));
            if (DYNAMIC) acc = __fadd_rn(acc, r[3]);
            ((float *)out)[i] = acc;
        }
    }
}


static inline PassPlan make_plan_bits(int key_bits) {
    PassPlan pl{};
    int np = (key_bits + kRadixBits - 1) / kRadixBits;
    if (np < 1) np = 1;
    pl.npasses = np;
    int done = 0;
    for (int p = 0; p < np; ++p) {
        const int left = key_bits - done, b = (left + (np - p) - 1) / (np - p);
        pl.shift[p] = done;
        pl.bits[p] = b < 1 ? 1 : b;
        done += b;
    }
    return pl;
}

template <typename KeyT, typename ValT>
static void launch_radix_scatter(uint32_t grid, bool first, bool write_keys, bool want_ranges, int valmode, const KeyT *kin, const ValT *vin,
                                 uint32_t iota_top, KeyT *kout, ValT *vout, uint32_t n, const unsigned long long *n_dev, unsigned long long n_cap,
                                 int shift, int bits, const uint32_t *tile_offsets, uint32_t stride, uint2 *ranges, uint32_t *clear_hist, SortControl *reset_ctl,
                                 cudaStream_t st) {
#define GS_PASS(VM, WK, RG) gs_launch(k_radix_scatter<KeyT, ValT, VM, WK, RG>, grid, kRadixThreads, 0, st, kin, vin, iota_top, kout, vout, n, n_dev, n_cap, shift, bits, tile_offsets, stride, ranges, clear_hist, reset_ctl)
    if (!first) valmode = kValArray;
    if (want_ranges && !write_keys) { GS_PASS(kValArray, false, true); }
    else if (want_ranges) {
        if (valmode == kValArray) GS_PASS(kValArray, true, true);
        else if (valmode == kValArrayReversed) GS_PASS(kValArrayReversed, true, true);
        else GS_PASS(kValIotaReversed, true, true);
    }
    else if (valmode == kValArray) { if (!write_keys) GS_PASS(kValArray, false, false); else GS_PASS(kValArray, true, false); }
    else if (valmode == kValArrayReversed) { if (!write_keys) GS_PASS(kValArrayReversed, false, false); else GS_PASS(kValArrayReversed, true, false); }
    else { if (!write_keys) GS_PASS(kValIotaReversed, false, false); else GS_PASS(kValIotaReversed, true, false); }
#undef GS_PASS
}

struct RadixNames { const char *hist[4], *scan[4], *scatter[4]; };

template <typename KeyT, typename ValT>
static void radix_sort_pairs(KeyT *keys0, KeyT *keys1, const ValT *vals_src, uint32_t iota_top, int first_valmode, ValT *vtmp0,
                             ValT *vtmp1, ValT *vals_final, uint32_t n, const unsigned long long *n_dev, unsigned long long n_cap,
                             const PassPlan &pl, SortControl *ctl, uint32_t *tile_hist, uint32_t stride, bool hist0_done, uint2 *ranges,
                             cudaStream_t st, uint32_t &launches, Profiler *prof, const RadixNames &names, bool self_clean = false,
                             bool keep_final_keys = false ,
                             KeyT **final_keys = nullptr) {
    const unsigned long long n_grid = n_dev ? n_cap : n;
    const uint32_t tiles = (uint32_t)((n_grid + kRadixTile - 1) / kRadixTile);
    if (!tiles) return;
    KeyT *kin = keys0, *kout = keys1;
    const ValT *vin = vals_src;
    ValT *vt[2] = {vtmp0, vtmp1};
    for (int p = 0; p < pl.npasses; ++p) {
        const bool last = (p == pl.npasses - 1);
        ValT *vout = last ? vals_final : vt[p & 1];
        uint32_t *th = tile_hist + (size_t)p * kRadix * stride;
        if (!(p == 0 && hist0_done)) {
            gs_launch(k_radix_hist<KeyT>, tiles, kRadixThreads, 0, st, kin, n, n_dev, n_cap, pl.shift[p], pl.bits[p], th, stride, &ctl->hist[p][0], 1);
            ++launches;
            if (prof) prof->mark(names.hist[p], st);
        }
        gs_launch(k_radix_scan, 1u << pl.bits[p], kScanColThreads, 0, st, th, stride, n, n_dev, n_cap, &ctl->hist[p][0]);
        ++launches;
        if (prof) prof->mark(names.scan[p], st);
        if (last && final_keys) *final_keys = kout;
        launch_radix_scatter<KeyT, ValT>(tiles, p == 0, !last || keep_final_keys, last && ranges != nullptr, first_valmode, kin, vin, iota_top, kout, vout, n, n_dev, n_cap,
                                   pl.shift[p], pl.bits[p], th, stride, ranges, self_clean ? &ctl->hist[p][0] : nullptr,
                                   (self_clean && last) ? ctl : nullptr, st);
        ++launches;
        if (prof) prof->mark(names.scatter[p], st);
        vin = vout;
        KeyT *t = kin; kin = kout; kout = t;
    }
}
static inline size_t radix_tile_hist_words(unsigned long long n, int npasses, uint32_t *stride_out) {
    const size_t tiles = (size_t)((n + kRadixTile - 1) / kRadixTile);
    const size_t stride = (tiles + 31) & ~(size_t)31;
    if (stride_out) *stride_out = (uint32_t)stride;
    return stride * kRadix * (size_t)npasses;
}

}
```

Baseline: 3262.

## Fold radix scan into scatter via hierarchical prefix rows, drop scan kernels

Removes the separate k_radix_scan launch per radix pass. Per-tile digit counts now go into a PrefixRows layout with superblock rows, and the scatter kernel derives its tile offsets from these rows plus the global histogram itself. Super-row scratch is cleared in the depth kernel, or by a new clear kernel on the ray and generate paths, replacing the per-pass histogram clearing inside scatter. This trades one launch and one global round-trip per pass for extra prefix work inside the scatter, which may wait on predecessor tiles or do redundant lookback. The binning kernels are reworked to use the same row layout.

```diff
diff --git a/gaussiansplats3d_b200/csrc/engine.cu b/gaussiansplats3d_b200/csrc/engine.cu
--- a/gaussiansplats3d_b200/csrc/engine.cu
+++ b/gaussiansplats3d_b200/csrc/engine.cu
@@ -314,9 +314,10 @@
 
 template <int MODE>
 static void launch_depth(bool identity, int blocks, cudaStream_t st, const uint32_t *idx, const void *centers, const void *pre,
-                         const uint32_t *scene, const float *tr, const DepthParams *P, uint32_t s0, uint32_t rc, int32_t *dist, SortControl *ctl) {
-    if (identity) gs_launch(k_depth<MODE, true>, blocks, kDepthThreads, 0, st, idx, centers, pre, scene, tr, P, s0, rc, dist, ctl);
-    else gs_launch(k_depth<MODE, false>, blocks, kDepthThreads, 0, st, idx, centers, pre, scene, tr, P, s0, rc, dist, ctl);
+                         const uint32_t *scene, const float *tr, const DepthParams *P, uint32_t s0, uint32_t rc, int32_t *dist, SortControl *ctl,
+                         uint32_t *super_rows, uint32_t super_words) {
+    if (identity) gs_launch(k_depth<MODE, true>, blocks, kDepthThreads, 0, st, idx, centers, pre, scene, tr, P, s0, rc, dist, ctl, super_rows, super_words);
+    else gs_launch(k_depth<MODE, false>, blocks, kDepthThreads, 0, st, idx, centers, pre, scene, tr, P, s0, rc, dist, ctl, super_rows, super_words);
 }
 
 static int enqueue_depth(gs_engine *e, const uint32_t *d_indexes, const float *mvp, bool use_pre, uint32_t lo, uint32_t hi, bool capturing) {
@@ -336,13 +337,16 @@
     const int dblocks = (int)std::max<uint64_t>(1, std::min<uint64_t>(((uint64_t)n + kDepthThreads * kDepthItems - 1) / (kDepthThreads * kDepthItems), (uint64_t)e->sm_count * 8));
     const bool identity = (d_indexes == nullptr);
     const void *pre = e->precomputed.p;
+    const RadixLayout L = radix_layout(n, make_plan_bits(e->key_bits).npasses);
+    uint32_t *sup = L.super_base(e->tile_hist.p);
+    const uint32_t sw = (uint32_t)L.super_words();
     switch (mode) {
-        case kIntStatic: launch_depth<kIntStatic>(identity, dblocks, st, d_indexes, e->centers.p, pre, e->scene_idx.p, e->transforms.p, e->depthp.p + e->rs.frame_parity, lo, hi, e->dist.p, e->ctl.p); break;
-        case kIntDynamic: launch_depth<kIntDynamic>(identity, dblocks, st, d_indexes, e->centers.p, pre, e->scene_idx.p, e->transforms.p, e->depthp.p + e->rs.frame_parity, lo, hi, e->dist.p, e->ctl.p); break;
-        case kIntPrecomputed: launch_depth<kIntPrecomputed>(identity, dblocks, st, d_indexes, e->centers.p, pre, e->scene_idx.p, e->transforms.p, e->depthp.p + e->rs.frame_parity, lo, hi, e->dist.p, e->ctl.p); break;
-        case kFloatStatic: launch_depth<kFloatStatic>(identity, dblocks, st, d_indexes, e->centers.p, pre, e->scene_idx.p, e->transforms.p, e->depthp.p + e->rs.frame_parity, lo, hi, e->dist.p, e->ctl.p); break;
-        case kFloatDynamic: launch_depth<kFloatDynamic>(identity, dblocks, st, d_indexes, e->centers.p, pre, e->scene_idx.p, e->transforms.p, e->depthp.p + e->rs.frame_parity, lo, hi, e->dist.p, e->ctl.p); break;
-        default: launch_depth<kFloatPrecomputed>(identity, dblocks, st, d_indexes, e->centers.p, pre, e->scene_idx.p, e->transforms.p, e->depthp.p + e->rs.frame_parity, lo, hi, e->dist.p, e->ctl.p); break;
+        case kIntStatic: launch_depth<kIntStatic>(identity, dblocks, st, d_indexes, e->centers.p, pre, e->scene_idx.p, e->transforms.p, e->depthp.p + e->rs.frame_parity, lo, hi, e->dist.p, e->ctl.p, sup, sw); break;
+        case kIntDynamic: launch_depth<kIntDynamic>(identity, dblocks, st, d_indexes, e->centers.p, pre, e->scene_idx.p, e->transforms.p, e->depthp.p + e->rs.frame_parity, lo, hi, e->dist.p, e->ctl.p, sup, sw); break;
+        case kIntPrecomputed: launch_depth<kIntPrecomputed>(identity, dblocks, st, d_indexes, e->centers.p, pre, e->scene_idx.p, e->transforms.p, e->depthp.p + e->rs.frame_parity, lo, hi, e->dist.p, e->ctl.p, sup, sw); break;
+        case kFloatStatic: launch_depth<kFloatStatic>(identity, dblocks, st, d_indexes, e->centers.p, pre, e->scene_idx.p, e->transforms.p, e->depthp.p + e->rs.frame_parity, lo, hi, e->dist.p, e->ctl.p, sup, sw); break;
+        case kFloatDynamic: launch_depth<kFloatDynamic>(identity, dblocks, st, d_indexes, e->centers.p, pre, e->scene_idx.p, e->transforms.p, e->depthp.p + e->rs.frame_parity, lo, hi, e->dist.p, e->ctl.p, sup, sw); break;
+        default: launch_depth<kFloatPrecomputed>(identity, dblocks, st, d_indexes, e->centers.p, pre, e->scene_idx.p, e->transforms.p, e->depthp.p + e->rs.frame_parity, lo, hi, e->dist.p, e->ctl.p, sup, sw); break;
     }
     return GS_OK;
 }
@@ -355,9 +359,9 @@
     const uint32_t s0 = render_count - sort_count, n = sort_count;
     const PassPlan pl = make_plan_bits(e->key_bits);
     uint32_t launches = 0;
-    uint32_t stride = 0;
-    int rc = e->tile_hist.ensure(radix_tile_hist_words(std::max(n, 1u), pl.npasses, &stride));
-    if (rc) return rc;
+    int rc = e->tile_hist.ensure(radix_tile_hist_words(std::max(n, 1u), pl.npasses));
+    if (rc) return rc;
+    const RadixLayout L = radix_layout(n, pl.npasses);
     if (!capturing) CU(cudaEventRecord(e->ev[EV_SORT0], st));
     if (!e->have_prof_begin) e->prof.begin(st);
     if (e->ctl_dirty && !capturing) {
@@ -387,22 +391,21 @@
             n_dev = &e->rs.rctl.p->subset_count;
         }
         static const RadixNames names = {{"k_radix_hist[depth,0]", "k_radix_hist[depth,1]", "k_radix_hist[depth,2]", "k_radix_hist[depth,3]"},
-                                         {"k_radix_scan[depth,0]", "k_radix_scan[depth,1]", "k_radix_scan[depth,2]", "k_radix_scan[depth,3]"},
                                          {"k_radix_scatter[depth,0]", "k_radix_scatter[depth,1]", "k_radix_scatter[depth,2]", "k_radix_scatter[depth,3]"}};
         if (e->key_bits <= 16) {
-            gs_launch(k_bucket<uint16_t>, tiles, kRadixThreads, 0, st, dist_sorted, (uint16_t *)e->keys[0].p, n, n_dev, R, pl, write_buckets ? 1 : 0, e->ctl.p, e->tile_hist.p, stride);
+            gs_launch(k_bucket<uint16_t>, tiles, kRadixThreads, 0, st, dist_sorted, (uint16_t *)e->keys[0].p, n, n_dev, R, pl, write_buckets ? 1 : 0, e->ctl.p, L.pass(e->tile_hist.p, 0));
             ++launches;
             e->prof.mark("k_bucket", st);
             if (!capturing) CU(cudaEventRecord(e->ev[EV_BUCKET], st));
             radix_sort_pairs<uint16_t, uint32_t>((uint16_t *)e->keys[0].p, (uint16_t *)e->keys[1].p, vsrc, render_count - 1u, vmode, e->vals[0].p, e->vals[1].p,
-                                       e->sorted.p + s0, n, n_dev, (unsigned long long)n, pl, e->ctl.p, e->tile_hist.p, stride, true, nullptr, st, launches, &e->prof, names, true);
+                                       e->sorted.p + s0, n, n_dev, (unsigned long long)n, pl, e->ctl.p, e->tile_hist.p, true, nullptr, st, launches, &e->prof, names, true);
         } else {
-            gs_launch(k_bucket<uint32_t>, tiles, kRadixThreads, 0, st, dist_sorted, e->keys[0].p, n, n_dev, R, pl, write_buckets ? 1 : 0, e->ctl.p, e->tile_hist.p, stride);
+            gs_launch(k_bucket<uint32_t>, tiles, kRadixThreads, 0, st, dist_sorted, e->keys[0].p, n, n_dev, R, pl, write_buckets ? 1 : 0, e->ctl.p, L.pass(e->tile_hist.p, 0));
             ++launches;
             e->prof.mark("k_bucket", st);
             if (!capturing) CU(cudaEventRecord(e->ev[EV_BUCKET], st));
             radix_sort_pairs<uint32_t, uint32_t>(e->keys[0].p, e->keys[1].p, vsrc, render_count - 1u, vmode, e->vals[0].p, e->vals[1].p, e->sorted.p + s0, n,
-                                       n_dev, (unsigned long long)n, pl, e->ctl.p, e->tile_hist.p, stride, true, nullptr, st, launches, &e->prof, names, true);
+                                       n_dev, (unsigned long long)n, pl, e->ctl.p, e->tile_hist.p, true, nullptr, st, launches, &e->prof, names, true);
         }
     } else if (!capturing) {
         CU(cudaEventRecord(e->ev[EV_DEPTH], st));
@@ -492,7 +495,7 @@
         (rc = e->shard.local_sorted.ensure(e->cfg.max_splat_count)))
         return rc;
     const PassPlan pl = make_plan_bits(e->key_bits);
-    if ((rc = e->tile_hist.ensure(radix_tile_hist_words(std::max(e->cfg.max_splat_count, 1u), pl.npasses, nullptr))) || (rc = e->precomputed.ensure(e->cfg.max_splat_count))) return rc;
+    if ((rc = e->tile_hist.ensure(radix_tile_hist_words(std::max(e->cfg.max_splat_count, 1u), pl.npasses))) || (rc = e->precomputed.ensure(e->cfg.max_splat_count))) return rc;
     return GS_OK;
 }
 template <typename F> static inline void preload_kernel(F f) { cudaFuncAttributes a; (void)cudaFuncGetAttributes(&a, f); }
@@ -509,7 +512,7 @@
 }
 template <int MODE> static void shard_preload_depth() { preload_kernel(k_depth<MODE, true>); preload_kernel(k_depth<MODE, false>); }
 static void shard_preload(gs_engine *e) {
-    preload_kernel(k_sort_init); preload_kernel(k_copy_head); preload_kernel(k_radix_scan);
+    preload_kernel(k_sort_init); preload_kernel(k_copy_head);
     preload_kernel(k_shard_exchange_minmax); preload_kernel(k_shard_exchange_runs); preload_kernel(k_shard_totals); preload_kernel(k_shard_delta); preload_kernel(k_shard_done);
     shard_preload_depth<kIntStatic>(); shard_preload_depth<kIntDynamic>(); shard_preload_depth<kIntPrecomputed>();
     shard_preload_depth<kFloatStatic>(); shard_preload_depth<kFloatDynamic>(); shard_preload_depth<kFloatPrecomputed>();
@@ -594,24 +597,23 @@
     cudaStream_t st = e->stream;
     const uint32_t n = hi - lo, R = e->cfg.distance_map_range;
     const PassPlan pl = make_plan_bits(e->key_bits);
-    uint32_t stride = 0;
-    int rc = e->tile_hist.ensure(radix_tile_hist_words(std::max(n, 1u), pl.npasses, &stride));
-    if (rc) return rc;
+    int rc = e->tile_hist.ensure(radix_tile_hist_words(std::max(n, 1u), pl.npasses));
+    if (rc) return rc;
+    const RadixLayout L = radix_layout(n, pl.npasses);
     const bool identity = (d_indexes == nullptr);
     static const RadixNames names = {{"k_radix_hist[shard,0]", "k_radix_hist[shard,1]", "k_radix_hist[shard,2]", "k_radix_hist[shard,3]"},
-                                     {"k_radix_scan[shard,0]", "k_radix_scan[shard,1]", "k_radix_scan[shard,2]", "k_radix_scan[shard,3]"},
                                      {"k_radix_scatter[shard,0]", "k_radix_scatter[shard,1]", "k_radix_scatter[shard,2]", "k_radix_scatter[shard,3]"}};
     const uint32_t me = e->cfg.rank, world = e->shard.world, seq = e->shard.seq;
     uint2 *runs = (uint2 *)shard_runs(e->shard.block.p);
     KeyT *final_keys = nullptr;
     if (n) {
         const uint32_t tiles = (n + kRadixTile - 1) / kRadixTile;
-        gs_launch(k_bucket<KeyT>, tiles, kRadixThreads, 0, st, e->dist.p + lo, (KeyT *)e->keys[0].p, n, nullptr, R, pl, 0, e->ctl.p, e->tile_hist.p, stride);
+        gs_launch(k_bucket<KeyT>, tiles, kRadixThreads, 0, st, e->dist.p + lo, (KeyT *)e->keys[0].p, n, nullptr, R, pl, 0, e->ctl.p, L.pass(e->tile_hist.p, 0));
         ++launches;
         e->prof.mark("k_bucket", st);
         radix_sort_pairs<KeyT, uint32_t>((KeyT *)e->keys[0].p, (KeyT *)e->keys[1].p, identity ? nullptr : d_indexes + lo, hi - 1u,
                                          identity ? kValIotaReversed : kValArrayReversed, e->vals[0].p, e->vals[1].p, e->shard.local_sorted.p, n, nullptr,
-                                         (unsigned long long)n, pl, e->ctl.p, e->tile_hist.p, stride, true, runs, st, launches, &e->prof, names, true, true, &final_keys);
+                                         (unsigned long long)n, pl, e->ctl.p, e->tile_hist.p, true, runs, st, launches, &e->prof, names, true, true, &final_keys);
     }
     k_shard_exchange_runs<<<1, 32, 0, st>>>(e->shard.peers, me, world, seq);
     ++launches;
@@ -982,9 +984,8 @@
         unsigned long long *gkey = e->rs.frame_parity ? e->graph_key_alt : e->graph_key;
         if (!gexec || memcmp(key, gkey, sizeof(key)) != 0) {
             if (gexec) { cudaGraphExecDestroy(gexec); gexec = nullptr; }
-            uint32_t stride = 0;
             const PassPlan pl = make_plan_bits(e->key_bits);
-            if ((rc = e->tile_hist.ensure(radix_tile_hist_words(std::max(q.sort_count, 1u), pl.npasses, &stride)))) return rc;
+            if ((rc = e->tile_hist.ensure(radix_tile_hist_words(std::max(q.sort_count, 1u), pl.npasses)))) return rc;
             CU(cudaStreamBeginCapture(st, cudaStreamCaptureModeThreadLocal));
             struct CaptureGuard {
                 cudaStream_t st; bool armed;
@@ -1293,17 +1294,16 @@
     if (!k) { e->tm.kernel_launches = launches; return GS_OK; }
     const uint32_t *perm = nullptr;
     if (total > 1) {
-        uint32_t stride = 0;
         int pos_bits = 1;
         while (pos_bits < 32 && (1ull << pos_bits) < (unsigned long long)t.splats) ++pos_bits;
         if ((rc = R.keys[0].ensure(n)) || (rc = R.keys[1].ensure(n)) || (rc = R.vals[0].ensure(n)) || (rc = R.vals[1].ensure(n)) || (rc = R.vals[2].ensure(n)) ||
-            (rc = R.vals[3].ensure(n)) || (rc = R.tile_hist.ensure(radix_tile_hist_words(total, 4, &stride))))
+            (rc = R.vals[3].ensure(n)) || (rc = R.tile_hist.ensure(radix_tile_hist_words(total, 4))))
             return rc;
         if (!R.ctl.p) {
             if ((rc = R.ctl.ensure(1))) return rc;
             CU(cudaMemsetAsync(R.ctl.p, 0, sizeof(SortControl), st));
         }
-        static const RadixNames names{{"ray_hist0", "ray_hist1", "ray_hist2", "ray_hist3"}, {"ray_scan0", "ray_scan1", "ray_scan2", "ray_scan3"},
+        static const RadixNames names{{"ray_hist0", "ray_hist1", "ray_hist2", "ray_hist3"},
                                       {"ray_scatter0", "ray_scatter1", "ray_scatter2", "ray_scatter3"}};
         uint32_t *order = nullptr;
         for (int which = 0; which < 4; ++which) {
@@ -1311,8 +1311,9 @@
             uint32_t *dst = R.vals[2 + (which & 1)].p;
             k_ray_keys<<<(total + 255) / 256, 256, 0, st>>>(R.hits.p, order, total, which, R.keys[0].p, R.vals[0].p);
             ++launches;
+            radix_clear_rows(R.ctl.p, R.tile_hist.p, radix_layout(total, pl.npasses), st, launches);
             radix_sort_pairs<uint32_t, uint32_t>(R.keys[0].p, R.keys[1].p, R.vals[0].p, 0, kValArray, R.vals[1].p, R.vals[0].p, dst, total, nullptr, 0, pl,
-                                                 R.ctl.p, R.tile_hist.p, stride, false, nullptr, st, launches, nullptr, names, true);
+                                                 R.ctl.p, R.tile_hist.p, false, nullptr, st, launches, nullptr, names, true);
             order = dst;
         }
         perm = order;
@@ -1665,15 +1666,14 @@
     ScopedBuf<SortControl> ctl;
     int run(const unsigned long long *key, const uint32_t *order, uint32_t n, int bits, uint32_t *out, cudaStream_t st, uint32_t &launches) {
         int rc;
-        uint32_t stride = 0;
         if ((rc = keys[0].ensure(n)) || (rc = keys[1].ensure(n)) || (rc = vals[0].ensure(n)) || (rc = vals[1].ensure(n)) || (rc = vals[2].ensure(n)) ||
-            (rc = tile_hist.ensure(radix_tile_hist_words(std::max(n, 1u), 3, &stride))))
+            (rc = tile_hist.ensure(radix_tile_hist_words(std::max(n, 1u), 3))))
             return rc;
         if (!ctl.p) {
             if ((rc = ctl.ensure(1))) return rc;
             CU(cudaMemsetAsync(ctl.p, 0, sizeof(SortControl), st));
         }
-        static const RadixNames names{{"gen_hist0", "gen_hist1", "gen_hist2", "gen_hist3"}, {"gen_scan0", "gen_scan1", "gen_scan2", "gen_scan3"},
+        static const RadixNames names{{"gen_hist0", "gen_hist1", "gen_hist2", "gen_hist3"},
                                       {"gen_scatter0", "gen_scatter1", "gen_scatter2", "gen_scatter3"}};
         if (n == 0) return GS_OK;
         const int rounds = std::max(1, (bits + 23) / 24);
@@ -1682,8 +1682,9 @@
             uint32_t *dst = (r == rounds - 1) ? out : vals[2].p;
             k_gen_sort_piece<<<(n + 255) / 256, 256, 0, st>>>(key, order, n, 24 * r, keys[0].p, vals[0].p);
             ++launches;
+            radix_clear_rows(ctl.p, tile_hist.p, radix_layout(n, pl.npasses), st, launches);
             radix_sort_pairs<uint32_t, uint32_t>(keys[0].p, keys[1].p, vals[0].p, 0, kValArray, vals[1].p, vals[0].p, dst, n, nullptr, 0, pl,
-                                                 ctl.p, tile_hist.p, stride, false, nullptr, st, launches, nullptr, names, true);
+                                                 ctl.p, tile_hist.p, false, nullptr, st, launches, nullptr, names, true);
             order = dst;
         }
         return GS_OK;
diff --git a/gaussiansplats3d_b200/csrc/raster_kernels.cuh b/gaussiansplats3d_b200/csrc/raster_kernels.cuh
--- a/gaussiansplats3d_b200/csrc/raster_kernels.cuh
+++ b/gaussiansplats3d_b200/csrc/raster_kernels.cuh
@@ -600,8 +600,8 @@
 
 __global__ void __launch_bounds__(kBinWarps * 32)
 k_bin_count(const uint32_t *__restrict__ order, uint32_t render_count_host, const unsigned long long *__restrict__ n_dev, const ushort4 *__restrict__ rects,
-            int coarse_x, uint32_t nt, uint32_t *__restrict__ hist, uint32_t stride, uint32_t *__restrict__ totals, ushort4 *__restrict__ rect_by_rank,
-            OwnMask own, int sharded) {
+            int coarse_x, uint32_t nt, PrefixRows chunk_rows, uint32_t *__restrict__ totals,
+            ushort4 *__restrict__ rect_by_rank, OwnMask own, int sharded) {
     pdl_enter();
     constexpr int W = kBinWarps, ITEMS = kBinRankItems, NT = kBinTiles;
     const uint32_t n = n_dev ? (uint32_t)*n_dev : render_count_host;
@@ -636,67 +636,55 @@
     __syncthreads();
     for (uint32_t t = threadIdx.x; t < nt; t += W * 32) {
         const uint32_t v = s_hist[t];
-        hist[(size_t)t * stride + blockIdx.x] = v;
+        prefix_publish(chunk_rows, blockIdx.x, t, v);
         if (v) atomicAdd(&totals[t], v);
-    }
-}
-
-__global__ void __launch_bounds__(1024)
-k_bin_scan(uint32_t *__restrict__ hist, uint32_t stride, uint32_t ranks_per_chunk, uint32_t render_count_host, const unsigned long long *__restrict__ n_dev,
-           const uint32_t *__restrict__ totals, uint32_t nt, uint2 *__restrict__ ranges, RasterControl *rctl, uint32_t *__restrict__ tile_order,
-           unsigned long long capacity) {
-    pdl_enter();
-    __shared__ uint32_t s_scan[40];
-    __shared__ uint32_t s_carry;
-    {
-        const uint32_t mine = totals[blockIdx.x];
-        bool ahead = false;
-        if (threadIdx.x < nt) { const uint32_t o = totals[threadIdx.x]; ahead = o > mine || (o == mine && threadIdx.x < blockIdx.x); }
-        const int rank = __syncthreads_count(ahead);
-        if (threadIdx.x == 0) tile_order[rank] = blockIdx.x;
-    }
-    const uint32_t n = n_dev ? (uint32_t)*n_dev : render_count_host;
-    const uint32_t nchunks = (uint32_t)(((uint64_t)n + ranks_per_chunk - 1) / ranks_per_chunk);
-    const uint32_t d = blockIdx.x;
-    {
-        uint32_t total;
-        const uint32_t c = threadIdx.x < d ? totals[threadIdx.x] : 0u;
-        (void)block_exclusive_scan<1024>(c, s_scan, total);
-        if (threadIdx.x == 0) {
-            s_carry = total;
-            const uint32_t mine = totals[d];
-            const unsigned long long lo = total, hi = lo + mine;
-            ranges[d] = make_uint2((uint32_t)min(lo, capacity), (uint32_t)min(hi, capacity));
-            if (d == nt - 1) rctl->total_instances = hi;
-        }
-    }
-    __syncthreads();
-    uint32_t *col = hist + (size_t)d * stride;
-    for (uint32_t b = 0; b < nchunks; b += 1024) {
-        const uint32_t t = b + threadIdx.x;
-        const uint32_t v = t < nchunks ? col[t] : 0u;
-        uint32_t total;
-        const uint32_t ex = block_exclusive_scan<1024>(v, s_scan, total);
-        const uint32_t carry = s_carry;
-        if (t < nchunks) col[t] = ex + carry;
-        __syncthreads();
-        if (threadIdx.x == 0) s_carry = carry + total;
-        __syncthreads();
     }
 }
 
 __global__ void __launch_bounds__(kBinWarps * 32)
 k_bin_place(const uint32_t *__restrict__ order, uint32_t render_count_host, const unsigned long long *__restrict__ n_dev, const ushort4 *__restrict__ rect_by_rank,
-            int coarse_x, uint32_t nt, const uint32_t *__restrict__ offsets, uint32_t stride, unsigned long long *__restrict__ list, unsigned long long capacity,
-            RasterControl *rctl, OwnMask own, int sharded, int pack_ok) {
+            int coarse_x, uint32_t nt, PrefixRows chunk_rows, const uint32_t *__restrict__ totals, uint2 *__restrict__ ranges, uint32_t *__restrict__ tile_order,
+            unsigned long long *__restrict__ list, unsigned long long capacity, RasterControl *rctl, OwnMask own, int sharded, int pack_ok) {
     pdl_enter();
     constexpr int W = kBinWarps, ITEMS = kBinRankItems, NT = kBinTiles;
+    static_assert(W * 32 == 2 * NT && NT == 256, "prefix_before and the tile schedule below take 512 threads over 256 tiles");
     const uint32_t n = n_dev ? (uint32_t)*n_dev : render_count_host;
     const uint32_t base = blockIdx.x * (uint32_t)(W * 32 * ITEMS);
-    if (base >= n) return;
     __shared__ uint32_t s_pre[W][NT];
     __shared__ __align__(8) uint32_t s_mask[W][NT];
     static_assert(NT * 4 >= 32 * ITEMS * 8, "the mask row of a warp doubles as the staging buffer of its compacted items");
+    __shared__ uint32_t s_first[NT];
+    __shared__ uint32_t s_scan[40];
+    const uint32_t tid = threadIdx.x, tt = tid % NT, half = tid / NT;
+    const uint32_t tot = tt < nt ? totals[tt] : 0u;
+    uint32_t list_base;
+    {
+        uint32_t total;
+        list_base = block_exclusive_scan<W * 32>(half == 0 ? tot : 0u, s_scan, total);
+    }
+    if (blockIdx.x == 0) {
+        if (half == 0 && tt < nt) {
+            const unsigned long long lo = list_base, hi = lo + tot;
+            ranges[tt] = make_uint2((uint32_t)min(lo, capacity), (uint32_t)min(hi, capacity));
+            if (tt == nt - 1) rctl->total_instances = hi;
+        }
+        uint32_t *s_tot = s_pre[0], *s_rank = s_pre[1];
+        if (half == 0) { s_tot[tt] = tot; s_rank[tt] = 0; }
+        __syncthreads();
+        if (tt < nt) {
+            uint32_t ahead = 0;
+            for (uint32_t o = half; o < nt; o += 2) { const uint32_t v = s_tot[o]; ahead += (v > tot || (v == tot && o < tt)) ? 1u : 0u; }
+            atomicAdd(&s_rank[tt], ahead);
+        }
+        __syncthreads();
+        if (half == 0 && tt < nt) tile_order[s_rank[tt]] = tt;
+        __syncthreads();
+    }
+    if (base >= n) return;
+    {
+        const uint32_t before = prefix_before(chunk_rows, blockIdx.x, &s_pre[0][0]);
+        if (half == 0) s_first[tt] = list_base + before;
+    }
     for (uint32_t i = threadIdx.x; i < (uint32_t)(W * NT); i += W * 32) (&s_pre[0][0])[i] = 0;
     __syncthreads();
     const int lane = threadIdx.x & 31, warp = threadIdx.x >> 5;
@@ -747,7 +735,7 @@
             round_instances(sid[k] != 0xffffffffu, sid[k], rc[k], coarse_x, own, sharded != 0, [&](int, uint32_t, int t, uint32_t) { atomicAdd(&my_pre[t], 1u); });
     __syncthreads();
     for (uint32_t t = threadIdx.x; t < nt; t += W * 32) {
-        uint32_t at = offsets[(size_t)t * stride + blockIdx.x];
+        uint32_t at = s_first[t];
 #pragma unroll
         for (int w = 0; w < W; ++w) {
             const uint32_t c = s_pre[w][t];
@@ -842,7 +830,8 @@
     }
 }
 
-__global__ void k_raster_init(RasterControl *rctl, SortControl *ctl, uint2 *ranges, uint32_t ntiles, uint32_t *super_sums, uint32_t nsuper, uint32_t *bin_totals, uint32_t *tile_order) {
+__global__ void k_raster_init(RasterControl *rctl, SortControl *ctl, uint2 *ranges, uint32_t ntiles, uint32_t *super_sums, uint32_t nsuper, uint32_t *bin_totals,
+                              uint32_t *tile_order, uint32_t *radix_super, uint32_t radix_super_words) {
     pdl_enter();
     const size_t tid = (size_t)blockIdx.x * blockDim.x + threadIdx.x;
     const size_t stride = (size_t)gridDim.x * blockDim.x;
@@ -851,8 +840,7 @@
         rctl->frame_seq += 1;
         ctl->error = 0;
     }
-    uint32_t *h = &ctl->hist[0][0];
-    for (size_t i = tid; i < 4 * kRadix; i += stride) h[i] = 0;
+    radix_clear(ctl, radix_super, radix_super_words, tid, stride);
     for (size_t i = tid; i < ntiles; i += stride) ranges[i] = make_uint2(0xffffffffu, 0u);
     for (size_t i = tid; i < (size_t)kVisibleSlots * 8; i += stride) rctl->visible_slots[i] = 0;
     for (size_t i = tid; i < nsuper; i += stride) super_sums[i] = 0;
@@ -1113,7 +1101,7 @@
     RBuf<ushort4> rect_by_rank;
     RBuf<uint32_t> tile_order;
     RBuf<uint32_t> bin_totals;
-    uint32_t bin_stride = 0;
+    uint32_t bin_super_off = 0;
     RBuf<DynamicUniforms> dyn;
     RBuf<ProjParams> projp;
     RBuf<unsigned char> frame;
@@ -1131,7 +1119,6 @@
     void *peer_frame = nullptr;
     bool peer_root = false, peer_attached = false;
     unsigned long long instance_capacity = 0;
-    uint32_t hist_stride = 0;
     int sm_count = 132;
     int last_format = GS_FRAME_RGBA32F;
     size_t last_frame_bytes = 0;
@@ -1172,7 +1159,8 @@
         RCU(rs.block_sums.ensure((n + kBinTile - 1) / kBinTile + 1));
         RCU(rs.warp_sums.ensure(((n + kBinTile - 1) / kBinTile + 1) * (kBinThreads / 32)));
         rs.super_stride = (uint32_t)(((n + kBinTile - 1) / kBinTile) / kBinThreads + 2);
-        RCU(rs.super_sums.ensure(2 * (size_t)rs.super_stride));
+        rs.bin_super_off = (2 * rs.super_stride + 3u) & ~3u;
+        RCU(rs.super_sums.ensure(rs.bin_super_off + ((n + kBinRanks - 1) / kBinRanks + 2) * (size_t)kBinTiles));
         const char *f = getenv("GS_INSTANCE_FACTOR");
         const double factor = f ? atof(f) : 4.0;
         const size_t tiles = (size_t)((c.max_width + kTile - 1) / kTile) * ((c.max_height + kTile - 1) / kTile);
@@ -1184,13 +1172,11 @@
         RCU(rs.frame.ensure((size_t)c.max_width * (c.max_height + kTile) * 16));
         if (frame_coarse_tiles(c.max_width, c.max_height) > (uint32_t)kBinTiles) {
             for (int i = 0; i < 2; ++i) { RCU(rs.ikeys[i].ensure(rs.instance_capacity)); RCU(rs.ivals[i].ensure(rs.instance_capacity)); }
-            RCU(rs.tile_hist.ensure(radix_tile_hist_words(rs.instance_capacity, 2, &rs.hist_stride)));
+            RCU(rs.tile_hist.ensure(radix_tile_hist_words(rs.instance_capacity, 2)));
         }
         {
-            const size_t coarse = (size_t)((c.max_width + kTile * kCoarseW - 1) / (kTile * kCoarseW)) * ((c.max_height + kTile * kCoarseH - 1) / (kTile * kCoarseH));
             const size_t chunks = (n + kBinRanks - 1) / kBinRanks + 1;
-            rs.bin_stride = (uint32_t)((chunks + 31) & ~(size_t)31);
-            RCU(rs.bin_hist.ensure(std::max<size_t>(coarse, 1) * rs.bin_stride));
+            RCU(rs.bin_hist.ensure(chunks * kBinTiles));
             RCU(rs.rect_by_rank.ensure(n));
             RCU(rs.bin_totals.ensure(kBinTiles));
             RCU(cudaMemset(rs.bin_totals.p, 0, kBinTiles * 4));
@@ -1305,8 +1291,14 @@
     int tile_bits = 1;
     while ((1u << tile_bits) < std::max(ncoarse, 2u)) ++tile_bits;
     const PassPlan pl = make_plan_bits(tile_bits);
+    const bool counting_sort = ncoarse <= (uint32_t)kBinTiles;
+    const PrefixLayout bin_layout = prefix_layout((p.render_count + kBinRanks - 1u) / kBinRanks);
+    const PrefixRows bin_rows = prefix_rows(bin_layout, rs.bin_hist.p, rs.super_sums.p + rs.bin_super_off);
     if (phases & 1) {
-        gs_launch(k_raster_init, 8, 256, 0, st, rs.rctl.p, rs.sctl.p, rs.ranges.p, ncoarse, rs.super_sums.p, 2 * rs.super_stride, rs.bin_totals.p, rs.tile_order.p);
+        const uint32_t bin_acc = counting_sort ? (uint32_t)bin_layout.acc_words() : 0u;
+        const RadixLayout L = radix_layout(counting_sort ? 0ull : rs.instance_capacity, pl.npasses);
+        gs_launch(k_raster_init, 8, 256, 0, st, rs.rctl.p, rs.sctl.p, rs.ranges.p, ncoarse, rs.super_sums.p, rs.bin_super_off + bin_acc, rs.bin_totals.p,
+                  rs.tile_order.p, L.super_base(rs.tile_hist.p), (uint32_t)L.super_words());
         ++launches;
         prof.mark("k_raster_init", st);
         if (world > 1 && rs.peer_root) { k_peer_release<<<1, 1, 0, st>>>(rs.peer_sync, rs.rctl.p, (uint32_t)(rs.frame_parity && rs.frame_half2)); ++launches; }
@@ -1318,20 +1310,17 @@
     }
     if (!(phases & 2)) { tm.kernel_launches = launches; return GS_OK; }
     rs.snapshot_taken = false;
-    const bool counting_sort = ncoarse <= (uint32_t)kBinTiles;
     if (p.render_count && local_tiles && counting_sort) {
         const OwnMask own = make_own_mask(rank, world);
         const int sharded = world > 1 ? 1 : 0;
-        const uint32_t chunks = (p.render_count + kBinRanks - 1u) / kBinRanks;
-        gs_launch(k_bin_count, chunks, kBinWarps * 32, 0, st, d_order, p.render_count, order_count_dev, rs.rects.p, coarse_x, ncoarse, rs.bin_hist.p, rs.bin_stride,
+        const uint32_t chunks = bin_layout.items;
+        gs_launch(k_bin_count, chunks, kBinWarps * 32, 0, st, d_order, p.render_count, order_count_dev, rs.rects.p, coarse_x, ncoarse, bin_rows,
                   rs.bin_totals.p, rs.rect_by_rank.p, own, sharded);
         ++launches;
         prof.mark("k_bin_count", st);
-        gs_launch(k_bin_scan, ncoarse, 1024, 0, st, rs.bin_hist.p, rs.bin_stride, (uint32_t)kBinRanks, p.render_count, order_count_dev, rs.bin_totals.p, ncoarse, rs.ranges.p, rs.rctl.p, rs.tile_order.p, rs.instance_capacity);
-        ++launches;
-        prof.mark("k_bin_scan", st);
-        gs_launch(k_bin_place, chunks, kBinWarps * 32, 0, st, d_order, p.render_count, order_count_dev, rs.rect_by_rank.p, coarse_x, ncoarse, rs.bin_hist.p, rs.bin_stride,
-                  rs.list.p, rs.instance_capacity, rs.rctl.p, own, sharded, (tiles_x <= 256 && tiles_y <= 256) ? 1 : 0);
+        gs_launch(k_bin_place, chunks, kBinWarps * 32, 0, st, d_order, p.render_count, order_count_dev, rs.rect_by_rank.p, coarse_x, ncoarse, bin_rows,
+                  rs.bin_totals.p, rs.ranges.p, rs.tile_order.p, rs.list.p, rs.instance_capacity, rs.rctl.p, own, sharded,
+                  (tiles_x <= 256 && tiles_y <= 256) ? 1 : 0);
         ++launches;
         prof.mark("k_bin_place", st);
     }
@@ -1345,11 +1334,10 @@
         ++launches;
         prof.mark("k_tile_emit", st);
         static const RadixNames names = {{"k_radix_hist[tile,0]", "k_radix_hist[tile,1]", "k_radix_hist[tile,2]", "k_radix_hist[tile,3]"},
-                                         {"k_radix_scan[tile,0]", "k_radix_scan[tile,1]", "k_radix_scan[tile,2]", "k_radix_scan[tile,3]"},
                                          {"k_radix_scatter[tile,0]", "k_radix_scatter[tile,1]", "k_radix_scatter[tile,2]", "k_radix_scatter[tile,3]"}};
         const unsigned long long *n_dev = &rs.rctl.p->total_instances;
         radix_sort_pairs<uint16_t, unsigned long long>(rs.ikeys[0].p, rs.ikeys[1].p, rs.ivals[0].p, 0u, kValArray, rs.ivals[1].p, rs.ivals[0].p, rs.list.p, 0u,
-                                                       n_dev, rs.instance_capacity, pl, rs.sctl.p, rs.tile_hist.p, rs.hist_stride, false, rs.ranges.p, st, launches,
+                                                       n_dev, rs.instance_capacity, pl, rs.sctl.p, rs.tile_hist.p, false, rs.ranges.p, st, launches,
                                                        &prof, names);
     }
     if (record_events) RCU(cudaEventRecord(ev_bin, st));
diff --git a/gaussiansplats3d_b200/csrc/sort_kernels.cuh b/gaussiansplats3d_b200/csrc/sort_kernels.cuh
--- a/gaussiansplats3d_b200/csrc/sort_kernels.cuh
+++ b/gaussiansplats3d_b200/csrc/sort_kernels.cuh
@@ -12,6 +12,86 @@
     float frow[4];
     float mvp[16];
 };
+
+struct PrefixLayout {
+    uint32_t items = 0, group = 1, mids = 0, tops = 0;
+    size_t acc_words() const { return ((size_t)mids + tops) * 256; }
+};
+static inline PrefixLayout prefix_layout(uint64_t items) {
+    PrefixLayout L;
+    L.items = (uint32_t)items;
+    while (2ull * L.group * L.group * L.group < items) L.group <<= 1;
+    L.mids = (L.items + L.group - 1) / L.group;
+    L.tops = (L.mids + L.group - 1) / L.group;
+    return L;
+}
+struct PrefixRows {
+    uint32_t *rows, *mids, *tops;
+    uint32_t group;
+};
+static inline PrefixRows prefix_rows(const PrefixLayout &L, uint32_t *rows, uint32_t *acc) {
+    return PrefixRows{rows, acc, acc + (size_t)L.mids * 256, L.group};
+}
+__device__ __forceinline__ void prefix_publish(const PrefixRows &P, uint32_t t, uint32_t c, uint32_t v) {
+    P.rows[(size_t)t * 256 + c] = v;
+    if (v) {
+        atomicAdd(&P.mids[(size_t)(t / P.group) * 256 + c], v);
+        atomicAdd(&P.tops[(size_t)(t / P.group / P.group) * 256 + c], v);
+    }
+}
+__device__ __forceinline__ const uint32_t *prefix_row(const PrefixRows &P, uint32_t i, uint32_t na, uint32_t nb, uint32_t top, uint32_t m) {
+    const uint32_t *base = i < na ? P.tops : (i < nb ? P.mids : P.rows);
+    const uint32_t r = i < na ? i : (i < nb ? top * P.group + (i - na) : m * P.group + (i - nb));
+    return base + (size_t)r * 256;
+}
+__device__ __forceinline__ uint32_t prefix_before(const PrefixRows &P, uint32_t t, uint32_t *s_red) {
+    const uint32_t tid = threadIdx.x, slot = tid >> 6, c4 = (tid & 63) * 4;
+    const uint32_t m = t / P.group, top = m / P.group;
+    const uint32_t na = top, nb = na + (m - top * P.group), nall = nb + (t - m * P.group);
+    uint4 v[4];
+#pragma unroll
+    for (int k = 0; k < 4; ++k) {
+        const uint32_t i = slot + 8u * k;
+        v[k] = i < nall ? *reinterpret_cast<const uint4 *>(prefix_row(P, i, na, nb, top, m) + c4) : make_uint4(0u, 0u, 0u, 0u);
+    }
+    uint4 acc = v[0];
+#pragma unroll
+    for (int k = 1; k < 4; ++k) { acc.x += v[k].x; acc.y += v[k].y; acc.z += v[k].z; acc.w += v[k].w; }
+    for (uint32_t i = slot + 32u; i < nall; i += 8) {
+        const uint4 w = *reinterpret_cast<const uint4 *>(prefix_row(P, i, na, nb, top, m) + c4);
+        acc.x += w.x; acc.y += w.y; acc.z += w.z; acc.w += w.w;
+    }
+    *reinterpret_cast<uint4 *>(s_red + slot * 256 + c4) = acc;
+    __syncthreads();
+    uint32_t sum = 0;
+    if (tid < 256) {
+#pragma unroll
+        for (int k = 0; k < 8; ++k) sum += s_red[k * 256 + tid];
+    }
+    __syncthreads();
+    return sum;
+}
+
+struct RadixLayout {
+    PrefixLayout P;
+    int npasses = 0;
+    size_t row_words() const { return (size_t)npasses * P.items * kRadix; }
+    size_t super_words() const { return (size_t)npasses * P.acc_words(); }
+    uint32_t *super_base(uint32_t *scratch) const { return scratch + row_words(); }
+    PrefixRows pass(uint32_t *scratch, int p) const {
+        return prefix_rows(P, scratch + (size_t)p * P.items * kRadix, super_base(scratch) + (size_t)p * P.acc_words());
+    }
+};
+
+__device__ __forceinline__ void radix_clear(SortControl *ctl, uint32_t *super_rows, uint32_t super_words, size_t tid, size_t nthreads) {
+    uint32_t *h = &ctl->hist[0][0];
+    for (size_t i = tid; i < 4 * kRadix; i += nthreads) h[i] = 0;
+    for (size_t i = tid; i < super_words; i += nthreads) super_rows[i] = 0;
+}
+__global__ void k_radix_clear(SortControl *ctl, uint32_t *super_rows, uint32_t super_words) {
+    pdl_enter();
+    radix_clear(ctl, super_rows, super_words, (size_t)blockIdx.x * blockDim.x + threadIdx.x, (size_t)gridDim.x * blockDim.x);
+}
 
 __global__ void k_sort_init(SortControl *ctl) {
     pdl_enter();
@@ -72,8 +152,9 @@
 __global__ void __launch_bounds__(kDepthThreads)
 k_depth(const uint32_t *__restrict__ indexes, const void *__restrict__ centers, const void *__restrict__ pre,
         const uint32_t *__restrict__ scene_idx, const float *__restrict__ transforms, const DepthParams *__restrict__ Pp, uint32_t s0,
-        uint32_t rc, int32_t *__restrict__ dist, SortControl *ctl) {
-    pdl_enter();
+        uint32_t rc, int32_t *__restrict__ dist, SortControl *ctl, uint32_t *__restrict__ super_rows, uint32_t super_words) {
+    pdl_enter();
+    radix_clear(ctl, super_rows, super_words, (size_t)blockIdx.x * blockDim.x + threadIdx.x, (size_t)gridDim.x * blockDim.x);
     DepthParams P;
 #pragma unroll
     for (int i = 0; i < 4; ++i) { P.irow[i] = __ldg(&Pp->irow[i]); P.frow[i] = __ldg(&Pp->frow[i]); }
@@ -165,7 +246,7 @@
 __global__ void __launch_bounds__(kRadixThreads)
 k_bucket(int32_t *__restrict__ dist , KeyT *__restrict__ keys, uint32_t n_host,
          const unsigned long long *__restrict__ n_dev, uint32_t R, PassPlan plan, int write_buckets, SortControl *ctl,
-         uint32_t *__restrict__ tile_hist, uint32_t stride) {
+         PrefixRows tile_rows) {
     pdl_enter();
     __shared__ uint32_t s_hist[kRadix];
     if (threadIdx.x < kRadix) s_hist[threadIdx.x] = 0;
@@ -201,7 +282,7 @@
     __syncthreads();
     if (threadIdx.x < kRadix) {
         const uint32_t v = s_hist[threadIdx.x];
-        tile_hist[(size_t)threadIdx.x * stride + blockIdx.x] = v;
+        prefix_publish(tile_rows, blockIdx.x, threadIdx.x, v);
         if (v) atomicAdd(&ctl->hist[0][threadIdx.x], v);
     }
     if (err) atomicOr(&ctl->error, err);
@@ -211,7 +292,7 @@
 template <typename KeyT>
 __global__ void __launch_bounds__(kRadixThreads)
 k_radix_hist(const KeyT *__restrict__ keys, uint32_t n_host, const unsigned long long *__restrict__ n_dev, unsigned long long n_cap,
-             int shift, int bits, uint32_t *__restrict__ tile_hist, uint32_t stride, uint32_t *global_hist, int add_global) {
+             int shift, int bits, PrefixRows tile_rows, uint32_t *global_hist) {
     pdl_enter();
     const uint32_t n = n_dev ? (uint32_t)min(*n_dev, n_cap) : n_host;
     const uint64_t base = (uint64_t)blockIdx.x * kRadixTile;
@@ -232,46 +313,15 @@
     __syncthreads();
     if (threadIdx.x < kRadix) {
         const uint32_t v = s_hist[threadIdx.x];
-        tile_hist[(size_t)threadIdx.x * stride + blockIdx.x] = v;
-        if (add_global && v) atomicAdd(global_hist + threadIdx.x, v);
-    }
-}
-
-constexpr int kScanColThreads = 1024;
-__global__ void __launch_bounds__(kScanColThreads)
-k_radix_scan(uint32_t *__restrict__ tile_hist, uint32_t stride, uint32_t n_host, const unsigned long long *__restrict__ n_dev,
-             unsigned long long n_cap, const uint32_t *__restrict__ global_hist) {
-    pdl_enter();
-    __shared__ uint32_t s_scan[40];
-    __shared__ uint32_t s_carry;
-    const uint32_t n = n_dev ? (uint32_t)min(*n_dev, n_cap) : n_host;
-    const uint32_t ntiles = (uint32_t)(((uint64_t)n + kRadixTile - 1) / kRadixTile);
-    const uint32_t d = blockIdx.x;
-    {
-        uint32_t total;
-        const uint32_t c = (threadIdx.x < kRadix && threadIdx.x < d) ? global_hist[threadIdx.x] : 0u;
-        (void)block_exclusive_scan<kScanColThreads>(c, s_scan, total);
-        if (threadIdx.x == 0) s_carry = total;
-    }
-    __syncthreads();
-    uint32_t *col = tile_hist + (size_t)d * stride;
-    for (uint32_t base = 0; base < ntiles; base += kScanColThreads) {
-        const uint32_t t = base + threadIdx.x;
-        const uint32_t v = t < ntiles ? col[t] : 0u;
-        uint32_t total;
-        const uint32_t ex = block_exclusive_scan<kScanColThreads>(v, s_scan, total);
-        const uint32_t carry = s_carry;
-        if (t < ntiles) col[t] = ex + carry;
-        __syncthreads();
-        if (threadIdx.x == 0) s_carry = carry + total;
-        __syncthreads();
+        prefix_publish(tile_rows, blockIdx.x, threadIdx.x, v);
+        if (v) atomicAdd(global_hist + threadIdx.x, v);
     }
 }
 
 template <typename KeyT, typename ValT, int VALMODE, bool WRITE_KEYS, bool RANGES, bool FULL>
 __device__ __forceinline__ void radix_scatter_tile(const KeyT *__restrict__ keys_in, const ValT *__restrict__ vals_in, uint32_t iota_top,
                                                    KeyT *__restrict__ keys_out, ValT *__restrict__ vals_out, uint32_t n, uint32_t tile,
-                                                   int shift, uint32_t dmask, const uint32_t *__restrict__ tile_offsets, uint32_t stride,
+                                                   int shift, uint32_t dmask, const PrefixRows &tile_rows, const uint32_t *global_hist,
                                                    uint2 *ranges, unsigned char *s_raw, uint32_t *s_tile_count, uint32_t *s_tile_start,
                                                    uint32_t *s_gbase, uint32_t *s_scan) {
     uint32_t(*s_whist)[kRadix + 1] = reinterpret_cast<uint32_t(*)[kRadix + 1]>(s_raw);
@@ -280,15 +330,16 @@
     const int tid = threadIdx.x, lane = tid & 31, warp = tid >> 5;
     const uint32_t tile_base = tile * (uint32_t)kRadixTile;
     const uint32_t run_base = tile_base + (uint32_t)warp * (32 * kRadixItems) + lane;
-    for (int i = tid; i < kRadixWarps * (kRadix + 1); i += kRadixThreads) (&s_whist[0][0])[i] = 0;
-
     uint32_t key[kRadixItems];
 #pragma unroll
     for (int k = 0; k < kRadixItems; ++k) {
         const uint32_t e = run_base + (uint32_t)k * 32;
         key[k] = (FULL || e < n) ? (uint32_t)keys_in[e] : 0xffffffffu;
     }
-    const uint32_t my_offset = tid < kRadix ? tile_offsets[(size_t)tid * stride + tile] : 0u;
+    const uint32_t dg = tid & (kRadix - 1);
+    const uint32_t dtotal = tid >= kRadix ? global_hist[dg] : 0u;
+    const uint32_t part = prefix_before(tile_rows, tile, reinterpret_cast<uint32_t *>(s_raw));
+    for (int i = tid; i < kRadixWarps * (kRadix + 1); i += kRadixThreads) (&s_whist[0][0])[i] = 0;
     uint32_t peers[kRadixItems];
 #pragma unroll
     for (int k = 0; k < kRadixItems; ++k) {
@@ -319,13 +370,17 @@
         s_tile_count[tid] = run;
     }
     __syncthreads();
+    const uint32_t valid = FULL ? (uint32_t)kRadixTile : (n - tile_base);
+    uint32_t tile_start;
     {
         uint32_t total;
-        const uint32_t c = tid < kRadix ? s_tile_count[tid] : 0u;
-        const uint32_t ex = block_exclusive_scan<kRadixThreads>(c, s_scan, total);
-        if (tid < kRadix) { s_tile_start[tid] = ex; s_gbase[tid] = my_offset - ex; }
-    }
-    __syncthreads();
+        const uint32_t c = tid < kRadix ? s_tile_count[tid] : dtotal;
+        tile_start = block_exclusive_scan<kRadixThreads>(c, s_scan, total);
+        if (tid < kRadix) s_tile_start[tid] = tile_start;
+        else s_gbase[dg] = tile_start - valid;
+    }
+    __syncthreads();
+    if (tid < kRadix) s_gbase[tid] += part - tile_start;
 #pragma unroll
     for (int k = 0; k < kRadixItems; ++k) {
         const uint32_t d = (key[k] >> shift) & dmask;
@@ -345,7 +400,6 @@
         }
     }
     __syncthreads();
-    const uint32_t valid = FULL ? (uint32_t)kRadixTile : (n - tile_base);
 #pragma unroll
     for (int k = 0; k < kRadixItems; ++k) {
         const uint32_t q = (uint32_t)k * kRadixThreads + tid;
@@ -368,14 +422,11 @@
 k_radix_scatter(const KeyT *__restrict__ keys_in, const ValT *__restrict__ vals_in, uint32_t iota_top,
                 KeyT *__restrict__ keys_out, ValT *__restrict__ vals_out, uint32_t n_host,
                 const unsigned long long *__restrict__ n_dev, unsigned long long n_cap, int shift, int bits,
-                const uint32_t *__restrict__ tile_offsets, uint32_t stride, uint2 *ranges, uint32_t *clear_hist, SortControl *reset_ctl) {
+                PrefixRows tile_rows, const uint32_t *global_hist, uint2 *ranges, SortControl *reset_ctl) {
     pdl_enter();
     const uint32_t n = n_dev ? (uint32_t)min(*n_dev, n_cap) : n_host;
     const uint32_t tile = blockIdx.x;
-    if (tile == 0) {
-        if (clear_hist && threadIdx.x < kRadix) clear_hist[threadIdx.x] = 0;
-        if (reset_ctl && threadIdx.x == 0) { reset_ctl->dmin = 2147483640; reset_ctl->dmax = -2147483640; }
-    }
+    if (tile == 0 && reset_ctl && threadIdx.x == 0) { reset_ctl->dmin = 2147483640; reset_ctl->dmax = -2147483640; }
     const uint64_t tile_base = (uint64_t)tile * kRadixTile;
     if (tile_base >= n) return;
     __shared__ __align__(16) unsigned char s_raw[kRadixTile * (sizeof(KeyT) + sizeof(ValT)) > kRadixWarps * (kRadix + 1) * 4
@@ -387,11 +438,11 @@
     __shared__ uint32_t s_scan[40];
     const uint32_t dmask = (1u << bits) - 1u;
     if (tile_base + kRadixTile <= n)
-        radix_scatter_tile<KeyT, ValT, VALMODE, WRITE_KEYS, RANGES, true>(keys_in, vals_in, iota_top, keys_out, vals_out, n, tile, shift, dmask, tile_offsets, stride,
-                                                                          ranges, s_raw, s_tile_count, s_tile_start, s_gbase, s_scan);
+        radix_scatter_tile<KeyT, ValT, VALMODE, WRITE_KEYS, RANGES, true>(keys_in, vals_in, iota_top, keys_out, vals_out, n, tile, shift, dmask, tile_rows,
+                                                                          global_hist, ranges, s_raw, s_tile_count, s_tile_start, s_gbase, s_scan);
     else
-        radix_scatter_tile<KeyT, ValT, VALMODE, WRITE_KEYS, RANGES, false>(keys_in, vals_in, iota_top, keys_out, vals_out, n, tile, shift, dmask, tile_offsets, stride,
-                                                                           ranges, s_raw, s_tile_count, s_tile_start, s_gbase, s_scan);
+        radix_scatter_tile<KeyT, ValT, VALMODE, WRITE_KEYS, RANGES, false>(keys_in, vals_in, iota_top, keys_out, vals_out, n, tile, shift, dmask, tile_rows,
+                                                                           global_hist, ranges, s_raw, s_tile_count, s_tile_start, s_gbase, s_scan);
 }
 
 __global__ void k_copy_head(const uint32_t *__restrict__ indexes, uint32_t *__restrict__ out, uint32_t s0) {
@@ -464,9 +515,9 @@
 template <typename KeyT, typename ValT>
 static void launch_radix_scatter(uint32_t grid, bool first, bool write_keys, bool want_ranges, int valmode, const KeyT *kin, const ValT *vin,
                                  uint32_t iota_top, KeyT *kout, ValT *vout, uint32_t n, const unsigned long long *n_dev, unsigned long long n_cap,
-                                 int shift, int bits, const uint32_t *tile_offsets, uint32_t stride, uint2 *ranges, uint32_t *clear_hist, SortControl *reset_ctl,
-                                 cudaStream_t st) {
-#define GS_PASS(VM, WK, RG) gs_launch(k_radix_scatter<KeyT, ValT, VM, WK, RG>, grid, kRadixThreads, 0, st, kin, vin, iota_top, kout, vout, n, n_dev, n_cap, shift, bits, tile_offsets, stride, ranges, clear_hist, reset_ctl)
+                                 int shift, int bits, const PrefixRows &tile_rows, const uint32_t *global_hist,
+                                 uint2 *ranges, SortControl *reset_ctl, cudaStream_t st) {
+#define GS_PASS(VM, WK, RG) gs_launch(k_radix_scatter<KeyT, ValT, VM, WK, RG>, grid, kRadixThreads, 0, st, kin, vin, iota_top, kout, vout, n, n_dev, n_cap, shift, bits, tile_rows, global_hist, ranges, reset_ctl)
     if (!first) valmode = kValArray;
     if (want_ranges && !write_keys) { GS_PASS(kValArray, false, true); }
     else if (want_ranges) {
@@ -480,17 +531,29 @@
 #undef GS_PASS
 }
 
-struct RadixNames { const char *hist[4], *scan[4], *scatter[4]; };
+struct RadixNames { const char *hist[4], *scatter[4]; };
+
+static inline RadixLayout radix_layout(unsigned long long n_grid, int npasses) {
+    RadixLayout L;
+    L.P = prefix_layout((n_grid + kRadixTile - 1) / kRadixTile);
+    L.npasses = npasses;
+    return L;
+}
+static inline void radix_clear_rows(SortControl *ctl, uint32_t *scratch, const RadixLayout &L, cudaStream_t st, uint32_t &launches) {
+    gs_launch(k_radix_clear, 8, 256, 0, st, ctl, L.super_base(scratch), (uint32_t)L.super_words());
+    ++launches;
+}
 
 template <typename KeyT, typename ValT>
 static void radix_sort_pairs(KeyT *keys0, KeyT *keys1, const ValT *vals_src, uint32_t iota_top, int first_valmode, ValT *vtmp0,
                              ValT *vtmp1, ValT *vals_final, uint32_t n, const unsigned long long *n_dev, unsigned long long n_cap,
-                             const PassPlan &pl, SortControl *ctl, uint32_t *tile_hist, uint32_t stride, bool hist0_done, uint2 *ranges,
+                             const PassPlan &pl, SortControl *ctl, uint32_t *scratch, bool hist0_done, uint2 *ranges,
                              cudaStream_t st, uint32_t &launches, Profiler *prof, const RadixNames &names, bool self_clean = false,
                              bool keep_final_keys = false ,
                              KeyT **final_keys = nullptr) {
     const unsigned long long n_grid = n_dev ? n_cap : n;
-    const uint32_t tiles = (uint32_t)((n_grid + kRadixTile - 1) / kRadixTile);
+    const RadixLayout L = radix_layout(n_grid, pl.npasses);
+    const uint32_t tiles = L.P.items;
     if (!tiles) return;
     KeyT *kin = keys0, *kout = keys1;
     const ValT *vin = vals_src;
@@ -498,30 +561,24 @@
     for (int p = 0; p < pl.npasses; ++p) {
         const bool last = (p == pl.npasses - 1);
         ValT *vout = last ? vals_final : vt[p & 1];
-        uint32_t *th = tile_hist + (size_t)p * kRadix * stride;
+        const PrefixRows rows = L.pass(scratch, p);
         if (!(p == 0 && hist0_done)) {
-            gs_launch(k_radix_hist<KeyT>, tiles, kRadixThreads, 0, st, kin, n, n_dev, n_cap, pl.shift[p], pl.bits[p], th, stride, &ctl->hist[p][0], 1);
+            gs_launch(k_radix_hist<KeyT>, tiles, kRadixThreads, 0, st, kin, n, n_dev, n_cap, pl.shift[p], pl.bits[p], rows, &ctl->hist[p][0]);
             ++launches;
             if (prof) prof->mark(names.hist[p], st);
         }
-        gs_launch(k_radix_scan, 1u << pl.bits[p], kScanColThreads, 0, st, th, stride, n, n_dev, n_cap, &ctl->hist[p][0]);
-        ++launches;
-        if (prof) prof->mark(names.scan[p], st);
         if (last && final_keys) *final_keys = kout;
         launch_radix_scatter<KeyT, ValT>(tiles, p == 0, !last || keep_final_keys, last && ranges != nullptr, first_valmode, kin, vin, iota_top, kout, vout, n, n_dev, n_cap,
-                                   pl.shift[p], pl.bits[p], th, stride, ranges, self_clean ? &ctl->hist[p][0] : nullptr,
-                                   (self_clean && last) ? ctl : nullptr, st);
+                                   pl.shift[p], pl.bits[p], rows, &ctl->hist[p][0], ranges, (self_clean && last) ? ctl : nullptr, st);
         ++launches;
         if (prof) prof->mark(names.scatter[p], st);
         vin = vout;
         KeyT *t = kin; kin = kout; kout = t;
     }
 }
-static inline size_t radix_tile_hist_words(unsigned long long n, int npasses, uint32_t *stride_out) {
+static inline size_t radix_tile_hist_words(unsigned long long n, int npasses) {
     const size_t tiles = (size_t)((n + kRadixTile - 1) / kRadixTile);
-    const size_t stride = (tiles + 31) & ~(size_t)31;
-    if (stride_out) *stride_out = (uint32_t)stride;
-    return stride * kRadix * (size_t)npasses;
-}
-
-}
+    return (size_t)npasses * kRadix * (2 * tiles + 6);
+}
+
+}
```

Measured after the change: 3331 (median of 6 runs). +2.1%, better.
